# nkkrnkl/category-agnostic-pose-estimation

Measured on AMD Instinct MI355X. Metric: episodes/sec (1-shot, 256x256, 17kpt) training step, higher is better.
Workload: dtype f32 storage/accumulate, GEMMs as bf16x3 split (3 bf16 MFMAs per product); 1 GPU; configs[1]: 1-shot training step (fwd+loss+bwd+clip+AdamW at learning rate 0, dropout on), 256x256, 17 kpt, ResNet-50 + deformable transformer, 16 episodes x 2 queries per GPU; episodes_per_gpu=16, queries_per_episode=2, image_size=256, global_batch_episodes=16, parallelism=dp1, weights=random init (no checkpoint offline)

## Files before the change

### category-agnostic-pose-estimation_amd/csrc/msda.hip

```cpp
#include <stdlib.h>
#include "common.h"

namespace {

struct Levels {
  int H[4], W[4], start[4];
};

constexpr int HEADS = 8, HD = 32, CH = HEADS * HD;

__device__ __forceinline__ int sel4(const int (&a)[4], int l) { return l == 0 ? a[0] : (l == 1 ? a[1] : (l == 2 ? a[2] : a[3])); }

__global__ void __launch_bounds__(256) msda_fwd_kernel(const float* __restrict__ value, const float* __restrict__ offw,
                                                        const float* __restrict__ ref, float* __restrict__ out,
                                                        Levels lv, int N, int S, int Lq, int L, int P, int blocks_per_image) {
  const int lane = threadIdx.x & 63, wv = threadIdx.x >> 6;
  int n, chunk;
  {
    const int b = blockIdx.x;
    const int xcd = b & 7, loc = b >> 3;
    const int imgs_per_x = (N + 7) >> 3;
    const int ii = loc / blocks_per_image;
    chunk = loc - ii * blocks_per_image;
    n = ii * 8 + xcd;
    if (ii >= imgs_per_x || n >= N) return;
  }
  const int q = chunk * 4 + wv;
  if (q >= Lq) return;
  const int LP = L * P;
  const int h = lane >> 3, c4 = lane & 7;
  const long long qrow = (long long)n * Lq + q;
  const float* ow = offw + qrow * (HEADS * LP * 3);
  const float* offs = ow + h * LP * 2;
  const float* logit = ow + HEADS * LP * 2 + h * LP;
  float px[2], py[2], lg[2];
  int lev[2];
#pragma unroll
  for (int s = 0; s < 2; ++s) {
    const int j = c4 + 8 * s;
    if (j < LP) {
      const int l = j / P;
      lev[s] = l;
      const float rx = ref[(qrow * L + l) * 2 + 0], ry = ref[(qrow * L + l) * 2 + 1];
      const float ox = offs[j * 2 + 0], oy = offs[j * 2 + 1];
      const float Wf = (float)sel4(lv.W, l), Hf = (float)sel4(lv.H, l);
      px[s] = (rx + ox / Wf) * Wf - 0.5f;
      py[s] = (ry + oy / Hf) * Hf - 0.5f;
      lg[s] = logit[j];
    } else {
      lev[s] = 0; px[s] = 0.f; py[s] = 0.f; lg[s] = -INFINITY;
    }
  }
  float mx = fmaxf(lg[0], lg[1]);
  mx = fmaxf(mx, __shfl_xor(mx, 1, 64)); mx = fmaxf(mx, __shfl_xor(mx, 2, 64)); mx = fmaxf(mx, __shfl_xor(mx, 4, 64));
  float e0 = __expf(lg[0] - mx), e1 = __expf(lg[1] - mx);
  float sm = e0 + e1;
  sm += __shfl_xor(sm, 1, 64); sm += __shfl_xor(sm, 2, 64); sm += __shfl_xor(sm, 4, 64);
  const float inv = 1.f / sm;
  const float aw[2] = {e0 * inv, e1 * inv};

  float4 acc = make_float4(0.f, 0.f, 0.f, 0.f);
  const float* vbase = value + (long long)n * S * CH + h * HD + c4 * 4;
#pragma unroll
  for (int s = 0; s < 2; ++s) {
#pragma unroll
    for (int jj = 0; jj < 8; ++jj) {
      const int j = jj + 8 * s;
      if (j >= LP) break;
      const int src = (lane & ~7) | jj;
      const float x = __shfl(px[s], src, 64), y = __shfl(py[s], src, 64), a = __shfl(aw[s], src, 64);
      const int l = __shfl(lev[s], src, 64);
      const int W = sel4(lv.W, l), H = sel4(lv.H, l);
      const float xf = floorf(x), yf = floorf(y);
      const float fx = x - xf, fy = y - yf;
      const int x0 = (int)xf, y0 = (int)yf;
      const float* vl = vbase + (long long)sel4(lv.start, l) * CH;
      const bool xa = x0 >= 0 && x0 < W, xb = x0 + 1 >= 0 && x0 + 1 < W;
      const bool ya = y0 >= 0 && y0 < H, yb = y0 + 1 >= 0 && y0 + 1 < H;
      float4 v;
      if (ya && xa) { v = *reinterpret_cast<const float4*>(vl + (long long)(y0 * W + x0) * CH); const float w = a * (1.f - fx) * (1.f - fy);
        acc.x += w * v.x; acc.y += w * v.y; acc.z += w * v.z; acc.w += w * v.w; }
      if (ya && xb) { v = *reinterpret_cast<const float4*>(vl + (long long)(y0 * W + x0 + 1) * CH); const float w = a * fx * (1.f - fy);
        acc.x += w * v.x; acc.y += w * v.y; acc.z += w * v.z; acc.w += w * v.w; }
      if (yb && xa) { v = *reinterpret_cast<const float4*>(vl + (long long)((y0 + 1) * W + x0) * CH); const float w = a * (1.f - fx) * fy;
        acc.x += w * v.x; acc.y += w * v.y; acc.z += w * v.z; acc.w += w * v.w; }
      if (yb && xb) { v = *reinterpret_cast<const float4*>(vl + (long long)((y0 + 1) * W + x0 + 1) * CH); const float w = a * fx * fy;
        acc.x += w * v.x; acc.y += w * v.y; acc.z += w * v.z; acc.w += w * v.w; }
    }
  }
  *reinterpret_cast<float4*>(out + qrow * CH + h * HD + c4 * 4) = acc;
}

__device__ __forceinline__ float half_sum32(float v) {
  v += __shfl_xor(v, 1, 64); v += __shfl_xor(v, 2, 64); v += __shfl_xor(v, 4, 64);
  v += __shfl_xor(v, 8, 64); v += __shfl_xor(v, 16, 64);
  return v;
}

__global__ void __launch_bounds__(256) msda_bwd_kernel(const float* __restrict__ d_out, const float* __restrict__ value,
                                                        const float* __restrict__ offw, const float* __restrict__ ref,
                                                        float* __restrict__ d_value, float* __restrict__ d_offw,
                                                        float* __restrict__ d_ref, Levels lv, int N, int S, int Lq, int L,
                                                        int P, long long total_waves) {
  const int lane = threadIdx.x & 63, wv = threadIdx.x >> 6;
  const long long wid = (long long)blockIdx.x * 4 + wv;
  if (wid >= total_waves) return;
  const int pair = (int)(wid & 3);
  const long long qrow = wid >> 2;
  const int n = (int)(qrow / Lq);
  const int hh = lane >> 5, c = lane & 31;
  const int h = pair * 2 + hh;
  const int LP = L * P;
  const int j = c & 15;
  const int rowlen = HEADS * LP * 3;
  const float* ow = offw + qrow * rowlen;
  float px = 0.f, py = 0.f, lg = -INFINITY;
  int l_own = 0;
  if (j < LP) {
    l_own = j / P;
    const float rx = ref[(qrow * L + l_own) * 2 + 0], ry = ref[(qrow * L + l_own) * 2 + 1];
    const float ox = ow[(h * LP + j) * 2 + 0], oy = ow[(h * LP + j) * 2 + 1];
    const float Wf = (float)sel4(lv.W, l_own), Hf = (float)sel4(lv.H, l_own);
    px = (rx + ox / Wf) * Wf - 0.5f;
    py = (ry + oy / Hf) * Hf - 0.5f;
    lg = ow[HEADS * LP * 2 + h * LP + j];
  }
  float mx = lg;
  mx = fmaxf(mx, __shfl_xor(mx, 1, 64)); mx = fmaxf(mx, __shfl_xor(mx, 2, 64));
  mx = fmaxf(mx, __shfl_xor(mx, 4, 64)); mx = fmaxf(mx, __shfl_xor(mx, 8, 64));
  const float e = __expf(lg - mx);
  float sm = e;
  sm += __shfl_xor(sm, 1, 64); sm += __shfl_xor(sm, 2, 64); sm += __shfl_xor(sm, 4, 64); sm += __shfl_xor(sm, 8, 64);
  const float aw = e / sm;

  const float go = d_out[qrow * CH + h * HD + c];
  const float* vbase = value + (long long)n * S * CH + h * HD + c;
  float* dvbase = d_value + (long long)n * S * CH + h * HD + c;
  float my_daw = 0.f, my_dpx = 0.f, my_dpy = 0.f;
  for (int jj = 0; jj < LP; ++jj) {
    const int src = (lane & 32) | jj;
    const float x = __shfl(px, src, 64), y = __shfl(py, src, 64), a = __shfl(aw, src, 64);
    const int l = __shfl(l_own, src, 64);
    const int W = sel4(lv.W, l), H = sel4(lv.H, l);
    const float xf = floorf(x), yf = floorf(y);
    const float fx = x - xf, fy = y - yf;
    const int x0 = (int)xf, y0 = (int)yf;
    const long long lofs = (long long)sel4(lv.start, l) * CH;
    const bool xa = x0 >= 0 && x0 < W, xb = x0 + 1 >= 0 && x0 + 1 < W;
    const bool ya = y0 >= 0 && y0 < H, yb = y0 + 1 >= 0 && y0 + 1 < H;
    float v00 = 0.f, v01 = 0.f, v10 = 0.f, v11 = 0.f;
    const float ga = go * a;
    if (ya && xa) { const long long o = lofs + (long long)(y0 * W + x0) * CH; v00 = vbase[o]; atomicAdd(dvbase + o, ga * (1.f - fx) * (1.f - fy)); }
    if (ya && xb) { const long long o = lofs + (long long)(y0 * W + x0 + 1) * CH; v01 = vbase[o]; atomicAdd(dvbase + o, ga * fx * (1.f - fy)); }
    if (yb && xa) { const long long o = lofs + (long long)((y0 + 1) * W + x0) * CH; v10 = vbase[o]; atomicAdd(dvbase + o, ga * (1.f - fx) * fy); }
    if (yb && xb) { const long long o = lofs + (long long)((y0 + 1) * W + x0 + 1) * CH; v11 = vbase[o]; atomicAdd(dvbase + o, ga * fx * fy); }
    const float samp = (1.f - fy) * ((1.f - fx) * v00 + fx * v01) + fy * ((1.f - fx) * v10 + fx * v11);
    const float dsx = (1.f - fy) * (v01 - v00) + fy * (v11 - v10);
    const float dsy = (1.f - fx) * (v10 - v00) + fx * (v11 - v01);
    const float r_aw = half_sum32(go * samp);
    const float r_px = half_sum32(ga * dsx);
    const float r_py = half_sum32(ga * dsy);
    if (j == jj) { my_daw = r_aw; my_dpx = r_px; my_dpy = r_py; }
  }
  float dot = aw * my_daw;
  dot += __shfl_xor(dot, 1, 64); dot += __shfl_xor(dot, 2, 64); dot += __shfl_xor(dot, 4, 64); dot += __shfl_xor(dot, 8, 64);
  const float dlogit = aw * (my_daw - dot);
  float* dow = d_offw + qrow * rowlen;
  if (c < 16 && j < LP) {
    dow[(h * LP + j) * 2 + 0] = my_dpx;
    dow[(h * LP + j) * 2 + 1] = my_dpy;
    dow[HEADS * LP * 2 + h * LP + j] = dlogit;
  }
  if (d_ref) {
    float rx = (c < 16 && j < LP) ? my_dpx * (float)sel4(lv.W, l_own) : 0.f;
    float ry = (c < 16 && j < LP) ? my_dpy * (float)sel4(lv.H, l_own) : 0.f;
    if (P == 4) {
      rx += __shfl_xor(rx, 1, 64); rx += __shfl_xor(rx, 2, 64);
      ry += __shfl_xor(ry, 1, 64); ry += __shfl_xor(ry, 2, 64);
      if (c < 16 && j < LP && (j & 3) == 0) {
        atomicAdd(&d_ref[(qrow * L + l_own) * 2 + 0], rx);
        atomicAdd(&d_ref[(qrow * L + l_own) * 2 + 1], ry);
      }
    } else if (c < 16 && j < LP) {
      atomicAdd(&d_ref[(qrow * L + l_own) * 2 + 0], rx);
      atomicAdd(&d_ref[(qrow * L + l_own) * 2 + 1], ry);
    }
  }
}



template <int CTRL>
__device__ __forceinline__ float dpp_f(float v) {
  return __builtin_bit_cast(float, __builtin_amdgcn_update_dpp(0, __builtin_bit_cast(int, v), CTRL, 0xf, 0xf, true));
}
__device__ __forceinline__ float sum8(float v) { v += dpp_f<0xB1>(v); v += dpp_f<0x4E>(v); v += dpp_f<0x141>(v); return v; }
__device__ __forceinline__ float max8(float v) {
  v = fmaxf(v, dpp_f<0xB1>(v)); v = fmaxf(v, dpp_f<0x4E>(v)); v = fmaxf(v, dpp_f<0x141>(v));
  return v;
}
__device__ __forceinline__ float sum16(float v) { v = sum8(v); v += dpp_f<0x140>(v); return v; }
__device__ __forceinline__ float max16(float v) { v = max8(v); v = fmaxf(v, dpp_f<0x140>(v)); return v; }

struct Tap { unsigned i00, i01, i10, i11; float fx, fy; };
__device__ __forceinline__ Tap make_tap(float px, float py, int W, int H, int start, bool live, int S) {
  const float xf = floorf(px), yf = floorf(py);
  Tap t;
  t.fx = px - xf; t.fy = py - yf;
  const int x0 = (int)xf, y0 = (int)yf;
  const bool xa = x0 >= 0 && x0 < W, xb = x0 + 1 >= 0 && x0 + 1 < W;
  const bool ya = y0 >= 0 && y0 < H, yb = y0 + 1 >= 0 && y0 + 1 < H;
  const int base = start + y0 * W + x0;
  t.i00 = (live && ya && xa) ? (unsigned)base : (unsigned)S;
  t.i01 = (live && ya && xb) ? (unsigned)(base + 1) : (unsigned)S;
  t.i10 = (live && yb && xa) ? (unsigned)(base + W) : (unsigned)S;
  t.i11 = (live && yb && xb) ? (unsigned)(base + W + 1) : (unsigned)S;
  return t;
}

__global__ void __launch_bounds__(256) msda_fwd_rec_kernel(const float* __restrict__ value, const float* __restrict__ offw,
                                                            const float* __restrict__ ref, float* __restrict__ out, Levels lv,
                                                            int N, int S, int Lq, int L, int P, int blocks_per_image) {
  __shared__ uint2 rec_ids[4][HEADS * 16];
  __shared__ float4 rec_w[4][HEADS * 16];
  const int lane = threadIdx.x & 63, wv = threadIdx.x >> 6;
  int n, chunk;
  {
    const int b = blockIdx.x;
    const int xcd = b & 7, loc = b >> 3;
    const int ii = loc / blocks_per_image;
    chunk = loc - ii * blocks_per_image;
    n = ii * 8 + xcd;
    if (n >= N) return;
  }
  const int q = chunk * 4 + wv;
  if (q >= Lq) return;
  const int LP = L * P;
  const int h = lane >> 3, i = lane & 7;
  const long long qrow = (long long)n * Lq + q;
  const float* ow = offw + qrow * (HEADS * LP * 3);
  float px[2], py[2], lg[2];
  int W[2], H[2], st[2];
#pragma unroll
  for (int s = 0; s < 2; ++s) {
    const int j = i + 8 * s;
    px[s] = 0.f; py[s] = 0.f; lg[s] = -INFINITY; W[s] = 1; H[s] = 1; st[s] = 0;
    if (j < LP) {
      const int l = j / P;
      W[s] = sel4(lv.W, l); H[s] = sel4(lv.H, l); st[s] = sel4(lv.start, l);
      const float2 rr = *reinterpret_cast<const float2*>(ref + (qrow * L + l) * 2);
      const float2 oo = *reinterpret_cast<const float2*>(ow + (h * LP + j) * 2);
      const float Wf = (float)W[s], Hf = (float)H[s];
      px[s] = (rr.x + oo.x / Wf) * Wf - 0.5f;
      py[s] = (rr.y + oo.y / Hf) * Hf - 0.5f;
      lg[s] = ow[HEADS * LP * 2 + h * LP + j];
    }
  }
  const float mx = max8(fmaxf(lg[0], lg[1]));
  const float e0 = __expf(lg[0] - mx), e1 = __expf(lg[1] - mx);
  const float inv = 1.f / sum8(e0 + e1);
  const float aw[2] = {e0 * inv, e1 * inv};
#pragma unroll
  for (int s = 0; s < 2; ++s) {
    const int j = i + 8 * s;
    const Tap t = make_tap(px[s], py[s], W[s], H[s], st[s], j < LP, S);
    const unsigned cl = (unsigned)(S - 1);
    float4 w = make_float4(aw[s] * (1.f - t.fx) * (1.f - t.fy), aw[s] * t.fx * (1.f - t.fy), aw[s] * (1.f - t.fx) * t.fy,
                           aw[s] * t.fx * t.fy);
    if (t.i00 >= (unsigned)S) w.x = 0.f;
    if (t.i01 >= (unsigned)S) w.y = 0.f;
    if (t.i10 >= (unsigned)S) w.z = 0.f;
    if (t.i11 >= (unsigned)S) w.w = 0.f;
    rec_ids[wv][h * 16 + j] = make_uint2(min(t.i00, cl) | (min(t.i01, cl) << 16), min(t.i10, cl) | (min(t.i11, cl) << 16));
    rec_w[wv][h * 16 + j] = w;
  }
  const float* vb = value + (long long)n * S * CH + h * HD + i * 4;
  const uint2* rid = &rec_ids[wv][h * 16];
  const float4* rw = &rec_w[wv][h * 16];
  constexpr int PF = 4;
  float4 v[PF + 1][4];
  auto fetch = [&](int j, int slot) {
    const uint2 ids = rid[j];
    v[slot][0] = *reinterpret_cast<const float4*>(vb + (ids.x & 0xFFFFu) * (unsigned)CH);
    v[slot][1] = *reinterpret_cast<const float4*>(vb + (ids.x >> 16) * (unsigned)CH);
    v[slot][2] = *reinterpret_cast<const float4*>(vb + (ids.y & 0xFFFFu) * (unsigned)CH);
    v[slot][3] = *reinterpret_cast<const float4*>(vb + (ids.y >> 16) * (unsigned)CH);
  };
#pragma unroll
  for (int j = 0; j < PF; ++j)
    if (j < LP) fetch(j, j);
  float4 acc = make_float4(0.f, 0.f, 0.f, 0.f);
#pragma unroll
  for (int j = 0; j < 16; ++j) {
    if (j >= LP) continue;
    if (j + PF < LP) fetch(j + PF, (j + PF) % (PF + 1));
    const int slot = j % (PF + 1);
    const float4 w = rw[j];
    acc.x += w.x * v[slot][0].x + w.y * v[slot][1].x + w.z * v[slot][2].x + w.w * v[slot][3].x;
    acc.y += w.x * v[slot][0].y + w.y * v[slot][1].y + w.z * v[slot][2].y + w.w * v[slot][3].y;
    acc.z += w.x * v[slot][0].z + w.y * v[slot][1].z + w.z * v[slot][2].z + w.w * v[slot][3].z;
    acc.w += w.x * v[slot][0].w + w.y * v[slot][1].w + w.z * v[slot][2].w + w.w * v[slot][3].w;
  }
  *reinterpret_cast<float4*>(out + qrow * CH + h * HD + i * 4) = acc;
}

__global__ void __launch_bounds__(256) msda_bwd_offw_kernel(const float* __restrict__ d_out, const float* __restrict__ value,
                                                             const float* __restrict__ offw, const float* __restrict__ ref,
                                                             float* __restrict__ d_offw, float* __restrict__ d_ref, Levels lv,
                                                             int N, int S, int Lq, int L, int P, int blocks_per_image) {
  __shared__ uint4 recs[4][HEADS * 16];
  const int lane = threadIdx.x & 63, wv = threadIdx.x >> 6;
  int n, chunk;
  {
    const int b = blockIdx.x;
    const int xcd = b & 7, loc = b >> 3;
    const int ii = loc / blocks_per_image;
    chunk = loc - ii * blocks_per_image;
    n = ii * 8 + xcd;
    if (n >= N) return;
  }
  const int q = chunk * 4 + wv;
  if (q >= Lq) return;
  const int LP = L * P;
  const int h = lane >> 3, i = lane & 7;
  const long long qrow = (long long)n * Lq + q;
  const int rowlen = HEADS * LP * 3;
  const float* ow = offw + qrow * rowlen;
  float lg[2], aw[2];
  int lev[2];
#pragma unroll
  for (int s = 0; s < 2; ++s) {
    const int j = i + 8 * s;
    const bool live = j < LP;
    float px = 0.f, py = 0.f;
    int W = 1, H = 1, st = 0;
    lg[s] = -INFINITY; lev[s] = 0;
    if (live) {
      const int l = j / P;
      lev[s] = l;
      W = sel4(lv.W, l); H = sel4(lv.H, l); st = sel4(lv.start, l);
      const float2 rr = *reinterpret_cast<const float2*>(ref + (qrow * L + l) * 2);
      const float2 oo = *reinterpret_cast<const float2*>(ow + (h * LP + j) * 2);
      const float Wf = (float)W, Hf = (float)H;
      px = (rr.x + oo.x / Wf) * Wf - 0.5f;
      py = (rr.y + oo.y / Hf) * Hf - 0.5f;
      lg[s] = ow[HEADS * LP * 2 + h * LP + j];
    }
    const Tap t = make_tap(px, py, W, H, st, live, S);
    recs[wv][h * 16 + j] = make_uint4(t.i00 | (t.i01 << 16), t.i10 | (t.i11 << 16), __float_as_uint(t.fx), __float_as_uint(t.fy));
  }
  {
    const float mx = max8(fmaxf(lg[0], lg[1]));
    const float e0 = __expf(lg[0] - mx), e1 = __expf(lg[1] - mx);
    const float inv = 1.f / sum8(e0 + e1);
    aw[0] = e0 * inv; aw[1] = e1 * inv;
  }
  const float4 go = *reinterpret_cast<const float4*>(d_out + qrow * CH + h * HD + i * 4);
  const float* vb = value + (long long)n * S * CH + h * HD + i * 4;
  float daw[2] = {0.f, 0.f}, dpx[2] = {0.f, 0.f}, dpy[2] = {0.f, 0.f};
  const uint4* myrec = &recs[wv][h * 16];
  constexpr int PF = 2;
  uint4 ra[PF + 1];
  float4 v[PF + 1][4];
  auto fetch = [&](int j, int slot) {
    ra[slot] = myrec[j];
    const unsigned ids[4] = {ra[slot].x & 0xFFFFu, ra[slot].x >> 16, ra[slot].y & 0xFFFFu, ra[slot].y >> 16};
#pragma unroll
    for (int k = 0; k < 4; ++k) {
      const unsigned idc = min(ids[k], (unsigned)(S - 1));
      const float4 x = *reinterpret_cast<const float4*>(vb + idc * (unsigned)CH);
      v[slot][k] = ids[k] < (unsigned)S ? x : make_float4(0.f, 0.f, 0.f, 0.f);
    }
  };
#pragma unroll
  for (int j = 0; j < PF; ++j)
    if (j < LP) fetch(j, j);
#pragma unroll
  for (int j = 0; j < 16; ++j) {
    if (j >= LP) continue;
    if (j + PF < LP) fetch(j + PF, (j + PF) % (PF + 1));
    const int slot = j % (PF + 1);
    const float fx = __uint_as_float(ra[slot].z), fy = __uint_as_float(ra[slot].w);
    const float4 v00 = v[slot][0], v01 = v[slot][1], v10 = v[slot][2], v11 = v[slot][3];
    float p_aw = 0.f, p_x = 0.f, p_y = 0.f;
#define CAPE_TAP_CH(C)                                                             \
    {                                                                              \
      const float dt = v01.C - v00.C, db = v11.C - v10.C;                          \
      const float top = v00.C + fx * dt, bot = v10.C + fx * db;                    \
      p_aw += go.C * (top + fy * (bot - top));                                     \
      p_x += go.C * (dt + fy * (db - dt));                                         \
      p_y += go.C * (bot - top);                                                   \
    }
    CAPE_TAP_CH(x) CAPE_TAP_CH(y) CAPE_TAP_CH(z) CAPE_TAP_CH(w)
#undef CAPE_TAP_CH
    const float r_aw = sum8(p_aw), r_x = sum8(p_x), r_y = sum8(p_y);
    if (i == (j & 7)) { daw[j >> 3] = r_aw; dpx[j >> 3] = r_x; dpy[j >> 3] = r_y; }
  }
  const float dot = sum8(aw[0] * daw[0] + aw[1] * daw[1]);
  float* dow = d_offw + qrow * rowlen;
#pragma unroll
  for (int s = 0; s < 2; ++s) {
    const int j = i + 8 * s;
    const bool live = j < LP;
    const float gx = aw[s] * dpx[s], gy = aw[s] * dpy[s];
    if (live) {
      *reinterpret_cast<float2*>(dow + (h * LP + j) * 2) = make_float2(gx, gy);
      dow[HEADS * LP * 2 + h * LP + j] = aw[s] * (daw[s] - dot);
    }
    if (d_ref) {
      float rx = live ? gx * (float)sel4(lv.W, lev[s]) : 0.f;
      float ry = live ? gy * (float)sel4(lv.H, lev[s]) : 0.f;
      if (P == 4) {
        rx += dpp_f<0xB1>(rx); rx += dpp_f<0x4E>(rx);
        ry += dpp_f<0xB1>(ry); ry += dpp_f<0x4E>(ry);
        rx += __shfl_xor(rx, 8); rx += __shfl_xor(rx, 16); rx += __shfl_xor(rx, 32);
        ry += __shfl_xor(ry, 8); ry += __shfl_xor(ry, 16); ry += __shfl_xor(ry, 32);
        if (live && h == 0 && (i & 3) == 0) *reinterpret_cast<float2*>(&d_ref[(qrow * L + lev[s]) * 2]) = make_float2(rx, ry);
      } else if (live) {
        atomicAdd(&d_ref[(qrow * L + lev[s]) * 2 + 0], rx);
        atomicAdd(&d_ref[(qrow * L + lev[s]) * 2 + 1], ry);
      }
    }
  }
}

struct ValRec { uint2 ids; float4 w; };

template <int VC>
__global__ void __launch_bounds__(1024) msda_bwd_value_kernel(const float* __restrict__ d_out, const float* __restrict__ offw,
                                                              const float* __restrict__ ref, float* __restrict__ d_value,
                                                              Levels lv, int N, int S, int Lq, int L, int P) {
  constexpr int VS = VC, GROUPS = HD / VC, BPI = HEADS * GROUPS;
  constexpr int SLOTS = 64 / VC;
  extern __shared__ __attribute__((aligned(16))) double slab[];
  __shared__ uint2 rec_ids[16][64];
  __shared__ float4 rec_w[16][64];
  int n, sub;
  {
    const int b = blockIdx.x, xcd = b & 7, loc = b >> 3;
    n = (loc / BPI) * 8 + xcd;
    sub = loc % BPI;
    if (n >= N) return;
  }
  const int h = sub / GROUPS, grp = sub % GROUPS;
  for (int k = threadIdx.x; k < (S + 1) * VS; k += 1024) slab[k] = 0.0;
  __syncthreads();

  const int lane = threadIdx.x & 63, wv = threadIdx.x >> 6;
  const int g = lane >> 4, j = lane & 15;
  const int c = lane & (VC - 1), slot = lane / VC;
  static_assert(SLOTS * VC == 64 && 16 % VC == 0, "a slot's records must stay inside one query");
  const int LP = L * P;
  const int rowlen = HEADS * LP * 3;
  const int choff = h * HD + grp * VC + c;

  const int l_own = j < LP ? j / P : 0;
  const int W = sel4(lv.W, l_own), H = sel4(lv.H, l_own), st = sel4(lv.start, l_own);
  const float Wf = (float)W, Hf = (float)H;
  const int g2 = (slot * VC) >> 4;
  struct In { float2 rr, oo; float lg, go; };
  auto fetch = [&](int qb) {
    In in;
    const int q = qb + g, q2 = qb + g2;
    const long long qrow = (long long)n * Lq + min(q, Lq - 1);
    const float* ow = offw + qrow * rowlen;
    const int jj = min(j, LP - 1);
    in.rr = *reinterpret_cast<const float2*>(ref + (qrow * L + l_own) * 2);
    in.oo = *reinterpret_cast<const float2*>(ow + (h * LP + jj) * 2);
    in.lg = ow[HEADS * LP * 2 + h * LP + jj];
    in.go = d_out[((long long)n * Lq + min(q2, Lq - 1)) * CH + choff];
    return in;
  };
  In cur = fetch(wv * 4);
  for (int qb = wv * 4; qb < Lq; qb += 64) {
    const In nxt = fetch(min(qb + 64, Lq - 1));
    const int q = qb + g;
    const bool qlive = q < Lq;
    {
      const bool slive = qlive && j < LP;
      const float px = (cur.rr.x + cur.oo.x / Wf) * Wf - 0.5f;
      const float py = (cur.rr.y + cur.oo.y / Hf) * Hf - 0.5f;
      const float lg = slive ? cur.lg : -INFINITY;
      const float mx = max16(lg);
      const float e = slive ? __expf(lg - mx) : 0.f;
      const float sm = sum16(e);
      const float aw = slive ? e / sm : 0.f;
      const Tap t = make_tap(px, py, W, H, st, slive, S);
      rec_ids[wv][lane] = make_uint2(t.i00 | (t.i01 << 16), t.i10 | (t.i11 << 16));
      rec_w[wv][lane] = make_float4(aw * (1.f - t.fx) * (1.f - t.fy), aw * t.fx * (1.f - t.fy), aw * (1.f - t.fx) * t.fy,
                                    aw * t.fx * t.fy);
    }
    const float go = (qb + g2 < Lq) ? cur.go : 0.f;
    const int rbase = slot * VC;
#pragma unroll
    for (int s = 0; s < VC; ++s) {
      const uint2 ids = rec_ids[wv][rbase + s];
      const float4 w = rec_w[wv][rbase + s];
      atomicAdd(&slab[(ids.x & 0xFFFFu) * VS + c], (double)(go * w.x));
      atomicAdd(&slab[(ids.x >> 16) * VS + c], (double)(go * w.y));
      atomicAdd(&slab[(ids.y & 0xFFFFu) * VS + c], (double)(go * w.z));
      atomicAdd(&slab[(ids.y >> 16) * VS + c], (double)(go * w.w));
    }
    cur = nxt;
  }
  __syncthreads();
  float* dvb = d_value + (long long)n * S * CH + h * HD + grp * VC;
  if constexpr (VC >= 4) {
    constexpr int Q = VC / 4;
    for (int k = threadIdx.x; k < S * Q; k += 1024) {
      const int p_ = k / Q, c4 = (k % Q) * 4;
      const double* sp = &slab[p_ * VS + c4];
      *reinterpret_cast<float4*>(dvb + (long long)p_ * CH + c4) = make_float4((float)sp[0], (float)sp[1], (float)sp[2], (float)sp[3]);
    }
  } else {
    for (int k = threadIdx.x; k < S; k += 1024)
      *reinterpret_cast<float2*>(dvb + (long long)k * CH) = make_float2((float)slab[k * VS], (float)slab[k * VS + 1]);
  }
}

typedef float v2f __attribute__((ext_vector_type(2)));

template <int VP>
__global__ void __launch_bounds__(1024) msda_bwd_value_fx_kernel(const float* __restrict__ d_out, const float* __restrict__ offw,
                                                                 const float* __restrict__ ref, float* __restrict__ d_value,
                                                                 Levels lv, int N, int S, int Lq, int L, int P) {
  constexpr int VC = 2 * VP, GROUPS = HD / VC, BPI = HEADS * GROUPS;
  constexpr int SLOTS = 64 / VP;
  extern __shared__ __attribute__((aligned(16))) unsigned long long fslab[];
  __shared__ uint4 rec_off[16][64];
  __shared__ float4 rec_w[16][64];
  __shared__ unsigned gmax_w[16];
  int n, sub;
  {
    const int b = blockIdx.x, xcd = b & 7, loc = b >> 3;
    n = (loc / BPI) * 8 + xcd;
    sub = loc % BPI;
    if (n >= N) return;
  }
  const int h = sub / GROUPS, grp = sub % GROUPS;
  const int lane = threadIdx.x & 63, wv = threadIdx.x >> 6;
  const int ch0 = h * HD + grp * VC;
  for (int k = threadIdx.x; k < (S + 1) * VP; k += 1024) fslab[k] = 0ull;
  unsigned gb = 0u;
  for (int k = threadIdx.x; k < Lq * VP; k += 1024) {
    const int q = k / VP, c2 = (k - q * VP) * 2;
    const float2 v = *reinterpret_cast<const float2*>(d_out + ((long long)n * Lq + q) * CH + ch0 + c2);
    gb = max(gb, max(__float_as_uint(fabsf(v.x)), __float_as_uint(fabsf(v.y))));
  }
#pragma unroll
  for (int o = 32; o >= 1; o >>= 1) gb = max(gb, (unsigned)__shfl_xor((int)gb, o));
  if (lane == 0) gmax_w[wv] = gb;
  __syncthreads();
  gb = gmax_w[0];
#pragma unroll
  for (int k = 1; k < 16; ++k) gb = max(gb, gmax_w[k]);
  const bool finite = gb < 0x7f800000u;
  float scale = 0.f, inv_scale = 0.f;
  if (finite && gb != 0u) {
    int e;
    (void)frexpf(__uint_as_float(gb), &e);
    const int lq_bits = Lq > 1 ? 32 - __clz(Lq - 1) : 0;
    const int sx = max(-126, min(126, min(30 - lq_bits, 21) - e));
    scale = ldexpf(1.f, sx);
    inv_scale = ldexpf(1.f, -sx);
  }

  const int g = lane >> 4, j = lane & 15;
  const int c = lane & (VP - 1), slot = lane / VP;
  static_assert(SLOTS * VP == 64 && 16 % VP == 0, "a slot's records must stay inside one query");
  const int LP = L * P;
  const int rowlen = HEADS * LP * 3;
  const int choff = ch0 + 2 * c;
  const int l_own = j < LP ? j / P : 0;
  const int W = sel4(lv.W, l_own), H = sel4(lv.H, l_own), st = sel4(lv.start, l_own);
  const float Wf = (float)W, Hf = (float)H;
  const int g2 = (slot * VP) >> 4;
  struct In { float2 rr, oo, go; float lg; };
  auto fetch = [&](int qb) {
    In in;
    const int q = qb + g, q2 = qb + g2;
    const long long qrow = (long long)n * Lq + min(q, Lq - 1);
    const float* ow = offw + qrow * rowlen;
    const int jj = min(j, LP - 1);
    in.rr = *reinterpret_cast<const float2*>(ref + (qrow * L + l_own) * 2);
    in.oo = *reinterpret_cast<const float2*>(ow + (h * LP + jj) * 2);
    in.lg = ow[HEADS * LP * 2 + h * LP + jj];
    in.go = *reinterpret_cast<const float2*>(d_out + ((long long)n * Lq + min(q2, Lq - 1)) * CH + choff);
    return in;
  };
  char* const slab_c = reinterpret_cast<char*>(fslab) + c * 8;
  auto add2 = [&](unsigned off, float wgt, v2f gg) {
    const v2f t = __builtin_elementwise_fma(gg, (v2f)(wgt), (v2f)(12582912.f));
    const int v0 = (int)__float_as_uint(t.x) - 0x4B400000, v1 = (int)__float_as_uint(t.y) - 0x4B400000;
    const unsigned long long pk = ((unsigned long long)(unsigned)(v1 + (v0 >> 31)) << 32) | (unsigned)v0;
    atomicAdd(reinterpret_cast<unsigned long long*>(slab_c + off), pk);
  };
  In cur = fetch(wv * 4);
  for (int qb = wv * 4; qb < Lq; qb += 64) {
    const In nxt = fetch(min(qb + 64, Lq - 1));
    const int q = qb + g;
    const bool qlive = q < Lq;
    {
      const bool slive = qlive && j < LP;
      const float px = (cur.rr.x + cur.oo.x / Wf) * Wf - 0.5f;
      const float py = (cur.rr.y + cur.oo.y / Hf) * Hf - 0.5f;
      const float lg = slive ? cur.lg : -INFINITY;
      const float mx = max16(lg);
      const float e = slive ? __expf(lg - mx) : 0.f;
      const float sm = sum16(e);
      const float aw = slive ? e / sm : 0.f;
      const Tap t = make_tap(px, py, W, H, st, slive, S);
      rec_off[wv][lane] = make_uint4(t.i00 * (VP * 8), t.i01 * (VP * 8), t.i10 * (VP * 8), t.i11 * (VP * 8));
      rec_w[wv][lane] = make_float4(aw * (1.f - t.fx) * (1.f - t.fy), aw * t.fx * (1.f - t.fy), aw * (1.f - t.fx) * t.fy,
                                    aw * t.fx * t.fy);
    }
    const bool live2 = qb + g2 < Lq;
    v2f gg;
    gg.x = live2 ? cur.go.x * scale : 0.f;
    gg.y = live2 ? cur.go.y * scale : 0.f;
    const int rbase = slot * VP;
#pragma unroll
    for (int s = 0; s < VP; ++s) {
      const uint4 off = rec_off[wv][rbase + s];
      const float4 w = rec_w[wv][rbase + s];
      add2(off.x, w.x, gg);
      add2(off.y, w.y, gg);
      add2(off.z, w.z, gg);
      add2(off.w, w.w, gg);
    }
    cur = nxt;
  }
  __syncthreads();
  float* dvb = d_value + (long long)n * S * CH + ch0;
  const float nanv = __uint_as_float(0x7fc00000u);
  auto dec = [&](unsigned long long wd, float& lo, float& hi) {
    const int l = (int)(unsigned)wd;
    const int hh = (int)(unsigned)(wd >> 32) - (l >> 31);
    lo = finite ? (float)l * inv_scale : nanv;
    hi = finite ? (float)hh * inv_scale : nanv;
  };
  constexpr int Q = VP / 2;
  for (int k = threadIdx.x; k < S * Q; k += 1024) {
    const int p_ = k / Q, c2 = (k % Q) * 2;
    float4 o;
    dec(fslab[p_ * VP + c2], o.x, o.y);
    dec(fslab[p_ * VP + c2 + 1], o.z, o.w);
    *reinterpret_cast<float4*>(dvb + (long long)p_ * CH + c2 * 2) = o;
  }
}

int fill_levels(Levels& lv, const int* shapes, const int* level_start, int L, int S) {
  CAPE_REQUIRE(L >= 1 && L <= 4, "cape_msda: L=%d must be in 1..4", L);
  long long tot = 0;
  for (int l = 0; l < 4; ++l) {
    lv.H[l] = l < L ? shapes[2 * l] : 1;
    lv.W[l] = l < L ? shapes[2 * l + 1] : 1;
    lv.start[l] = l < L ? level_start[l] : 0;
    if (l < L) {
      CAPE_REQUIRE(lv.H[l] > 0 && lv.W[l] > 0 && lv.start[l] == tot, "cape_msda: level %d shape/start inconsistent", l);
      tot += (long long)lv.H[l] * lv.W[l];
    }
  }
  CAPE_REQUIRE(tot == S, "cape_msda: sum(H*W)=%lld != S=%d", tot, S);
  return 0;
}

}

extern "C" int cape_msda_fwd(const float* value, const float* offw, const float* ref, const int* shapes,
                             const int* level_start, float* out, int N, int S, int Lq, int L, int P,
                             cape_stream_t stream) {
  CAPE_REQUIRE(value && offw && ref && shapes && level_start && out, "cape_msda_fwd: null pointer");
  CAPE_REQUIRE(P >= 1 && L * P <= 16, "cape_msda_fwd: L*P=%d must be <= 16", L * P);
  if (N <= 0 || Lq <= 0) return 0;
  Levels lv;
  if (fill_levels(lv, shapes, level_start, L, S)) return 1;
  const int bpi = (Lq + 3) / 4;
  const int imgs_per_x = (N + 7) / 8;
  const long long blocks = (long long)imgs_per_x * bpi * 8;
  CAPE_REQUIRE(blocks < (1ll << 31), "cape_msda_fwd: grid too large");
  static const bool shuffle_form = getenv("CAPE_MSDA_FWD_SHUFFLE") != nullptr;
  if (S < 65535 && !shuffle_form)
    hipLaunchKernelGGL(msda_fwd_rec_kernel, dim3((unsigned)blocks), dim3(256), 0, as_stream(stream), value, offw, ref, out, lv,
                       N, S, Lq, L, P, bpi);
  else
    hipLaunchKernelGGL(msda_fwd_kernel, dim3((unsigned)blocks), dim3(256), 0, as_stream(stream), value, offw, ref, out, lv,
                       N, S, Lq, L, P, bpi);
  CAPE_LAUNCH_CHECK("cape_msda_fwd");
  return 0;
}

static int msda_bwd_check(const float* d_out, const float* value, const float* offw, const float* ref, const int* shapes,
                          const int* level_start, float* d_value, float* d_offw, int L, int P) {
  CAPE_REQUIRE(d_out && value && offw && ref && shapes && level_start && d_value && d_offw, "cape_msda_bwd: null pointer");
  CAPE_REQUIRE(P >= 1 && L * P <= 16, "cape_msda_bwd: L*P=%d must be <= 16", L * P);
  return 0;
}

extern "C" int cape_msda_bwd_atomic(const float* d_out, const float* value, const float* offw, const float* ref,
                                    const int* shapes, const int* level_start, float* d_value, float* d_offw, float* d_ref,
                                    int N, int S, int Lq, int L, int P, cape_stream_t stream) {
  if (msda_bwd_check(d_out, value, offw, ref, shapes, level_start, d_value, d_offw, L, P)) return 1;
  if (N <= 0 || Lq <= 0) return 0;
  Levels lv;
  if (fill_levels(lv, shapes, level_start, L, S)) return 1;
  hipError_t e = hipMemsetAsync(d_value, 0, sizeof(float) * (size_t)N * S * CH, as_stream(stream));
  if (e == hipSuccess && d_ref) e = hipMemsetAsync(d_ref, 0, sizeof(float) * (size_t)N * Lq * L * 2, as_stream(stream));
  if (e != hipSuccess) return cape_set_error("cape_msda_bwd_atomic: memset: %s", hipGetErrorString(e));
  const long long waves = (long long)N * Lq * 4;
  const long long blocks = (waves + 3) / 4;
  CAPE_REQUIRE(blocks < (1ll << 31), "cape_msda_bwd_atomic: grid too large");
  hipLaunchKernelGGL(msda_bwd_kernel, dim3((unsigned)blocks), dim3(256), 0, as_stream(stream), d_out, value, offw, ref,
                     d_value, d_offw, d_ref, lv, N, S, Lq, L, P, waves);
  CAPE_LAUNCH_CHECK("cape_msda_bwd_atomic");
  return 0;
}

extern "C" int cape_msda_bwd(const float* d_out, const float* value, const float* offw, const float* ref,
                             const int* shapes, const int* level_start, float* d_value, float* d_offw, float* d_ref,
                             int N, int S, int Lq, int L, int P, cape_stream_t stream) {
  return cape_msda_bwd_ex(d_out, value, offw, ref, shapes, level_start, d_value, d_offw, d_ref, N, S, Lq, L, P, 0, stream);
}

extern "C" int cape_msda_bwd_ex(const float* d_out, const float* value, const float* offw, const float* ref,
                                const int* shapes, const int* level_start, float* d_value, float* d_offw, float* d_ref,
                                int N, int S, int Lq, int L, int P, int value_accum, cape_stream_t stream) {
  CAPE_REQUIRE(value_accum == 0 || value_accum == 1, "cape_msda_bwd_ex: value_accum must be 0 (fp64 slab) or 1 (fixed-point pairs)");
  if (msda_bwd_check(d_out, value, offw, ref, shapes, level_start, d_value, d_offw, L, P)) return 1;
  if (N <= 0 || Lq <= 0) return 0;
  const size_t kMaxSlab = 160 * 1024 - 16 * 64 * (sizeof(uint4) + sizeof(float4)) - 512;
  int vc = 8;
  while (vc >= 2 && (size_t)(S + 1) * vc * sizeof(double) > kMaxSlab) vc >>= 1;
  const size_t slab_bytes = (size_t)(S + 1) * vc * sizeof(double);
  static const bool force_atomic = getenv("CAPE_MSDA_BWD_ATOMIC") != nullptr;
  const long long imgs8 = ((long long)N + 7) / 8;
  const int bpi = (Lq + 3) / 4;
  const long long vblocks = imgs8 * 8 * HEADS * (HD / (vc < 2 ? 2 : vc));
  if (force_atomic || vc < 2 || S >= 65535 || vblocks >= (1ll << 31) || imgs8 * 8 * bpi >= (1ll << 31))
    return cape_msda_bwd_atomic(d_out, value, offw, ref, shapes, level_start, d_value, d_offw, d_ref, N, S, Lq, L, P, stream);
  Levels lv;
  if (fill_levels(lv, shapes, level_start, L, S)) return 1;
  static bool attr_done = false;
  if (!attr_done) {
    hipError_t e = hipFuncSetAttribute(reinterpret_cast<const void*>(msda_bwd_value_kernel<8>),
                                       hipFuncAttributeMaxDynamicSharedMemorySize, (int)kMaxSlab);
    if (e == hipSuccess) e = hipFuncSetAttribute(reinterpret_cast<const void*>(msda_bwd_value_kernel<4>),
                                                 hipFuncAttributeMaxDynamicSharedMemorySize, (int)kMaxSlab);
    if (e == hipSuccess) e = hipFuncSetAttribute(reinterpret_cast<const void*>(msda_bwd_value_kernel<2>),
                                                 hipFuncAttributeMaxDynamicSharedMemorySize, (int)kMaxSlab);
    if (e == hipSuccess) e = hipFuncSetAttribute(reinterpret_cast<const void*>(msda_bwd_value_fx_kernel<8>),
                                                 hipFuncAttributeMaxDynamicSharedMemorySize, (int)kMaxSlab);
    if (e == hipSuccess) e = hipFuncSetAttribute(reinterpret_cast<const void*>(msda_bwd_value_fx_kernel<4>),
                                                 hipFuncAttributeMaxDynamicSharedMemorySize, (int)kMaxSlab);
    if (e == hipSuccess) e = hipFuncSetAttribute(reinterpret_cast<const void*>(msda_bwd_value_fx_kernel<2>),
                                                 hipFuncAttributeMaxDynamicSharedMemorySize, (int)kMaxSlab);
    if (e != hipSuccess) return cape_set_error("cape_msda_bwd: hipFuncSetAttribute: %s", hipGetErrorString(e));
    attr_done = true;
  }
  if (d_ref && P != 4) {
    hipError_t e = hipMemsetAsync(d_ref, 0, sizeof(float) * (size_t)N * Lq * L * 2, as_stream(stream));
    if (e != hipSuccess) return cape_set_error("cape_msda_bwd: memset: %s", hipGetErrorString(e));
  }
#define VALUE_LAUNCH(W)                                                                                                     \
  hipLaunchKernelGGL((msda_bwd_value_kernel<W>), dim3((unsigned)vblocks), dim3(1024), slab_bytes, as_stream(stream), d_out, offw, \
                     ref, d_value, lv, N, S, Lq, L, P)
#define VALUE_LAUNCH_FX(W)                                                                                                  \
  hipLaunchKernelGGL((msda_bwd_value_fx_kernel<W>), dim3((unsigned)fxblocks), dim3(1024), fx_bytes, as_stream(stream),           \
                     d_out, offw, ref, d_value, lv, N, S, Lq, L, P)
  if (value_accum == 1) {
    int vp = vc;
    while (vp > 2 && imgs8 * 8 * HEADS * (HD / (2 * vp)) < 256) vp >>= 1;
    const long long fxblocks = imgs8 * 8 * HEADS * (HD / (2 * vp));
    const size_t fx_bytes = (size_t)(S + 1) * vp * sizeof(unsigned long long);
    if (vp == 8) VALUE_LAUNCH_FX(8); else if (vp == 4) VALUE_LAUNCH_FX(4); else VALUE_LAUNCH_FX(2);
  } else {
    if (vc == 8) VALUE_LAUNCH(8); else if (vc == 4) VALUE_LAUNCH(4); else VALUE_LAUNCH(2);
  }
#undef VALUE_LAUNCH_FX
#undef VALUE_LAUNCH
  hipLaunchKernelGGL(msda_bwd_offw_kernel, dim3((unsigned)(imgs8 * 8 * bpi)), dim3(256), 0, as_stream(stream), d_out, value, offw,
                     ref, d_offw, d_ref, lv, N, S, Lq, L, P, bpi);
  CAPE_LAUNCH_CHECK("cape_msda_bwd");
  return 0;
}
```

### category-agnostic-pose-estimation_amd/hip/functional.py

```python
import contextlib
import ctypes
import os

import torch

from . import lib, ops


class Runtime:
    rng = None
    direct_grad = False
    use_side_stream = os.environ.get("CAPE_SIDE_STREAM", "1") == "1"
    side = None
    on_param_grad = []
    capture_keep = None

    pending = []
    side_dirty = False

    defer_wgrad = os.environ.get("CAPE_DEFER_WGRAD", "1") == "1"
    wgrad_group = int(os.environ.get("CAPE_WGRAD_GROUP", "12"))
    wq = {}
    wq_total = 0
    wq_notify = []
# ... 536 lines not shown
    return BottleneckFn.apply(x, w1, w2, w3, wd, bn1[0], bn1[1], bn2[0], bn2[1], bn3[0], bn3[1], sd, bd, int(stride), torch.is_grad_enabled(),
                              int(dilation))


def conv_bn_act(x, weight, scale, shift, stride=1, pad=0, relu=False, residual=None, dilation=1):
    return ConvFn.apply(x, weight, scale, shift, residual, int(stride), int(pad), bool(relu), torch.is_grad_enabled(), int(dilation))


class AddLayerNormFn(torch.autograd.Function):
    @staticmethod
    def forward(ctx, x, y, gamma, beta, pos, dropout_p, rng_stream):
        x, y, pos = _c(x), _c(y), _c(pos)
        rng = Runtime.get_rng(x.device) if dropout_p > 0 else None
        out, mean, rstd, out_pos = ops.add_layernorm_fwd(x, y, gamma, beta, pos=pos, dropout_p=dropout_p, rng=rng,
                                                         rng_stream=rng_stream)
        ctx.save_for_backward(x, y, gamma, mean, rstd)
        ctx.refs = (gamma, beta)
        ctx.slot = _slot_of(x)
        ctx.meta = (dropout_p, rng_stream, pos is not None)
        ctx.set_materialize_grads(False)
        if pos is None:
            return out
        return out, out_pos

    @staticmethod
    def backward(ctx, d_out, d_out_pos=None):
        x, y, gamma, mean, rstd = ctx.saved_tensors
        p, stream, has_pos = ctx.meta
        g_pos = d_out_pos
        if d_out is None and d_out_pos is None:
            return None, None, None, None, None, None, None
        if d_out is None:
            d_out, d_out_pos = d_out_pos, None
        d_out, d_out_pos = _c(d_out), _c(d_out_pos)
        pg = _ParamGrads(ctx.refs)
        rng = Runtime.get_rng(x.device) if p > 0 else None
        dx, dy = ops.add_layernorm_bwd(d_out, d_out_pos, x, y, gamma, mean, rstd, *pg.bufs, dropout_p=p, rng=rng,
                                       rng_stream=stream)
        if y is None or dy is not dx:
            _slot_offer(ctx.slot, dx)
        dpos = g_pos if (has_pos and ctx.needs_input_grad[4]) else None
        return (dx, (dy if y is not None else None)) + pg.result() + (dpos, None, None)


def add_layernorm(x, y, gamma, beta, pos=None, dropout_p=0.0, rng_stream=0):
    return AddLayerNormFn.apply(x, y, gamma, beta, pos, float(dropout_p), int(rng_stream))


class AddFn(torch.autograd.Function):
    @staticmethod
    def forward(ctx, a, b):
        return ops.add(_c(a), _c(b))

    @staticmethod
    def backward(ctx, g):
        return g, g


def add(a, b):
    return AddFn.apply(a, b)


class FanOutFn(torch.autograd.Function):

    @staticmethod
    def forward(ctx, x, k, slot):
        ctx.k, ctx.slot = k, slot
        ctx.set_materialize_grads(False)
        return tuple(x.view_as(x) for _ in range(k))

    @staticmethod
    def backward(ctx, *grads):
        ctx.slot.buf = None
        gs, seen = [], set()
        for g in grads:
            if g is not None and (g.data_ptr(), g.numel()) not in seen:
                seen.add((g.data_ptr(), g.numel()))
                gs.append(g)
        if not gs:
            return None, None, None
        if len(gs) > 1 and len(gs) <= 8 and not all(g.is_contiguous() for g in gs) and all(_row_strided(g) for g in gs):
            return ops.add_n_rows(gs), None, None
        gs = [_c(g) for g in gs]
        out = gs[0]
        for i in range(0, len(gs) - 1, 7):
            out = ops.add_n([out] + gs[1 + i:8 + i]) if len(gs) > 1 else out
        return out, None, None


def _row_strided(g):
    if g.dim() < 2 or g.stride(-1) != 1 or g.shape[-1] % 4 or g.data_ptr() % 16 or g.stride(-2) % 4:
        return False
    st, sh = g.stride(), g.shape
    return all(st[i] == st[i + 1] * sh[i + 1] for i in range(len(sh) - 2))


def fanout(x, k):
    if k == 1 or not (torch.is_grad_enabled() and x.requires_grad):
        return (x,) * k
    slot = _Slot()
    outs = FanOutFn.apply(x, k, slot)
    for o in outs:
        o._cape_slot = slot
    return outs


class GeluFn(torch.autograd.Function):
    @staticmethod
    def forward(ctx, x):
        x = _c(x)
        ctx.save_for_backward(x)
        return ops.gelu(x)

    @staticmethod
    def backward(ctx, g):
        (x,) = ctx.saved_tensors
        return ops.gelu_bwd(x, _c(g))


def gelu(x):
    return GeluFn.apply(x)


class ScaleResidualFn(torch.autograd.Function):

    @staticmethod
    def forward(ctx, x, y, gamma):
        y = _c(y)
        ctx.has_x = x is not None
        ctx.save_for_backward(y, gamma)
        ctx.gref = gamma
        return ops.scale_residual(_c(x) if x is not None else torch.zeros_like(y), y, gamma)

    @staticmethod
    def backward(ctx, g):
        y, gamma = ctx.saved_tensors
        g = _c(g)
        dx = g if ctx.has_x else None
        if gamma is None:
            return dx, g, None
        pg = _ParamGrads((ctx.gref,))
        dy = ops.scale_residual_bwd(g, y, gamma, pg.bufs[0])
        return (dx, dy) + pg.result()


def scale_residual(x, y, gamma=None):
    return ScaleResidualFn.apply(x, y, gamma)


class BiAttnCoreFn(torch.autograd.Function):

    @staticmethod
    def forward(ctx, rv_l, rv_p, nheads, scale):
        rv_l, rv_p = _c(rv_l), _c(rv_p)
        B, Nl, D2 = rv_l.shape
        Np, D = rv_p.shape[1], D2 // 2
        ctx.route = "scalar"
        lat, s1 = ops.attn_core_fwd(ctx.route, rv_l[..., :D], rv_p[..., :D], rv_p[..., D:], B, nheads, Nl, Np, scale)
        pat, s2 = ops.attn_core_fwd(ctx.route, rv_p[..., :D], rv_l[..., :D], rv_l[..., D:], B, nheads, Np, Nl, scale)
        ctx.save_for_backward(rv_l, rv_p, lat, pat, *s1, *s2)
        ctx.meta = (nheads, scale)
        return lat, pat

    @staticmethod
    def backward(ctx, d_lat, d_pat):
        rv_l, rv_p, lat, pat, *saved = ctx.saved_tensors
        s1, s2 = saved[:len(saved) // 2], saved[len(saved) // 2:]
        nheads, scale = ctx.meta
        B, Nl, D2 = rv_l.shape
        Np, D = rv_p.shape[1], D2 // 2
        d_l, d_p = torch.empty_like(rv_l), torch.empty_like(rv_p)
        t_l, t_p = torch.empty_like(rv_l), torch.empty_like(rv_p)
        ops.attn_core_bwd(ctx.route, s1, _c(d_lat), rv_l[..., :D], rv_p[..., :D], rv_p[..., D:], lat, d_l[..., :D], d_p[..., :D],
                          d_p[..., D:], B, nheads, Nl, Np, scale)
        ops.attn_core_bwd(ctx.route, s2, _c(d_pat), rv_p[..., :D], rv_l[..., :D], rv_l[..., D:], pat, t_p[..., :D], t_l[..., :D],
                          d_l[..., D:], B, nheads, Np, Nl, scale)
        ops.add_n_rows([d_l[..., :D], t_l[..., :D]], out=d_l[..., :D])
        ops.add_n_rows([d_p[..., :D], t_p[..., :D]], out=d_p[..., :D])
        return d_l, d_p, None, None


def bi_attn_core(rv_l, rv_p, nheads, scale):
    return BiAttnCoreFn.apply(rv_l, rv_p, nheads, float(scale))


class AttnKVFn(torch.autograd.Function):

    @staticmethod
    def forward(ctx, r_q, rv_kv, nheads, scale):
        r_q, rv_kv = _c(r_q), _c(rv_kv)
        B, Nq, D = r_q.shape
        Nk = rv_kv.shape[1]
        ctx.route = "scalar"
        out, saved = ops.attn_core_fwd(ctx.route, r_q, rv_kv[..., :D], rv_kv[..., D:], B, nheads, Nq, Nk, scale)
        ctx.save_for_backward(r_q, rv_kv, out, *saved)
        ctx.meta = (nheads, scale)
        return out

    @staticmethod
    def backward(ctx, d_out):
        r_q, rv_kv, out, *saved = ctx.saved_tensors
        nheads, scale = ctx.meta
        B, Nq, D = r_q.shape
        Nk = rv_kv.shape[1]
        dq, dkv = torch.empty_like(r_q), torch.empty_like(rv_kv)
        ops.attn_core_bwd(ctx.route, saved, _c(d_out), r_q, rv_kv[..., :D], rv_kv[..., D:], out, dq, dkv[..., :D], dkv[..., D:], B, nheads,
                          Nq, Nk, scale)
        return dq, dkv, None, None


def attn_kv(r_q, rv_kv, nheads, scale):
    return AttnKVFn.apply(r_q, rv_kv, nheads, float(scale))


class LevelGroupNormFn(torch.autograd.Function):

    @staticmethod
    def forward(ctx, geo, *args):
        L = geo.L
        xs, gammas, betas = args[:L], args[L:2 * L], args[2 * L:3 * L]
        N, C = xs[0].shape[0], xs[0].shape[-1]
        out = torch.empty(N, geo.S, C, dtype=torch.float32, device=xs[0].device)
        stats = []
        xs = [_c(x) for x in xs]
        for l, x in enumerate(xs):
            h, w = geo.shapes[l]
            assert x.shape[1] == h and x.shape[2] == w
            stats.append(ops.groupnorm_fwd(x, gammas[l], betas[l], out[:, geo.starts[l]:], geo.S * C, N, h * w, C))
        ctx.geo = geo
        ctx.refs = (tuple(gammas), tuple(betas))
        ctx.save_for_backward(*xs, *gammas, *[s for st in stats for s in st])
        return out

    @staticmethod
    def backward(ctx, d_out):
        geo = ctx.geo
        L = geo.L
        sv = ctx.saved_tensors
        xs, gammas, st = sv[:L], sv[L:2 * L], sv[2 * L:]
        d_out = _c(d_out)
        N, S, C = d_out.shape
        dxs, dgs, dbs = [], [], []
        for l in range(L):
            h, w = geo.shapes[l]
            pg = _ParamGrads((ctx.refs[0][l], ctx.refs[1][l]))
            dx = ops.groupnorm_bwd(d_out[:, geo.starts[l]:], S * C, xs[l], gammas[l], st[2 * l], st[2 * l + 1], *pg.bufs, N,
                                   h * w, C)
            dg, db = pg.result()
            dxs.append(dx); dgs.append(dg); dbs.append(db)
        return (None, *dxs, *dgs, *dbs)


def level_groupnorm(geo, xs, gammas, betas):
    return LevelGroupNormFn.apply(geo, *xs, *gammas, *betas)


_SINE_CACHE = {}


class LevelPosFn(torch.autograd.Function):

    @staticmethod
    def forward(ctx, geo, level_embed, *masks_u8):
        N = masks_u8[0].shape[0]
        C = level_embed.shape[1]
        out = torch.empty(N, geo.S, C, dtype=torch.float32, device=level_embed.device)
        key = (tuple(m.data_ptr() for m in masks_u8), tuple(geo.shapes), N, C, str(level_embed.device))
        sine = _SINE_CACHE.get(key) if all(getattr(m, "_cape_all_false", False) for m in masks_u8) else None
        if sine is None:
            target = out
            if all(getattr(m, "_cape_all_false", False) for m in masks_u8) and not capturing():
                target = torch.empty_like(out)
            zero_row = torch.zeros(C, dtype=torch.float32, device=level_embed.device) if target is not out else None
            for l, m in enumerate(masks_u8):
                h, w = geo.shapes[l]
                ops.pos_sine_level(_c(m), zero_row if zero_row is not None else level_embed[l], target[:, geo.starts[l]:], geo.S * C, N, h, w, C)
            if target is not out:
                if len(_SINE_CACHE) >= 8:
                    _SINE_CACHE.pop(next(iter(_SINE_CACHE)))
                _SINE_CACHE[key] = sine = target
        if sine is not None:
            ops.level_embed_add(sine, _c(level_embed), geo, out)
        ctx.geo = geo
        ctx.N = N
        ctx.le_ref = level_embed
        return out

    @staticmethod
    def backward(ctx, d_pos):
        geo, N = ctx.geo, ctx.N
        d_pos = _c(d_pos)
        C = d_pos.shape[-1]
        pg = _ParamGrads((ctx.le_ref,))
        for l in range(geo.L):
            h, w = geo.shapes[l]
            ops.colsum(d_pos[0, geo.starts[l]:], h * w, C, pg.bufs[0][l], nbatch=N, batch_stride=geo.S * C)
        return (None,) + pg.result() + (None,) * geo.L


def level_pos(geo, level_embed, masks_u8):
    return LevelPosFn.apply(geo, level_embed, *masks_u8)


class MSDAFn(torch.autograd.Function):
    @staticmethod
    def forward(ctx, value, offw, ref, geo, P):
        value, offw, ref = _c(value), _c(offw), _c(ref)
        N, Lq = offw.shape[0], offw.shape[1]
        out = ops.msda_fwd(value, offw, ref, geo, N, Lq, P)
        ctx.save_for_backward(value, offw, ref)
        ctx.meta = (geo, N, Lq, P)
        return out

    @staticmethod
    def backward(ctx, d_out):
        value, offw, ref = ctx.saved_tensors
        geo, N, Lq, P = ctx.meta
        dv, do, dr = ops.msda_bwd(_c(d_out), value, offw, ref, geo, N, Lq, P, need_ref_grad=ctx.needs_input_grad[2])
        return dv, do, dr, None, None


def msda(value, offw, ref, geo, P=4):
    return MSDAFn.apply(value, offw, ref, geo, P)


def _from_row(t, r):
    return t if (t is None or r == 0) else t[r:]


def _col_blocks(groups, bufs, C):
    return [buf[..., j * C:(j + 1) * C] for (_, w, *_), buf in zip(groups, bufs) for j in range(w)]


class MHAFn(torch.autograd.Function):

    @staticmethod
    def forward(ctx, q_in, k_in, v_in, in_w, in_b, out_w, out_b, nheads, mask_mode, kpm_u8, dropout_p, rng_stream):
        ins = q_in, k_in, v_in = _c(q_in), _c(k_in), _c(v_in)
        N, Lq, C = q_in.shape
        Lk = k_in.shape[1]
        dev = q_in.device
        scale = (C // nheads) ** -0.5
        rng = Runtime.get_rng(dev) if dropout_p > 0 else None
        ctx.route = ops.attn_route(N, nheads, Lq, Lk, flash=False)
        if ctx.route != "mm" and k_in is v_in:
            layout = ((0, 3),) if q_in is k_in else ((0, 1), (1, 2))
        else:
            layout = ((0, 1), (1, 1), (2, 1))
        ctx.groups = tuple((r, w, r != 1 and ins[r] is k_in) for r, w in layout)
        bufs = [torch.empty(N, ins[r].shape[1], w * C, dtype=torch.float32, device=dev) for r, w in layout]
        for (r, w), buf in zip(layout, bufs):
            ops.gemm(ins[r].view(-1, C), _from_row(in_w, r * C), buf, N * ins[r].shape[1], w * C, C, bias=_from_row(in_b, r * C))
        q, k, v = _col_blocks(layout, bufs, C)
        O, saved = ops.attn_core_fwd(ctx.route, q, k, v, N, nheads, Lq, Lk, scale, mask_mode=mask_mode, kpm=kpm_u8, dropout_p=dropout_p,
                                     rng=rng, rng_stream=rng_stream)
        out = torch.empty(N, Lq, C, dtype=torch.float32, device=dev)
        ops.gemm(O.view(-1, C), out_w, out, N * Lq, C, C, bias=out_b)
        ctx.save_for_backward(q_in, k_in, v_in, in_w, out_w, q, k, v, O, kpm_u8, *saved)
        ctx.refs = (in_w, in_b, out_w, out_b)
        ctx.slot_q = _slot_of(q_in)
        ctx.meta = (nheads, mask_mode, dropout_p, rng_stream, scale)
        return out

    @staticmethod
    def backward(ctx, d_out):
        q_in, k_in, v_in, in_w, out_w, q, k, v, O, kpm, *saved = ctx.saved_tensors
        nheads, mask_mode, p, stream, scale = ctx.meta
        ins = q_in, k_in, v_in
        N, Lq, C = q_in.shape
        Lk = k_in.shape[1]
        dev = d_out.device
        d_out2 = _c(d_out).view(-1, C)
        Mq = N * Lq
        dO = torch.empty(Mq, C, dtype=torch.float32, device=dev)
        ops.gemm(d_out2, out_w, dO, Mq, C, C, a_mode=0, b_mode=1)
        pg = _ParamGrads(ctx.refs)
        d_in_w, d_in_b, d_out_w, d_out_b = pg.bufs
        with pg.side(d_out2, O):
            pg.gemm(d_out2, O.view(-1, C), d_out_w, C, C, Mq, a_mode=1, b_mode=1, accumulate=True,
                    split_k=ops.pick_split_k(C, C, Mq), colsum_out=d_out_b)
        dbufs = [torch.empty(N, ins[r].shape[1], w * C, dtype=torch.float32, device=dev) for r, w, _ in ctx.groups]
        dq, dk, dv = _col_blocks(ctx.groups, dbufs, C)
        rng = Runtime.get_rng(dev) if p > 0 else None
        ops.attn_core_bwd(ctx.route, saved, dO.view(N, Lq, C), q, k, v, O, dq, dk, dv, N, nheads, Lq, Lk, scale, mask_mode=mask_mode,
                          kpm=kpm, dropout_p=p, rng=rng, rng_stream=stream)
        pairs = list(zip(ctx.groups, dbufs))
        with pg.side(*dbufs, q_in, k_in, v_in):
            for (r, w, _), g in pairs:
                M = N * ins[r].shape[1]
                pg.gemm(g.view(-1, w * C), ins[r].view(-1, C), _from_row(d_in_w, r * C), w * C, C, M, a_mode=1, b_mode=1, lda=w * C,
                        accumulate=True, split_k=ops.pick_split_k(w * C, C, M), colsum_out=_from_row(d_in_b, r * C))
        d_in_w, d_in_b, d_out_w, d_out_b = pg.result()
        d_ins, dk_in = [None, None, None], None
        for (r, w, dup), g in pairs[1:] + pairs[:1]:
            live = [j for j in range(r, r + w) if ctx.needs_input_grad[j]]
            if not live:
                continue
            if dup and dk_in is not None:
                dst, acc = dk_in, True
            else:
                if r == 0 and len(pairs) == 2:
                    dst, acc = _grad_target(ctx.slot_q, ins[r].shape, dev)
                else:
                    dst, acc = torch.empty(ins[r].shape, dtype=torch.float32, device=dev), False
                d_ins[live[0]] = dst
            ops.gemm(g.view(-1, w * C), _from_row(in_w, r * C), dst, N * ins[r].shape[1], C, w * C, a_mode=0, b_mode=1, accumulate=acc)
            if live[0] == 1:
                dk_in = dst
        return (*d_ins, d_in_w, d_in_b, d_out_w, d_out_b, None, None, None, None, None)


class DecSelfAttnFn(torch.autograd.Function):

    @staticmethod
    def forward(ctx, tgt, pos, wq, wk, wv, in_w, in_b, out_w, out_b, nheads, dropout_p, rng_stream):
        N, L, C = tgt.shape
        M = N * L
        dev = tgt.device
        x, pos2 = _c(tgt).view(M, C), _c(pos).view(M, C)
        stacked = _adjacent(wq, wk) and _adjacent(wk, wv)
        qkv1 = torch.empty(M, 3 * C, dtype=torch.float32, device=dev)
        if stacked:
            ops.gemm(x, torch.as_strided(wq, (3 * C, C), (C, 1)), qkv1, M, 3 * C, C, residual=pos2, ldr=C, res_cols=C)
        else:
            ops.gemm(x, wq, qkv1, M, C, C, ldc=3 * C, residual=pos2, ldr=C)
            ops.gemm(x, wk, qkv1[:, C:], M, C, C, ldc=3 * C)
            ops.gemm(x, wv, qkv1[:, 2 * C:], M, C, C, ldc=3 * C)
        qkv2 = torch.empty(N, L, 3 * C, dtype=torch.float32, device=dev)
        ops.gemm(qkv1, in_w, qkv2, M, C, C, lda=3 * C, ldb=C, ldc=3 * C, bias=in_b,
                 batch=(3, 3, 0, C, 0, C * C, 0, C), bias_strides=(0, C))
        q, k, v = qkv2[..., :C], qkv2[..., C:2 * C], qkv2[..., 2 * C:]
        scale = (C // nheads) ** -0.5
        rng = Runtime.get_rng(dev) if dropout_p > 0 else None
        ctx.route = ops.attn_route(N, nheads, L, L, flash=True)
        O, saved = ops.attn_core_fwd(ctx.route, q, k, v, N, nheads, L, L, scale, mask_mode=1, dropout_p=dropout_p, rng=rng,
                                     rng_stream=rng_stream)
        out = torch.empty(N, L, C, dtype=torch.float32, device=dev)
        ops.gemm(O.view(M, C), out_w, out, M, C, C, bias=out_b)
        ctx.save_for_backward(x, wq, wk, wv, in_w, out_w, qkv1, qkv2, O, *saved)
        ctx.refs = (wq, wk, wv, in_w, in_b, out_w, out_b)
        ctx.meta = (nheads, dropout_p, rng_stream, scale, stacked, N, L, C)
        ctx.slot = _slot_of(tgt)
        return out

    @staticmethod
    def backward(ctx, d_out):
        x, wq, wk, wv, in_w, out_w, qkv1, qkv2, O, *saved = ctx.saved_tensors
        nheads, p, stream, scale, stacked, N, L, C = ctx.meta
        M = N * L
        dev = d_out.device
        d_out2 = _c(d_out).view(M, C)
        dO = torch.empty(M, C, dtype=torch.float32, device=dev)
        ops.gemm(d_out2, out_w, dO, M, C, C, a_mode=0, b_mode=1)
        dqkv2 = torch.empty(N, L, 3 * C, dtype=torch.float32, device=dev)
        dq, dk, dv = dqkv2[..., :C], dqkv2[..., C:2 * C], dqkv2[..., 2 * C:]
        q, k, v = qkv2[..., :C], qkv2[..., C:2 * C], qkv2[..., 2 * C:]
        rng = Runtime.get_rng(dev) if p > 0 else None
        ops.attn_core_bwd(ctx.route, saved, dO.view(N, L, C), q, k, v, O, dq, dk, dv, N, nheads, L, L, scale, mask_mode=1, dropout_p=p,
                          rng=rng, rng_stream=stream)
        dqkv1 = torch.empty(M, 3 * C, dtype=torch.float32, device=dev)
        ops.gemm(dqkv2.view(M, 3 * C), in_w, dqkv1, M, C, C, a_mode=0, b_mode=1, lda=3 * C, ldb=C, ldc=3 * C,
                 batch=(3, 3, 0, C, 0, C * C, 0, C))
        need_x, need_pos = ctx.needs_input_grad[0], ctx.needs_input_grad[1]
        dx = None
        if need_x:
            dx, acc = _grad_target(ctx.slot, (N, L, C), dev)
            if stacked:
                ops.gemm(dqkv1, torch.as_strided(wq, (3 * C, C), (C, 1)), dx, M, C, 3 * C, a_mode=0, b_mode=1, accumulate=acc)
            else:
                for i, w in enumerate((wq, wk, wv)):
                    ops.gemm(dqkv1[:, i * C:], w, dx, M, C, C, a_mode=0, b_mode=1, lda=3 * C, accumulate=acc or i > 0)

        pg = _ParamGrads(ctx.refs)
        d_wq, d_wk, d_wv, d_in_w, d_in_b, d_out_w, d_out_b = pg.bufs
        with pg.side(d_out2, O, dqkv2, qkv1, dqkv1, x):
            Mv = dqkv2.view(M, 3 * C)
            pg.gemm(d_out2, O.view(M, C), d_out_w, C, C, M, a_mode=1, b_mode=1, accumulate=True, split_k=ops.pick_split_k(C, C, M),
                    colsum_out=d_out_b)
            for i, dw in enumerate((d_wq, d_wk, d_wv)):
                pg.gemm(Mv[:, i * C:], qkv1[:, i * C:], d_in_w[i * C:], C, C, M, a_mode=1, b_mode=1, lda=3 * C, ldb=3 * C, accumulate=True,
                        split_k=ops.pick_split_k(C, C, M), colsum_out=d_in_b[i * C:])
                pg.gemm(dqkv1[:, i * C:], x, dw, C, C, M, a_mode=1, b_mode=1, lda=3 * C, ldb=C, accumulate=True,
                        split_k=ops.pick_split_k(C, C, M))
        dpos = dqkv1[:, :C].view(N, L, C) if need_pos else None
        return (dx, dpos) + pg.result() + (None, None, None)


def dec_self_attn(tgt, pos, wq, wk, wv, in_w, in_b, out_w, out_b, nheads=8, dropout_p=0.0, rng_stream=0):
    return DecSelfAttnFn.apply(tgt, pos, wq, wk, wv, in_w, in_b, out_w, out_b, nheads, float(dropout_p), int(rng_stream))


def mha(q_in, k_in, v_in, in_w, in_b, out_w, out_b, nheads=8, mask_mode=0, kpm_u8=None, dropout_p=0.0, rng_stream=0):
    return MHAFn.apply(q_in, k_in, v_in, in_w, in_b, out_w, out_b, nheads, mask_mode, kpm_u8, float(dropout_p), int(rng_stream))


class TokenEmbedFn(torch.autograd.Function):
    @staticmethod
    def forward(ctx, table, pad_idx, s11, s21, s12, s22, dx1, dx2, dy1, dy2):
        shape = s11.shape
        seqs = [_c(s).view(-1) for s in (s11, s21, s12, s22)]
        deltas = [_c(d).view(-1) for d in (dx1, dx2, dy1, dy2)]
        out = ops.token_embed_fwd(table, seqs, deltas)
        ctx.save_for_backward(*seqs, *deltas)
        ctx.t_ref = table
        ctx.meta = (table.shape, pad_idx)
        return out.view(*shape, table.shape[1])

    @staticmethod
    def backward(ctx, d_out):
        sv = ctx.saved_tensors
        tshape, pad_idx = ctx.meta
        pg = _ParamGrads((ctx.t_ref,))
        ops.token_embed_bwd(_c(d_out).view(-1, tshape[1]), sv[:4], sv[4:], pg.bufs[0], pad_idx if pad_idx is not None else -1)
        return pg.result() + (None,) * 9


def token_embed(table, pad_idx, s11, s21, s12, s22, dx1, dx2, dy1, dy2):
    return TokenEmbedFn.apply(table, pad_idx, s11, s21, s12, s22, dx1, dx2, dy1, dy2)


class QuerySineFn(torch.autograd.Function):
    @staticmethod
    def forward(ctx, ref):
        ref = _c(ref)
        ctx.save_for_backward(ref)
        return ops.query_sine_fwd(ref).view(*ref.shape[:-1], 256)

    @staticmethod
    def backward(ctx, d_out):
        (ref,) = ctx.saved_tensors
        return ops.query_sine_bwd(_c(d_out).view(-1, 256), ref).view_as(ref)


def query_sine(ref):
    return QuerySineFn.apply(ref)


class RefineFn(torch.autograd.Function):
    @staticmethod
    def forward(ctx, delta, ref):
        delta, ref = _c(delta), _c(ref)
        out = ops.refine_fwd(delta, ref)
        ctx.save_for_backward(out, ref)
        return out

    @staticmethod
    def backward(ctx, d_new):
        out, ref = ctx.saved_tensors
        d_delta, d_ref = ops.refine_bwd(_c(d_new), out, ref)
        return d_delta, d_ref


def refine(delta, ref):
    return RefineFn.apply(delta, ref)


class SigmoidFn(torch.autograd.Function):
    @staticmethod
    def forward(ctx, x):
        y = ops.sigmoid_fwd(_c(x))
        ctx.save_for_backward(y)
        return y

    @staticmethod
    def backward(ctx, dy):
        (y,) = ctx.saved_tensors
        return ops.sigmoid_bwd(_c(dy), y)


def sigmoid(x):
    return SigmoidFn.apply(x)


class RefScaleFn(torch.autograd.Function):

    @staticmethod
    def forward(ctx, ref, valid_ratios):
        ref, vr = _c(ref), _c(valid_ratios)
        N, Lq, _ = ref.shape
        L = vr.shape[1]
        ctx.save_for_backward(vr)
        ctx.meta = (N, Lq, L)
        return ops.ref_scale_fwd(ref, vr, Lq, L).view(N, Lq, L, 2)

    @staticmethod
    def backward(ctx, d):
        (vr,) = ctx.saved_tensors
        N, Lq, L = ctx.meta
        return ops.ref_scale_bwd(_c(d), vr, Lq, L).view(N, Lq, 2), None


def ref_scale(ref, valid_ratios):
    return RefScaleFn.apply(ref, valid_ratios)


class SupportEmbedFn(torch.autograd.Function):

    @staticmethod
    def forward(ctx, coords, W0, b0, pe1d):
        coords = _c(coords)
        N, P, _ = coords.shape
        C = W0.shape[0]
        h, pe = ops.support_embed_fwd(coords, W0, b0, pe1d, N, P, C)
        ctx.save_for_backward(h, coords)
        ctx.refs = (W0, b0)
        ctx.meta = (N, P, C)
        ctx.mark_non_differentiable(pe)
        ctx.set_materialize_grads(False)
        return h.view(N, P, C), pe.view(N, P, C)

    @staticmethod
    def backward(ctx, d_h, _d_pe):
        if d_h is None:
            return None, None, None, None
        h, coords = ctx.saved_tensors
        N, P, C = ctx.meta
        pg = _ParamGrads(ctx.refs)
        ops.support_embed_bwd(_c(d_h).view(-1, C), h, coords, *pg.bufs, N, P, C)
        return (None,) + pg.result() + (None,)


def support_embed(coords, W0, b0, pe1d):
    return SupportEmbedFn.apply(coords, W0, b0, pe1d)


class GCNAggFn(torch.autograd.Function):
# ... 156 lines not shown
```

### category-agnostic-pose-estimation_amd/hip/lib.py

```python
import ctypes
import os

import torch

from ctypes import POINTER, c_char_p, c_float, c_int, c_int32, c_int64, c_longlong, c_size_t, c_uint32, c_uint64, c_uint8, c_void_p

_HERE = os.path.dirname(os.path.abspath(__file__))
LIB_PATH = os.environ.get("CAPE_HIP_LIB", os.path.join(_HERE, "..", "csrc", "libcape_hip.so"))
LIB_PATH = os.path.abspath(LIB_PATH)

if not os.path.exists(LIB_PATH):
    raise ImportError(
        f"libcape_hip.so not found at {LIB_PATH}; build it with `python -c 'import __graft_entry__ as g; g.build()'` "
        "(or `make -C category-agnostic-pose-estimation_amd/csrc`).  There is no CPU fallback.")
try:
    _lib = ctypes.CDLL(LIB_PATH)
except OSError as e:
    raise ImportError(f"cannot load {LIB_PATH}: {e}") from e

_lib.cape_last_error.restype = c_char_p
_lib.cape_abi_version.restype = c_int


class GemmDesc(ctypes.Structure):
    _fields_ = [
        ("M", c_int), ("N", c_int), ("K", c_int), ("a_mode", c_int), ("b_mode", c_int),
        ("A", c_void_p), ("lda", c_longlong), ("B", c_void_p), ("ldb", c_longlong), ("C", c_void_p), ("ldc", c_longlong),
        ("cN", c_int), ("cH", c_int), ("cW", c_int), ("cC", c_int), ("cKH", c_int), ("cKW", c_int),
        ("cStride", c_int), ("cPad", c_int), ("cOH", c_int), ("cOW", c_int), ("cO", c_int),
        ("scale", c_void_p), ("bias", c_void_p), ("residual", c_void_p), ("ldr", c_longlong),
        ("relu", c_int), ("accumulate", c_int), ("split_k", c_int), ("dropout_p", c_float),
        ("rng_state", c_void_p), ("rng_stream", c_uint32), ("colsum_out", c_void_p), ("precision", c_int),
        ("B_packed", c_void_p),
        ("mask_src", c_void_p), ("ldm", c_longlong), ("mask_scale", c_float),
        ("batch", c_int), ("batch_div", c_int), ("sA0", c_longlong), ("sA1", c_longlong), ("sB0", c_longlong), ("sB1", c_longlong),
        ("sC0", c_longlong), ("sC1", c_longlong),
        ("res_cols", c_int), ("sBias0", c_longlong), ("sBias1", c_longlong),
        ("cPadX", c_int), ("cKHp", c_int), ("cKWp", c_int), ("cTapH0", c_int), ("cTapHS", c_int), ("cTapW0", c_int), ("cTapWS", c_int),
        ("cDil", c_int),
    ]


class PackItem(ctypes.Structure):
    _fields_ = [("B", c_void_p), ("out", c_void_p), ("ldb", c_longlong), ("N", c_int), ("K", c_int), ("b_mode", c_int), ("pad", c_int)]


class DecodeLinearDesc(ctypes.Structure):
    _fields_ = [
        ("N", c_int), ("K", c_int), ("Nout", c_int),
        ("X", c_void_p), ("ldx", c_longlong), ("in_gamma", c_void_p), ("in_beta", c_void_p), ("in_add", c_void_p), ("ld_add", c_longlong),
        ("W", c_void_p), ("ldw", c_longlong), ("bias", c_void_p),
        ("X2", c_void_p), ("ldx2", c_longlong), ("K2", c_int), ("W2", c_void_p), ("ldw2", c_longlong), ("n2", c_int),
        ("R", c_void_p), ("ldr", c_longlong), ("res_gamma", c_void_p), ("res_beta", c_void_p),
        ("relu", c_int), ("nseg", c_int), ("seg", c_int), ("out", c_void_p * 3), ("ldo", c_longlong * 3),
    ]


class DecodeTailDesc(ctypes.Structure):
    _fields_ = [
        ("N", c_int), ("L", c_int),
        ("P4", c_void_p), ("ldp", c_longlong), ("g3", c_void_p), ("b3", c_void_p),
        ("W1", c_void_p), ("B1", c_void_p), ("W2", c_void_p), ("B2", c_void_p), ("W3", c_void_p), ("B3", c_void_p),
        ("ref", c_void_p),
        ("Wc", c_void_p), ("Bc", c_void_p), ("ncls", c_int),
        ("Wp", c_void_p), ("Bp", c_void_p), ("gp", c_void_p), ("bp", c_void_p),
        ("dim_t", c_void_p), ("vr", c_void_p),
        ("ref_out", c_void_p), ("ld_ref", c_longlong),
        ("qpos_out", c_void_p), ("refin_out", c_void_p),
        ("cls_out", c_void_p), ("ld_cls", c_longlong),
        ("hs_out", c_void_p), ("ld_hs", c_longlong),
    ]


class AugItem(ctypes.Structure):
    _fields_ = [("src", c_void_p), ("aug", c_void_p), ("out", c_void_p), ("stat", c_void_p), ("h", c_int), ("w", c_int),
                ("M", c_float * 6), ("color_on", c_int), ("order", c_int * 4),
                ("bright", c_float), ("contrast", c_float), ("sat", c_float), ("hue", c_float),
                ("mode", c_int), ("noise_std", c_float), ("seed", c_uint32), ("blur_k", c_int), ("blur_w", c_float * 49)]


DECODE_MAX_LAYERS = 8
GEMM_GROUP_MAX = 32
SUMSQ_PARTS = 256
GUARD_ROW_SERIAL, GUARD_ROW_OK, GUARD_ROW_TOTAL, GUARD_ROW_NORM, GUARD_ROW_COEF, GUARD_ROW_LR, GUARD_ROW_LOSSES = range(7)
GUARD_NO_STEP = -1.0


class DecodeLayerDesc(ctypes.Structure):
    _fields_ = [(n, c_void_p) for n in (
        "w_qkv", "b_qkv", "w_qin", "k_cache", "v_cache", "w_o", "b_o", "ln2_g", "ln2_b",
        "w_sq", "b_sq", "sup_k", "sup_v", "sup_mask", "w_so", "b_so", "lns_g", "lns_b",
        "w_off", "b_off", "value", "w_mo", "b_mo", "ln1_g", "ln1_b",
        "w1", "b1", "w2", "b2", "ln3_g", "ln3_b", "m1w", "m1b", "m2w", "m2b", "m3w", "m3b")]


class DecodeStepDesc(ctypes.Structure):
    _fields_ = [
        ("N", c_int), ("n_layers", c_int), ("step", c_int), ("T", c_int), ("P", c_int), ("S", c_int), ("L", c_int),
        ("n_points", c_int), ("ncls", c_int), ("ffn_dim", c_int),
        ("shapes", c_int * 8), ("level_start", c_int * 4),
        ("emb", c_void_p), ("qpos0", c_void_p), ("refin0", c_void_p), ("ref0", c_void_p), ("vr", c_void_p), ("dim_t", c_void_p),
        ("class_w", c_void_p), ("class_b", c_void_p),
        ("pos_w", c_void_p), ("pos_b", c_void_p), ("pos_gamma", c_void_p), ("pos_beta", c_void_p),
        ("out_logits", c_void_p), ("ld_logits", c_longlong),
        ("out_coords", c_void_p), ("ld_coords", c_longlong),
        ("out_hs", c_void_p), ("ld_hs", c_longlong),
        ("layers", DecodeLayerDesc * DECODE_MAX_LAYERS),
    ]


P, I, LL, F, U32 = c_void_p, c_int, c_longlong, c_float, c_uint32
_SIGS = {
    "cape_rng_advance": [P, P],
    "cape_stream_fork": [P, P],
    "cape_stream_join": [P, P],
    "cape_gemm_f32": [POINTER(GemmDesc), P],
    "cape_gemm_group_f32": [POINTER(GemmDesc), I, I, P],
    "cape_pack_weights": [P, I, I, P],
    "cape_colsum_f32": [P, LL, I, LL, I, I, P, I, P],
    "cape_add_layernorm_fwd": [P, P, P, P, P, P, P, P, P, I, I, F, P, U32, P],
    "cape_add_layernorm_bwd": [P, P, P, P, P, P, P, P, P, P, P, I, I, F, P, U32, P],
    "cape_groupnorm_fwd": [P, P, P, P, LL, P, P, I, I, I, I, P, c_size_t, P],
    "cape_groupnorm_bwd": [P, LL, P, P, P, P, P, P, P, I, I, I, I, P, c_size_t, P],
    "cape_msda_fwd": [P, P, P, P, P, P, I, I, I, I, I, P],
    "cape_msda_bwd": [P, P, P, P, P, P, P, P, P, I, I, I, I, I, P],
    "cape_msda_bwd_ex": [P, P, P, P, P, P, P, P, P, I, I, I, I, I, I, P],
    "cape_msda_bwd_atomic": [P, P, P, P, P, P, P, P, P, I, I, I, I, I, P],
    "cape_attn_fwd": [P, P, P, P, P, LL, LL, LL, LL, LL, LL, LL, LL, I, I, I, I, F, I, I, P, F, P, U32, P],
    "cape_attn_bwd": [P, P, P, P, P, P, P, P, P, LL, LL, LL, LL, LL, LL, LL, LL, I, I, I, I, F, I, I, P, F, P, U32, P],
    "cape_flash_attn_fwd": [P, P, P, P, P, LL, LL, LL, LL, LL, LL, LL, LL, I, I, I, I, F, I, I, P, F, P, U32, P],
    "cape_flash_attn_bwd": [P, P, P, P, P, P, P, P, P, P, LL, LL, LL, LL, LL, LL, LL, LL, I, I, I, I, F, I, I, P, F, P, U32, P],
    "cape_attn_softmax_fwd": [P, P, P, I, I, I, I, F, I, I, P, F, P, U32, P],
    "cape_attn_softmax_bwd": [P, P, I, I, I, I, F, F, P, U32, P],
    "cape_add_f32": [P, P, P, LL, P],
    "cape_level_embed_add": [P, P, P, P, I, I, I, I, P],
    "cape_add_n_f32": [POINTER(c_void_p), I, P, LL, P],
    "cape_add_n_rows_f32": [POINTER(c_void_p), POINTER(c_longlong), I, P, LL, LL, I, P],
    "cape_augment_batch": [P, I, I, I, P, P, P],
    "cape_gelu_f32": [P, P, LL, P],
    "cape_support_masks": [P, P, P, I, I, I, P],
    "cape_interleave2x2_f32": [POINTER(c_void_p), P, P, I, I, I, I, P],
    "cape_gelu_bwd_f32": [P, P, P, LL, P],
    "cape_scale_residual_bwd_f32": [P, P, P, P, P, LL, I, P],
    "cape_scale_residual_f32": [P, P, P, P, LL, I, P],
    "cape_nchw_to_nhwc": [P, P, I, I, I, I, I, P],
    "cape_bn_fold": [P, P, P, P, F, P, P, I, P],
    "cape_maxpool3x3s2_nhwc": [P, P, I, I, I, I, P],
    "cape_bn_relu_bwd": [P, P, P, P, P, LL, I, I, P],
    "cape_affine_act_f32": [P, P, P, P, LL, I, I, P],
    "cape_relu_drop_bwd": [P, P, P, LL, F, P],
    "cape_pos_sine_level": [P, P, P, P, LL, I, I, I, I, P],
    "cape_token_embed_fwd": [P, P, P, P, P, P, P, P, P, P, LL, I, I, P],
    "cape_token_embed_bwd": [P, P, P, P, P, P, P, P, P, P, LL, I, I, I, P],
    "cape_query_sine_fwd": [P, P, P, LL, P],
    "cape_query_sine_bwd": [P, P, P, P, I, LL, P],
    "cape_refine_fwd": [P, P, P, LL, P],
    "cape_refine_bwd": [P, P, P, P, P, I, LL, P],
    "cape_sigmoid_fwd": [P, P, LL, P],
    "cape_sigmoid_bwd": [P, P, P, I, LL, P],
    "cape_ref_scale_fwd": [P, P, P, LL, I, I, P],
    "cape_ref_scale_bwd": [P, P, P, I, LL, I, I, P],
    "cape_support_embed_fwd": [P, P, P, P, P, P, P, I, I, I, P],
    "cape_support_embed_bwd": [P, P, P, P, P, I, I, I, P],
    "cape_adjacency": [P, P, P, P, I, I, P],
    "cape_gcn_aggregate_fwd": [P, P, P, I, I, I, P],
    "cape_gcn_aggregate_bwd": [P, P, P, P, I, I, I, P],
    "cape_zero_rows": [P, P, LL, I, P],
    "cape_legacy_coord_embed_fwd": [P, P, P, P, I, I, P],
    "cape_legacy_coord_embed_bwd": [P, P, P, P, P, P, P, I, I, P],
    "cape_support_edge_info_fwd": [P, P, P, P, LL, P, P, P, I, I, I, P],
    "cape_support_edge_info_bwd": [P, LL, P, P, P, I, I, P],
    "cape_pe_dropout_fwd": [P, P, P, I, I, I, F, P, U32, P],
    "cape_pe_dropout_bwd": [P, P, LL, F, P, U32, P],
    "cape_loss_fwd_bwd": [P, P, P, P, P, P, F, F, F, P, P, P, P, I, LL, P],
    "cape_sumsq": [P, LL, P, P],
    "cape_adamw_step": [P, P, P, P, LL, F, F, F, F, F, F, P, I, P, P, P],
    "cape_step_increment": [P, P],
    "cape_step_guard": [P, P, I, P, I, F, P, P, P, P, P, I, I, P],
    "cape_adamw_step_guarded": [P, P, P, P, LL, F, F, F, F, F, F, P, I, P, P, P, P],
    "cape_decode_next_tokens": [P, P, P, P, P, P, I, I, I, I, I, I, P],
    "cape_decode_advance": [P, LL, P, LL, P, P, P, I, I, I, I, I, I, I, P, I, I, P, P, P],
    "cape_decode_linear": [POINTER(DecodeLinearDesc), P],
    "cape_decode_tail": [POINTER(DecodeTailDesc), P],
    "cape_decode_step": [POINTER(DecodeStepDesc), P],
}
EXPORTS = ["cape_last_error", "cape_abi_version", "cape_groupnorm_workspace_bytes", "cape_packed_weight_bytes"] + list(_SIGS)
_lib.cape_packed_weight_bytes.argtypes = [I, I]
_lib.cape_packed_weight_bytes.restype = c_size_t
_lib.cape_groupnorm_workspace_bytes.argtypes = [I, I, I]
_lib.cape_groupnorm_workspace_bytes.restype = c_size_t

for _name, _args in _SIGS.items():
    _fn = getattr(_lib, _name)
    _fn.argtypes = _args
    _fn.restype = c_int


def last_error() -> str:
    return _lib.cape_last_error().decode()


def abi_version() -> int:
    return _lib.cape_abi_version()


def call(name, *args):
    rc = getattr(_lib, name)(*args)
    if rc != 0:
        raise RuntimeError(f"{name} failed: {last_error()}")


def raw():
    return _lib
```

### category-agnostic-pose-estimation_amd/hip/ops.py

```python
import ctypes
import math
import os
import weakref

import torch

from . import lib

_F32 = torch.float32


_raw_stream = getattr(torch._C, "_cuda_getCurrentRawStream", None)
_raw_device = getattr(torch._C, "_cuda_getDevice", None)


_side = [None]


def raw_current_stream():
    if _raw_stream is not None and _raw_device is not None:
        return _raw_stream(_raw_device())
    return torch.cuda.current_stream().cuda_stream


# ... 130 lines not shown
                return None
            cls._pack([e])
            e["epoch"], e["version"] = cls.epoch, base._version
        return e["buf"]

    @classmethod
    def _items(cls, es):
        arr = (lib.PackItem * len(es))()
        for i, e in enumerate(es):
            ptr, N, K, ldb, mode = e["item"]
            arr[i].B, arr[i].out, arr[i].ldb, arr[i].N, arr[i].K, arr[i].b_mode = ptr, e["buf"].data_ptr(), ldb, N, K, mode
        host = torch.frombuffer(bytearray(bytes(arr)), dtype=torch.uint8)
        return host

    @classmethod
    def _pack(cls, es):
        dev = es[0]["buf"].device
        tab = cls._items(es).to(dev)
        lib.call("cape_pack_weights", _p(tab), len(es), 16, _stream())
        es[0].setdefault("_keep", None)
        es[0]["_keep"] = tab

    @classmethod
    def invalidate_and_repack(cls):
        cls.epoch += 1
        if not cls.enabled or not cls.entries:
            return
        dead = [k for k, e in cls.entries.items() if e["base"]() is None]
        if dead and not torch.cuda.is_current_stream_capturing():
            for k in dead:
                del cls.entries[k]
            cls._table = None
        es = list(cls.entries.values())
        if not es:
            return
        if cls._table is None or cls._table[1] != len(es):
            if torch.cuda.is_current_stream_capturing():
                raise RuntimeError("PackedWeights: new weights were registered inside a graph capture")
            cls._table = (cls._items(es).to(es[0]["buf"].device), len(es))
        lib.call("cape_pack_weights", _p(cls._table[0]), len(es), 16, _stream())
        for e in es:
            b = e["base"]()
            e["epoch"], e["version"] = cls.epoch, (b._version if b is not None else -1)

    @classmethod
    def signature(cls):
        return tuple(cls.entries.keys())

    @classmethod
    def mark_repacked(cls):
        cls.epoch += 1
        for e in cls.entries.values():
            b = e["base"]()
            e["epoch"], e["version"] = cls.epoch, (b._version if b is not None else -1)

    @classmethod
    def clear(cls):
        cls.entries, cls._table = {}, None


def gemm(*args, **kw):
    launch_gemm(gemm_desc(*args, **kw)[0])


def gemm_desc(A, B, C, M, N, K, a_mode=0, b_mode=0, lda=None, ldb=None, ldc=None, bias=None, scale=None, residual=None,
              ldr=None, relu=False, accumulate=False, split_k=1, dropout_p=0.0, rng=None, rng_stream=0, conv=None,
              colsum_out=None, packed=None, mask_src=None, mask_scale=1.0, batch=None, res_cols=0, bias_strides=None, conv_sub=None,
              conv_dil=1):
    for t, n in ((A, "A"), (B, "B"), (C, "C"), (bias, "bias"), (scale, "scale"), (residual, "residual")):
        _chk(t, "gemm." + n, contiguous=False)
    if (_AUTO_SPLIT_NN and a_mode == 0 and b_mode == 1 and split_k == 1 and K >= 512 and M > 64 and batch is None and conv is None
            and bias is None and scale is None and residual is None and not relu and mask_src is None and dropout_p == 0.0
            and colsum_out is None and (ldc is None or ldc == N) and C.is_contiguous() and ((M + 63) // 64) * ((N + 63) // 64) <= 64):
        sk = pick_split_k(M, N, K)
        if sk >= 4 and _avail(C) >= M * N:
            if not accumulate:
                C.view(-1)[:M * N].zero_()
            split_k, accumulate = sk, True
    d = lib.GemmDesc()
    d.M, d.N, d.K, d.a_mode, d.b_mode = M, N, K, a_mode, b_mode
    d.A, d.B, d.C = A.data_ptr(), B.data_ptr(), C.data_ptr()
    d.lda = lda if lda is not None else (K if a_mode == 0 else M)
    d.ldb = ldb if ldb is not None else (K if b_mode == 0 else N)
    d.ldc = ldc if ldc is not None else N
    if conv is not None:
        (d.cN, d.cH, d.cW, d.cC, d.cKH, d.cKW, d.cStride, d.cPad, d.cOH, d.cOW, d.cO) = conv
        if conv_sub is not None:
            (d.cPadX, d.cKHp, d.cKWp, d.cTapH0, d.cTapHS, d.cTapW0, d.cTapWS) = conv_sub
            assert a_mode == 3 and b_mode == 2 and _avail(B) >= d.cO * d.cKHp * d.cKWp * d.cC
            assert _avail(A) >= d.cN * d.cOH * d.cOW * d.cO and _avail(C) >= d.cN * d.cH * d.cW * d.cC
            assert conv_dil == 1, "gemm: a tap sub-lattice takes no dilation"
        else:
            assert conv_dil >= 1, "gemm: conv dilation must be >= 1"
            assert d.cOH == (d.cH + 2 * d.cPad - conv_dil * (d.cKH - 1) - 1) // d.cStride + 1, "gemm: conv OH does not match the geometry"
            assert d.cOW == (d.cW + 2 * d.cPad - conv_dil * (d.cKW - 1) - 1) // d.cStride + 1, "gemm: conv OW does not match the geometry"
            n_in, n_out, n_w = d.cN * d.cH * d.cW * d.cC, d.cN * d.cOH * d.cOW * d.cO, d.cO * d.cKH * d.cKW * d.cC
            if a_mode == 2:
                assert _avail(A) >= n_in, "gemm: conv input too small"
            if a_mode == 3:
                assert _avail(A) >= n_out, "gemm: conv output gradient too small"
            if b_mode == 2:
                assert _avail(B) >= n_w, "gemm: conv weight too small"
            if b_mode == 3:
                assert _avail(B) >= n_in, "gemm: conv input too small"
        d.cDil = int(conv_dil)
    else:
        assert conv_dil == 1 and conv_sub is None, "gemm: conv_dil / conv_sub need the conv geometry"
    d.scale = scale.data_ptr() if scale is not None else None
    d.bias = bias.data_ptr() if bias is not None else None
    d.residual = residual.data_ptr() if residual is not None else None
    d.ldr = ldr if ldr is not None else N
    d.res_cols = int(res_cols)
    d.relu, d.accumulate, d.split_k = int(relu), int(accumulate), int(split_k)
    d.dropout_p = float(dropout_p)
    d.rng_state = rng.t.data_ptr() if (rng is not None and dropout_p > 0) else None
    d.rng_stream = rng_stream
    d.precision = GEMM_PRECISION
    if (packed is None and PackedWeights.enabled and GEMM_PRECISION >= 1 and a_mode == 0 and b_mode in (0, 1) and batch is None
            and split_k == 1 and K in (64, 128, 256) and M > 64 and 32 <= N <= _PACK_MAX_N):
        packed = PackedWeights.lookup(B, N, K, d.ldb, b_mode)
    if packed is not None and GEMM_PRECISION >= 1:
        assert packed.dtype == torch.int16 and packed.is_cuda and packed.numel() * 2 >= lib.raw().cape_packed_weight_bytes(N, K)
        d.B_packed = packed.data_ptr()
    if mask_src is not None:
        _chk(mask_src, "gemm.mask_src")
        assert mask_src.numel() == M * N and split_k == 1
        d.mask_src, d.ldm, d.mask_scale = mask_src.data_ptr(), N, float(mask_scale)
    if colsum_out is not None:
        _chk(colsum_out, "gemm.colsum_out", contiguous=False)
        assert a_mode == 1 and _avail(colsum_out) >= M
        d.colsum_out = colsum_out.data_ptr()
    if batch is not None:
        cnt, div, sA0, sA1, sB0, sB1, sC0, sC1 = batch
        assert cnt >= 1 and div >= 1 and cnt % div == 0
        d.batch, d.batch_div = cnt, div
        d.sA0, d.sA1, d.sB0, d.sB1, d.sC0, d.sC1 = sA0, sA1, sB0, sB1, sC0, sC1
        if bias_strides is not None:
            d.sBias0, d.sBias1 = bias_strides
            assert bias is not None and _avail(bias) >= (cnt // div - 1) * d.sBias0 + (div - 1) * d.sBias1 + N
        last0, last1 = cnt // div - 1, div - 1
        offA, offB, offC = last0 * sA0 + last1 * sA1, last0 * sB0 + last1 * sB1, last0 * sC0 + last1 * sC1
    else:
        offA = offB = offC = 0
    if a_mode == 0 and M > 0:
        assert _avail(A) >= offA + (M - 1) * d.lda + K, "gemm: A too small"
    if a_mode == 1 and K > 0:
        assert _avail(A) >= offA + (K - 1) * d.lda + M, "gemm: A^T too small"
    if b_mode == 0 and N > 0:
        assert _avail(B) >= offB + (N - 1) * d.ldb + K, "gemm: B too small"
    if b_mode == 1 and K > 0:
        assert _avail(B) >= offB + (K - 1) * d.ldb + N, "gemm: B too small"
    if M > 0:
        assert _avail(C) >= offC + (M - 1) * d.ldc + N, "gemm: C too small"
    if residual is not None:
        assert res_cols % 32 == 0 and 0 <= res_cols <= N
        assert _avail(residual) >= (M - 1) * d.ldr + (res_cols or N), "gemm: residual too small"
    if bias is not None:
        assert _avail(bias) >= N
    if scale is not None:
        assert scale.numel() >= N
    return d, (A, B, C, colsum_out)


def launch_gemm(d):
    if GemmProfiler.enabled:
        e0, e1 = torch.cuda.Event(enable_timing=True), torch.cuda.Event(enable_timing=True)
        st = _stream()
        ext = torch.cuda.ExternalStream(st.value) if _side[0] is not None else None
        e0.record(ext)
        lib.call("cape_gemm_f32", ctypes.byref(d), st)
        e1.record(ext)
        M, N, K, nb = d.M, d.N, d.K, max(d.batch, 1)
        GemmProfiler.records.append((e0, e1, 2.0 * M * N * K * nb, (M, N, K, d.a_mode, d.b_mode, d.split_k, nb),
                                     GemmProfiler.alg_bytes(M, N, K, nb), 1))
        return
    lib.call("cape_gemm_f32", ctypes.byref(d), _stream())


_AUTO_SPLIT_NN = os.environ.get("CAPE_AUTO_SPLIT_NN", "1") == "1" and os.environ.get("CAPE_DETERMINISTIC", "0") != "1"
_PACK_MAX_N = int(os.environ.get("CAPE_PACK_MAX_N", "1000000"))
_GROUP_BIG_MN = int(os.environ.get("CAPE_GROUP_BIG_MN", str(64 * 1024)))


def group_tile(M, N, K):
    return 128 if (M >= 128 and N >= 128 and M * N >= _GROUP_BIG_MN and K >= 4096) else 64


def plan_group_splits(shapes, tile):
    target = 1024 if tile == 64 else 512
    tiles = [((M + tile - 1) // tile) * ((N + tile - 1) // tile) for M, N, K in shapes]
    kt = [(K + 31) // 32 for M, N, K in shapes]
    work = sum(t * k for t, k in zip(tiles, kt))
    per_block = max(8.0, work / float(target))
    out = []
    for k in kt:
        s = int(max(1, min(round(k / per_block), k // 8 if k >= 16 else 1, 64)))
        if s >= 8:
            s = s // 8 * 8
        out.append(s)
    return out


def gemm_group(descs, shapes, tile):
    n = len(descs)
    assert 1 <= n <= lib.GEMM_GROUP_MAX
    arr = (lib.GemmDesc * n)(*descs)
    if GemmProfiler.enabled:
        e0, e1 = torch.cuda.Event(enable_timing=True), torch.cuda.Event(enable_timing=True)
        st = _stream()
        ext = torch.cuda.ExternalStream(st.value) if _side[0] is not None else None
        e0.record(ext)
        lib.call("cape_gemm_group_f32", arr, n, tile, st)
        e1.record(ext)
        fl = sum(2.0 * M * N * K for M, N, K, _, _ in shapes)
        by = sum(GemmProfiler.alg_bytes(M, N, K) for M, N, K, _, _ in shapes)
        GemmProfiler.records.append((e0, e1, fl, ("group", tile, shapes[0][4], n), by, n))
        return
    lib.call("cape_gemm_group_f32", arr, n, tile, _stream())


def colsum(X, M, N, out, ldx=None, accumulate=True, nbatch=1, batch_stride=0):
    _chk(X, "colsum.X", contiguous=False)
    _chk(out, "colsum.out", contiguous=False)
    ldx = N if ldx is None else ldx
    assert M == 0 or _avail(X) >= (nbatch - 1) * batch_stride + (M - 1) * ldx + N
    assert _avail(out) >= N
    lib.call("cape_colsum_f32", _p(X), ldx, nbatch, batch_stride, M, N, _p(out), int(accumulate), _stream())


def add_layernorm_fwd(x, y, gamma, beta, pos=None, dropout_p=0.0, rng=None, rng_stream=0):
    C = x.shape[-1]
    rows = x.numel() // C
    for t, n in ((x, "x"), (y, "y"), (gamma, "gamma"), (beta, "beta"), (pos, "pos")):
        _chk(t, "ln." + n)
    if y is not None:
        assert y.shape == x.shape
    if pos is not None:
        assert pos.numel() == x.numel()
    out = torch.empty_like(x)
    mean = torch.empty(rows, dtype=_F32, device=x.device)
    rstd = torch.empty(rows, dtype=_F32, device=x.device)
    out_pos = torch.empty_like(x) if pos is not None else None
    lib.call("cape_add_layernorm_fwd", _p(x), _p(y), _p(gamma), _p(beta), _p(out), _p(mean), _p(rstd), _p(pos),
             _p(out_pos), rows, C, float(dropout_p), rng.ptr if (rng is not None and dropout_p > 0) else None,
             rng_stream, _stream())
    return out, mean, rstd, out_pos


def add_layernorm_bwd(d_out, d_out_pos, x, y, gamma, mean, rstd, dgamma, dbeta, dropout_p=0.0, rng=None, rng_stream=0):
    C = x.shape[-1]
    rows = x.numel() // C
    for t, n in ((d_out, "d_out"), (d_out_pos, "d_out_pos"), (x, "x"), (y, "y"), (dgamma, "dgamma"), (dbeta, "dbeta")):
        _chk(t, "ln_bwd." + n)
    d_x = torch.empty_like(x)
    d_y = torch.empty_like(x) if (y is not None and dropout_p > 0) else None
    lib.call("cape_add_layernorm_bwd", _p(d_out), _p(d_out_pos), _p(x), _p(y), _p(gamma), _p(mean), _p(rstd), _p(d_x),
             _p(d_y), _p(dgamma), _p(dbeta), rows, C, float(dropout_p),
             rng.ptr if (rng is not None and dropout_p > 0) else None, rng_stream, _stream())
    return d_x, (d_y if d_y is not None else d_x)


def _gn_workspace(N, C, G, device):
    nbytes = lib.raw().cape_groupnorm_workspace_bytes(N, C, G)
    return torch.empty((nbytes + 7) // 8, dtype=torch.float64, device=device), nbytes


def groupnorm_fwd(x, gamma, beta, out, out_image_stride, N, HW, C, G=32):
    for t, n in ((x, "x"), (gamma, "gamma"), (beta, "beta")):
        _chk(t, "gn." + n)
    _chk(out, "gn.out", contiguous=False)
    assert x.numel() == N * HW * C
    mean = torch.empty(N * G, dtype=_F32, device=x.device)
    rstd = torch.empty(N * G, dtype=_F32, device=x.device)
    ws, nbytes = _gn_workspace(N, C, G, x.device)
    lib.call("cape_groupnorm_fwd", _p(x), _p(gamma), _p(beta), _p(out), out_image_stride, _p(mean), _p(rstd), N, HW, C, G,
             _p(ws), nbytes, _stream())
    return mean, rstd


def groupnorm_bwd(d_out, d_out_image_stride, x, gamma, mean, rstd, dgamma, dbeta, N, HW, C, G=32):
    _chk(d_out, "gn_bwd.d_out", contiguous=False)
    d_x = torch.empty_like(x)
    ws, nbytes = _gn_workspace(N, C, G, x.device)
    lib.call("cape_groupnorm_bwd", _p(d_out), d_out_image_stride, _p(x), _p(gamma), _p(mean), _p(rstd), _p(d_x),
             _p(dgamma), _p(dbeta), N, HW, C, G, _p(ws), nbytes, _stream())
    return d_x


class LevelGeometry:

    def __init__(self, shapes):
        self.shapes = [(int(h), int(w)) for h, w in shapes]
        self.L = len(self.shapes)
        starts, s = [], 0
        for h, w in self.shapes:
            starts.append(s)
            s += h * w
        self.S = s
        self.starts = starts
        self._shapes_c = (ctypes.c_int * (2 * self.L))(*[v for hw in self.shapes for v in hw])
        self._starts_c = (ctypes.c_int * self.L)(*starts)


def msda_fwd(value, offw, ref, geo, N, Lq, P=4):
    for t, n in ((value, "value"), (offw, "offw"), (ref, "ref")):
        _chk(t, "msda." + n)
    assert value.numel() == N * geo.S * 256 and offw.numel() == N * Lq * 8 * geo.L * P * 3
    assert ref.numel() == N * Lq * geo.L * 2
    out = torch.empty(N, Lq, 256, dtype=_F32, device=value.device)
    lib.call("cape_msda_fwd", _p(value), _p(offw), _p(ref), geo._shapes_c, geo._starts_c, _p(out), N, geo.S, Lq, geo.L, P,
             _stream())
    return out


MSDA_VALUE_ACCUM = os.environ.get("CAPE_MSDA_VALUE_ACCUM", "auto")


def msda_bwd(d_out, value, offw, ref, geo, N, Lq, P=4, need_ref_grad=True, form="split"):
    _chk(d_out, "msda_bwd.d_out")
    d_value = torch.empty_like(value)
    d_offw = torch.empty_like(offw)
    d_ref = torch.empty_like(ref) if need_ref_grad else None
    if form == "split":
        form = MSDA_VALUE_ACCUM if MSDA_VALUE_ACCUM != "auto" else ("f64" if GEMM_PRECISION == 0 else "fx")
    if form == "atomic":
        lib.call("cape_msda_bwd_atomic", _p(d_out), _p(value), _p(offw), _p(ref), geo._shapes_c, geo._starts_c, _p(d_value),
                 _p(d_offw), _p(d_ref), N, geo.S, Lq, geo.L, P, _stream())
    else:
        lib.call("cape_msda_bwd_ex", _p(d_out), _p(value), _p(offw), _p(ref), geo._shapes_c, geo._starts_c, _p(d_value),
                 _p(d_offw), _p(d_ref), N, geo.S, Lq, geo.L, P, {"f64": 0, "fx": 1}[form], _stream())
    return d_value, d_offw, d_ref


def _ld(t):
    assert t.stride(-1) == 1
    return t.stride(-2)


def _attn_views(tag, Q, K, V, N, H, Lq, Lk, flash):
    for t, n, L_ in ((Q, "Q", Lq), (K, "K", Lk), (V, "V", Lk)):
        _chk(t, tag + "." + n, contiguous=False)
        assert t.dim() == 3 and t.shape[0] == N and t.shape[1] >= L_ and t.shape[2] == H * 32
        if flash:
            assert t.stride(2) == 1 and t.stride(1) % 4 == 0 and t.stride(0) % 4 == 0 and t.data_ptr() % 16 == 0
        assert _avail(t) >= (N - 1) * t.stride(0) + (L_ - 1) * t.stride(1) + H * 32


def _rng_ptr(rng, dropout_p):
    return rng.ptr if (rng is not None and dropout_p > 0) else None


def _attn_tail(Q, K, V, N, H, Lq, Lk, scale, mask_mode, causal_offset, kpm, dropout_p, rng, rng_stream):
    return (_ld(Q), _ld(K), _ld(V), H * 32, Q.stride(0), K.stride(0), V.stride(0), Lq * H * 32, N, H, Lq, Lk, float(scale), mask_mode,
            causal_offset, _p(kpm), float(dropout_p), _rng_ptr(rng, dropout_p), rng_stream, _stream())


def _attn_fwd(flash, Q, K, V, N, H, Lq, Lk, scale, mask_mode, causal_offset, kpm, dropout_p, rng, rng_stream):
    tag = "flash_attn" if flash else "attn"
    _attn_views(tag, Q, K, V, N, H, Lq, Lk, flash)
    if kpm is not None:
        _chk(kpm, tag + ".kpm", dtype=torch.uint8)
        assert kpm.numel() == N * Lk
    O = torch.empty(N, Lq, H * 32, dtype=_F32, device=Q.device)
    lse = torch.empty(N, H, Lq, dtype=_F32, device=Q.device)
    lib.call("cape_" + tag + "_fwd", _p(Q), _p(K), _p(V), _p(O), _p(lse),
             *_attn_tail(Q, K, V, N, H, Lq, Lk, scale, mask_mode, causal_offset, kpm, dropout_p, rng, rng_stream))
    return O, lse


def _attn_bwd(flash, dO, Q, K, V, O, lse, dQ, dK, dV, N, H, Lq, Lk, scale, mask_mode, causal_offset, kpm, dropout_p, rng, rng_stream):
    tag = "flash_attn_bwd" if flash else "attn_bwd"
    _chk(dO, tag + ".dO")
    for t in (dQ, dK, dV):
        _chk(t, tag + ".grad", contiguous=False)
    assert _ld(dQ) == _ld(Q) and _ld(dK) == _ld(K) and _ld(dV) == _ld(V)
    assert dQ.stride(0) == Q.stride(0) and dK.stride(0) == K.stride(0) and dV.stride(0) == V.stride(0)
    assert O.is_contiguous() and dO.shape == O.shape
    ws = None
    if flash:
        _attn_views("flash_attn", Q, K, V, N, H, Lq, Lk, True)
        _attn_views("flash_attn", dQ, dK, dV, N, H, Lq, Lk, True)
        _chk(O, tag + ".O"); _chk(lse, tag + ".lse")
        assert O.shape == (N, Lq, H * 32) and lse.numel() == N * H * Lq
        ws = torch.empty(N * H * Lq, dtype=_F32, device=dO.device)
    lib.call("cape_" + tag, _p(dO), _p(Q), _p(K), _p(V), _p(O), _p(lse), _p(dQ), _p(dK), _p(dV), *((_p(ws),) if flash else ()),
             *_attn_tail(Q, K, V, N, H, Lq, Lk, scale, mask_mode, causal_offset, kpm, dropout_p, rng, rng_stream))


def attn_fwd(Q, K, V, N, H, Lq, Lk, scale, mask_mode=0, causal_offset=0, kpm=None, dropout_p=0.0, rng=None, rng_stream=0):
    return _attn_fwd(False, Q, K, V, N, H, Lq, Lk, scale, mask_mode, causal_offset, kpm, dropout_p, rng, rng_stream)


def attn_bwd(dO, Q, K, V, O, lse, dQ, dK, dV, N, H, Lq, Lk, scale, mask_mode=0, causal_offset=0, kpm=None, dropout_p=0.0,
             rng=None, rng_stream=0):
    _attn_bwd(False, dO, Q, K, V, O, lse, dQ, dK, dV, N, H, Lq, Lk, scale, mask_mode, causal_offset, kpm, dropout_p, rng, rng_stream)


FLASH_MAX_L = 224


def flash_attn_ok(N, H, Lq, Lk):
    return (os.environ.get("CAPE_FLASH_ATTN", "1") == "1" and GEMM_PRECISION == 1 and 32 <= Lq <= FLASH_MAX_L and 32 <= Lk <= FLASH_MAX_L
            and N <= 65535 and H <= 65535)


def flash_attn_fwd(Q, K, V, N, H, Lq, Lk, scale, mask_mode=0, causal_offset=0, kpm=None, dropout_p=0.0, rng=None, rng_stream=0):
    return _attn_fwd(True, Q, K, V, N, H, Lq, Lk, scale, mask_mode, causal_offset, kpm, dropout_p, rng, rng_stream)


def flash_attn_bwd(dO, Q, K, V, O, lse, dQ, dK, dV, N, H, Lq, Lk, scale, mask_mode=0, causal_offset=0, kpm=None, dropout_p=0.0,
                   rng=None, rng_stream=0):
    _attn_bwd(True, dO, Q, K, V, O, lse, dQ, dK, dV, N, H, Lq, Lk, scale, mask_mode, causal_offset, kpm, dropout_p, rng, rng_stream)


def attn_mm_ok(N, H, Lq, Lk):
    return (os.environ.get("CAPE_ATTN_MM", "1") == "1" and Lq >= 64 and Lk >= 64 and Lq % 4 == 0 and Lk % 4 == 0 and N * H <= 65535)


def attn_mm_fwd(Q, K, V, N, H, Lq, Lk, scale, mask_mode=0, causal_offset=0, kpm=None, dropout_p=0.0, rng=None, rng_stream=0):
    dev = Q.device
    S = torch.empty(N, H, Lq, Lk, dtype=_F32, device=dev)
    gemm(Q, K, S, Lq, Lk, 32, lda=_ld(Q), ldb=_ld(K), ldc=Lk,
         batch=(N * H, H, Q.stride(0), 32, K.stride(0), 32, H * Lq * Lk, Lq * Lk))
    P = torch.empty_like(S)
    Pd = torch.empty_like(S) if dropout_p > 0 else None
    lib.call("cape_attn_softmax_fwd", _p(S), _p(P), _p(Pd), N, H, Lq, Lk, float(scale), mask_mode, causal_offset, _p(kpm),
             float(dropout_p), _rng_ptr(rng, dropout_p), rng_stream, _stream())
    Pu = Pd if Pd is not None else P
    O = torch.empty(N, Lq, H * 32, dtype=_F32, device=dev)
    gemm(Pu, V, O, Lq, 32, Lk, a_mode=0, b_mode=1, lda=Lk, ldb=_ld(V), ldc=H * 32,
         batch=(N * H, H, H * Lq * Lk, Lq * Lk, V.stride(0), 32, Lq * H * 32, 32))
    return O, P, Pu


def attn_mm_bwd(dO, Q, K, V, P, Pu, dQ, dK, dV, N, H, Lq, Lk, scale, dropout_p=0.0, rng=None, rng_stream=0):
    blk, img = Lq * Lk, H * Lq * Lk
    gemm(Pu, dO, dV, Lk, 32, Lq, a_mode=1, b_mode=1, lda=Lk, ldb=H * 32, ldc=_ld(dV),
         batch=(N * H, H, img, blk, Lq * H * 32, 32, dV.stride(0), 32))
    dS = torch.empty(N, H, Lq, Lk, dtype=_F32, device=dO.device)
    gemm(dO, V, dS, Lq, Lk, 32, lda=H * 32, ldb=_ld(V), ldc=Lk,
         batch=(N * H, H, Lq * H * 32, 32, V.stride(0), 32, img, blk))
    lib.call("cape_attn_softmax_bwd", _p(P), _p(dS), N, H, Lq, Lk, float(scale), float(dropout_p),
             _rng_ptr(rng, dropout_p), rng_stream, _stream())
    gemm(dS, K, dQ, Lq, 32, Lk, a_mode=0, b_mode=1, lda=Lk, ldb=_ld(K), ldc=_ld(dQ),
         batch=(N * H, H, img, blk, K.stride(0), 32, dQ.stride(0), 32))
    gemm(dS, Q, dK, Lk, 32, Lq, a_mode=1, b_mode=1, lda=Lk, ldb=_ld(Q), ldc=_ld(dK),
         batch=(N * H, H, img, blk, Q.stride(0), 32, dK.stride(0), 32))


def attn_route(N, H, Lq, Lk, flash=False):
    if flash and flash_attn_ok(N, H, Lq, Lk):
        return "flash"
    return "mm" if attn_mm_ok(N, H, Lq, Lk) else "scalar"


_ATTN_LAUNCHERS = {"scalar": (attn_fwd, attn_bwd), "flash": (flash_attn_fwd, flash_attn_bwd)}


def attn_core_fwd(route, Q, K, V, N, H, Lq, Lk, scale, mask_mode=0, causal_offset=0, kpm=None, dropout_p=0.0, rng=None, rng_stream=0):
    if route == "mm":
        O, P, Pu = attn_mm_fwd(Q, K, V, N, H, Lq, Lk, scale, mask_mode, causal_offset, kpm, dropout_p, rng, rng_stream)
        return O, (P, Pu)
    O, lse = _ATTN_LAUNCHERS[route][0](Q, K, V, N, H, Lq, Lk, scale, mask_mode, causal_offset, kpm, dropout_p, rng, rng_stream)
    return O, (lse,)


def attn_core_bwd(route, saved, dO, Q, K, V, O, dQ, dK, dV, N, H, Lq, Lk, scale, mask_mode=0, causal_offset=0, kpm=None, dropout_p=0.0,
                  rng=None, rng_stream=0):
    if route == "mm":
        attn_mm_bwd(dO, Q, K, V, *saved, dQ, dK, dV, N, H, Lq, Lk, scale, dropout_p, rng, rng_stream)
    else:
        _ATTN_LAUNCHERS[route][1](dO, Q, K, V, O, *saved, dQ, dK, dV, N, H, Lq, Lk, scale, mask_mode, causal_offset, kpm, dropout_p,
                                  rng, rng_stream)


def add(a, b):
    _chk(a, "add.a"); _chk(b, "add.b")
    assert a.shape == b.shape
    out = torch.empty_like(a)
    lib.call("cape_add_f32", _p(a), _p(b), _p(out), a.numel(), _stream())
    return out


def add_n(tensors):
    k = len(tensors)
    assert 1 <= k <= 8
    for t in tensors:
        _chk(t, "add_n.src")
        assert t.shape == tensors[0].shape
    if k == 1:
        return tensors[0]
    out = torch.empty_like(tensors[0])
    arr = (ctypes.c_void_p * k)(*[t.data_ptr() for t in tensors])
    lib.call("cape_add_n_f32", arr, k, _p(out), out.numel(), _stream())
    return out


def augment_batch(items_dev_u8, n, max_pixels, out_size, mean=None, std=None):
    _chk(items_dev_u8, "augment.items", dtype=torch.uint8)
    assert items_dev_u8.numel() >= n * ctypes.sizeof(lib.AugItem)
    if mean is not None:
        _chk(mean, "augment.mean"); _chk(std, "augment.std")
        assert mean.numel() == 3 and std.numel() == 3
    lib.call("cape_augment_batch", _p(items_dev_u8), n, int(max_pixels), int(out_size), _p(mean), _p(std), _stream())


def _row_ld(t, rows, cols):
    if t.is_contiguous():
        return cols
    st, sh = t.stride(), t.shape
    assert t.stride(-1) == 1 and all(st[i] == st[i + 1] * sh[i + 1] for i in range(len(sh) - 2)), "add_n_rows: leading dims do not collapse"
    return st[-2]


def add_n_rows(tensors, out=None):
    k = len(tensors)
    assert 1 <= k <= 8
    shape = tensors[0].shape
    cols = shape[-1]
    rows = tensors[0].numel() // cols
    lds = []
    for t in tensors:
        _chk(t, "add_n_rows.src", contiguous=False)
        assert t.shape == shape and t.stride(-1) == 1 and cols % 4 == 0
        v = t.reshape(rows, cols) if t.is_contiguous() else t
        if not t.is_contiguous():
            st, sh = t.stride(), t.shape
            assert all(st[i] == st[i + 1] * sh[i + 1] for i in range(len(sh) - 2)), "add_n_rows: leading dims do not collapse"
            lds.append(st[-2])
        else:
            lds.append(cols)
        assert _avail(t) >= (rows - 1) * lds[-1] + cols
    if out is None:
        out = torch.empty(shape, dtype=_F32, device=tensors[0].device)
    _chk(out, "add_n_rows.out", contiguous=False)
    assert out.shape == shape
    ldo = _row_ld(out, rows, cols)
    assert _avail(out) >= (rows - 1) * ldo + cols
    arr = (ctypes.c_void_p * k)(*[t.data_ptr() for t in tensors])
    ld = (ctypes.c_longlong * k)(*lds)
    lib.call("cape_add_n_rows_f32", arr, ld, k, _p(out), ldo, rows, cols, _stream())
    return out


def gelu(x):
    _chk(x, "gelu.x")
    out = torch.empty_like(x)
    lib.call("cape_gelu_f32", _p(x), _p(out), x.numel(), _stream())
    return out


def interleave2x2(classes, acc, out):
    _chk(out, "interleave2x2.out"); _chk(acc, "interleave2x2.acc")
    N, H, W, C = out.shape
    assert len(classes) == 4 and H % 2 == 0 and W % 2 == 0 and C % 4 == 0 and (acc is None or acc.shape == out.shape)
    for c in classes:
        _chk(c, "interleave2x2.class")
        assert c is None or c.numel() == N * (H // 2) * (W // 2) * C
    arr = (ctypes.c_void_p * 4)(*[c.data_ptr() if c is not None else None for c in classes])
    lib.call("cape_interleave2x2_f32", arr, _p(acc), _p(out), N, H, W, C, _stream())
    return out


def gelu_bwd(x, g):
    _chk(x, "gelu_bwd.x"); _chk(g, "gelu_bwd.g")
    assert x.shape == g.shape
    dx = torch.empty_like(x)
    lib.call("cape_gelu_bwd_f32", _p(x), _p(g), _p(dx), x.numel(), _stream())
    return dx


def scale_residual_bwd(g, y, gamma, dgamma):
    _chk(g, "scale_residual_bwd.g"); _chk(y, "scale_residual_bwd.y"); _chk(gamma, "scale_residual_bwd.gamma")
    _chk(dgamma, "scale_residual_bwd.dgamma", contiguous=False)
    C = y.shape[-1]
    assert g.shape == y.shape and gamma.numel() == C and _avail(dgamma) >= C
    dy = torch.empty_like(y)
    lib.call("cape_scale_residual_bwd_f32", _p(g), _p(y), _p(gamma), _p(dy), _p(dgamma), y.numel() // C, C, _stream())
    return dy


def scale_residual(x, y, gamma=None):
    _chk(x, "scale_residual.x"); _chk(y, "scale_residual.y"); _chk(gamma, "scale_residual.gamma")
    assert x.shape == y.shape and (gamma is None or gamma.numel() == x.shape[-1])
    out = torch.empty_like(x)
    C = x.shape[-1]
    lib.call("cape_scale_residual_f32", _p(x), _p(y), _p(gamma), _p(out), x.numel() // C, C, _stream())
    return out


def nchw_to_nhwc(x, Cp):
    _chk(x, "nchw_to_nhwc.x")
    N, C, H, W = x.shape
    out = torch.empty(N, H, W, Cp, dtype=_F32, device=x.device)
    lib.call("cape_nchw_to_nhwc", _p(x), _p(out), N, C, H, W, Cp, _stream())
    return out


def bn_fold(w, b, rm, rv, eps=1e-5):
    for t in (w, b, rm, rv):
        _chk(t, "bn_fold")
    scale, shift = torch.empty_like(w), torch.empty_like(w)
    lib.call("cape_bn_fold", _p(w), _p(b), _p(rm), _p(rv), float(eps), _p(scale), _p(shift), w.numel(), _stream())
    return scale, shift


def maxpool3x3s2(x):
    _chk(x, "maxpool.x")
    N, H, W, C = x.shape
    OH, OW = (H - 1) // 2 + 1, (W - 1) // 2 + 1
    out = torch.empty(N, OH, OW, C, dtype=_F32, device=x.device)
    lib.call("cape_maxpool3x3s2_nhwc", _p(x), _p(out), N, H, W, C, _stream())
    return out


def bn_relu_bwd(dy, y, scale, relu, want_res):
    _chk(dy, "bn_relu_bwd.dy"); _chk(y, "bn_relu_bwd.y"); _chk(scale, "bn_relu_bwd.scale")
    C = dy.shape[-1]
    rows = dy.numel() // C
    d_pre = torch.empty_like(dy)
    d_res = torch.empty_like(dy) if want_res else None
    lib.call("cape_bn_relu_bwd", _p(dy), _p(y), _p(scale), _p(d_pre), _p(d_res), rows, C, int(relu), _stream())
    return d_pre, d_res


def affine_act_(x, scale, bias, residual, relu):
    _chk(x, "affine_act.x"); _chk(scale, "affine_act.scale"); _chk(bias, "affine_act.bias"); _chk(residual, "affine_act.residual")
    C = x.shape[-1]
    assert (scale is None or scale.numel() == C) and (bias is None or bias.numel() == C) and (residual is None or residual.shape == x.shape)
    lib.call("cape_affine_act_f32", _p(x), _p(scale), _p(bias), _p(residual), x.numel() // C, C, int(relu), _stream())
    return x


# ... 495 lines not shown
```

### category-agnostic-pose-estimation_amd/models/deformable_transformer_v2.py

```python
import copy
import math
import os

import numpy as np
import torch
from torch import nn
from torch.nn.init import normal_

from ..hip import functional as HF
from ..hip import ops
from .deformable_transformer import (DeformableTransformerEncoder, DeformableTransformerEncoderLayer, MSDeformAttn)
from ..util.misc import cached_zero_mask
from .kv_cache import KVCache, VCache

_ONES_VR = {}
_FUSED_SELF_ATTN = os.environ.get("CAPE_DEC_SELF_ATTN_NODE", "1") == "1"


def Embedding(num_embeddings, embedding_dim, padding_idx=None, zero_init=False):
    m = nn.Embedding(num_embeddings, embedding_dim, padding_idx=padding_idx)
    nn.init.normal_(m.weight, mean=0, std=embedding_dim ** -0.5)
    if padding_idx is not None:
        nn.init.constant_(m.weight[padding_idx], 0)
    if zero_init:
        nn.init.constant_(m.weight, 0)
    return m


def get_1d_sincos_pos_embed_from_grid(embed_dim, seq_len):
    pos = np.arange(seq_len, dtype=np.float32)
    omega = 1.0 / 10000 ** (np.arange(embed_dim // 2, dtype=np.float64) / (embed_dim / 2.0))
    out = np.einsum("m,d->md", pos.reshape(-1), omega)
    return np.concatenate([np.sin(out), np.cos(out)], axis=1)


class TransformerDecoderLayer(nn.Module):

    def __init__(self, d_model=256, d_ffn=1024, dropout=0.1, activation="relu", n_levels=4, n_heads=8, n_points=4,
                 use_qkv_proj=True):
        super().__init__()
        if activation != "relu" or not use_qkv_proj:
            raise ValueError("CAPE path: relu FFN and dec_qkv_proj=True (reference defaults)")
        self.d_model, self.n_heads = d_model, n_heads
        self.attn_q = nn.Linear(d_model, d_model, bias=False)
        self.attn_k = nn.Linear(d_model, d_model, bias=False)
        self.attn_v = nn.Linear(d_model, d_model, bias=False)
        self.self_attn = nn.MultiheadAttention(d_model, n_heads, dropout=dropout)
        self.dropout2 = nn.Dropout(dropout)
        self.norm2 = nn.LayerNorm(d_model)
        self.support_attn = nn.MultiheadAttention(d_model, n_heads, dropout=dropout, batch_first=True)
        self.dropout_support = nn.Dropout(dropout)
        self.norm_support = nn.LayerNorm(d_model)
        self.cross_attn = MSDeformAttn(d_model, n_levels, n_heads, n_points)
        self.dropout1 = nn.Dropout(dropout)
        self.norm1 = nn.LayerNorm(d_model)
        self.linear1 = nn.Linear(d_model, d_ffn)
        self.dropout3 = nn.Dropout(dropout)
        self.linear2 = nn.Linear(d_ffn, d_model)
        self.dropout4 = nn.Dropout(dropout)
        self.norm3 = nn.LayerNorm(d_model)
        self.kv_cache = None
        self._streams = [ops.new_stream_id() for _ in range(8)]

    def forward(self, tgt, query_pos, reference_points, src, geo, padding_rows_u8=None, support_features=None,
                support_kpm_u8=None):
        p = self.dropout2.p if self.training else 0.0
        st = self._streams
        sa = self.self_attn
        qp_q, qp_s = HF.fanout(query_pos, 2)
        if _FUSED_SELF_ATTN:
            t_a, t_r = HF.fanout(tgt, 2)
            t2 = HF.dec_self_attn(t_a, qp_q, self.attn_q.weight, self.attn_k.weight, self.attn_v.weight, sa.in_proj_weight,
                                  sa.in_proj_bias, sa.out_proj.weight, sa.out_proj.bias, self.n_heads, dropout_p=p, rng_stream=st[0])
        else:
            t_q, t_k, t_v, t_r = HF.fanout(tgt, 4)
            q = HF.linear(t_q, self.attn_q.weight, residual=qp_q)
            k = HF.linear(t_k, self.attn_k.weight)
            v = HF.linear(t_v, self.attn_v.weight)
            t2 = HF.mha(q, k, v, sa.in_proj_weight, sa.in_proj_bias, sa.out_proj.weight, sa.out_proj.bias, self.n_heads,
                        mask_mode=1, dropout_p=p, rng_stream=st[0])
        tgt = HF.add_layernorm(t_r, t2, self.norm2.weight, self.norm2.bias, dropout_p=p, rng_stream=st[1])
        if support_features is not None:
            ca = self.support_attn
            t_q, t_r = HF.fanout(tgt, 2)
            t2 = HF.mha(t_q, support_features, support_features, ca.in_proj_weight, ca.in_proj_bias, ca.out_proj.weight,
                        ca.out_proj.bias, self.n_heads, mask_mode=2 if support_kpm_u8 is not None else 0,
                        kpm_u8=support_kpm_u8, dropout_p=p, rng_stream=st[2])
            tgt, tgt_pos = HF.add_layernorm(t_r, t2, self.norm_support.weight, self.norm_support.bias, pos=qp_s,
                                            dropout_p=p, rng_stream=st[3])
        else:
            tgt, t_r = HF.fanout(tgt, 2)
            tgt_pos = HF.add(t_r, qp_s)
        t2 = self.cross_attn(tgt_pos, reference_points, src, geo, padding_rows_u8)
        tgt = HF.add_layernorm(tgt, t2, self.norm1.weight, self.norm1.bias, dropout_p=p, rng_stream=st[4])
        t_f, t_r = HF.fanout(tgt, 2)
        h = HF.ffn(t_f, self.linear1.weight, self.linear1.bias, self.linear2.weight, self.linear2.bias, dropout_p=p, rng_stream=st[5])
        return HF.add_layernorm(t_r, h, self.norm3.weight, self.norm3.bias, dropout_p=p, rng_stream=st[6])

    @torch.no_grad()
    def decode_step(self, tgt, query_pos, reference_points, geo, step, cache):
        C, H = self.d_model, self.n_heads
        N = tgt.shape[0]
        sa = self.self_attn
        W, B = sa.in_proj_weight, sa.in_proj_bias
        dev = tgt.device
        t2d = tgt.view(N, C)
        tmp = torch.empty(3, N, C, dtype=torch.float32, device=dev)
        ops.gemm(t2d, self.attn_q.weight, tmp[0], N, C, C, residual=query_pos.view(N, C))
        ops.gemm(t2d, self.attn_k.weight, tmp[1], N, C, C)
        ops.gemm(t2d, self.attn_v.weight, tmp[2], N, C, C)
        q = torch.empty(N, 1, C, dtype=torch.float32, device=dev)
        ops.gemm(tmp[0], W, q, N, C, C, bias=B)
        max_len = cache["k"].shape[1]
        ops.gemm(tmp[1], W[C:], cache["k"][:, step], N, C, C, bias=B[C:], ldc=max_len * C)
        ops.gemm(tmp[2], W[2 * C:], cache["v"][:, step], N, C, C, bias=B[2 * C:], ldc=max_len * C)
        Lk = step + 1
        O, _ = ops.attn_fwd(q, cache["k"], cache["v"], N, H, 1, Lk, (C // H) ** -0.5, mask_mode=0)
        t2 = torch.empty(N, 1, C, dtype=torch.float32, device=dev)
        ops.gemm(O.view(N, C), sa.out_proj.weight, t2, N, C, C, bias=sa.out_proj.bias)
        tgt, _, _, _ = ops.add_layernorm_fwd(tgt, t2, self.norm2.weight, self.norm2.bias)
        tgt_pos = None
        if cache.get("sup_k") is not None:
            ca = self.support_attn
            ops.gemm(tgt.view(N, C), ca.in_proj_weight, q, N, C, C, bias=ca.in_proj_bias)
            P = cache["sup_k"].shape[1]
            O, _ = ops.attn_fwd(q, cache["sup_k"], cache["sup_v"], N, H, 1, P, (C // H) ** -0.5,
                                mask_mode=2 if cache["sup_kpm"] is not None else 0, kpm=cache["sup_kpm"])
            ops.gemm(O.view(N, C), ca.out_proj.weight, t2, N, C, C, bias=ca.out_proj.bias)
            tgt, _, _, tgt_pos = ops.add_layernorm_fwd(tgt, t2, self.norm_support.weight, self.norm_support.bias, pos=query_pos)
        else:
            tgt_pos = ops.add(tgt, query_pos)
        m = self.cross_attn
        LP3 = m.n_heads * m.n_levels * m.n_points
        offw = torch.empty(N, 1, 3 * LP3, dtype=torch.float32, device=dev)
        ops.gemm(tgt_pos.view(N, C), m.sampling_offsets.weight, offw, N, 2 * LP3, C, bias=m.sampling_offsets.bias, ldc=3 * LP3)
        ops.gemm(tgt_pos.view(N, C), m.attention_weights.weight, offw.view(N, -1)[:, 2 * LP3:], N, LP3, C,
                 bias=m.attention_weights.bias, ldc=3 * LP3)
        a = ops.msda_fwd(cache["value"], offw, reference_points, geo, N, 1, m.n_points)
        ops.gemm(a.view(N, C), m.output_proj.weight, t2, N, C, C, bias=m.output_proj.bias)
        tgt, _, _, _ = ops.add_layernorm_fwd(tgt, t2, self.norm1.weight, self.norm1.bias)
        F_ = self.linear1.weight.shape[0]
        h = torch.empty(N, F_, dtype=torch.float32, device=dev)
        ops.gemm(tgt.view(N, C), self.linear1.weight, h, N, F_, C, bias=self.linear1.bias, relu=True)
        ops.gemm(h, self.linear2.weight, t2, N, C, F_, bias=self.linear2.bias)
        tgt, _, _, _ = ops.add_layernorm_fwd(tgt, t2, self.norm3.weight, self.norm3.bias)
        return tgt


class TransformerDecoder(nn.Module):
    def __init__(self, decoder_layer, num_layers, poly_refine=True, return_intermediate=False, aux_loss=False,
                 query_pos_type="none", vocab_size=None, pad_idx=None, use_anchor=None):
        super().__init__()
        if not poly_refine or query_pos_type != "sine" or use_anchor:
            raise ValueError("CAPE path: with_poly_refine=True, query_pos_type='sine', use_anchor=False (reference defaults)")
        self.layers = nn.ModuleList([copy.deepcopy(decoder_layer) for _ in range(num_layers)])
        for layer in self.layers:
            layer._streams = [ops.new_stream_id() for _ in range(8)]
        self.num_layers = num_layers
        self.poly_refine = poly_refine
        self.return_intermediate = return_intermediate
        self.aux_loss = aux_loss
        self.query_pos_type = query_pos_type
        self.coords_embed = None
        self.class_embed = None
        self.pos_trans = None
        self.pos_trans_norm = None
        self.use_anchor = use_anchor
        self.room_class_embed = None
        self.room_class_trans = None
        self.pad_idx = pad_idx
        self.token_embed = Embedding(vocab_size, self.layers[0].d_model, padding_idx=pad_idx, zero_init=False)

    def _seq_embed(self, seq11, seq12, seq21, seq22, delta_x1, delta_x2, delta_y1, delta_y2):
        return HF.token_embed(self.token_embed.weight, self.pad_idx, seq11, seq21, seq12, seq22,
                              delta_x1, delta_x2, delta_y1, delta_y2)

    def _query_pos(self, reference_points):
        qs = HF.query_sine(reference_points)
        qp = HF.linear(qs, self.pos_trans.weight, self.pos_trans.bias)
        return HF.add_layernorm(qp, None, self.pos_trans_norm.weight, self.pos_trans_norm.bias)

    def _mlp(self, mlp, x):
        n = len(mlp.layers)
        for i, layer in enumerate(mlp.layers):
            x = HF.linear(x, layer.weight, layer.bias, relu=(i < n - 1))
        return x

    def forward(self, reference_points, src, geo, src_valid_ratios, padding_rows_u8=None, seq_kwargs=None,
                support_features=None, support_mask=None):
        if support_features is None:
            support_features = getattr(self, "support_features", None)
        if support_mask is None:
            support_mask = getattr(self, "support_mask", None)
        kpm = ops.as_u8(support_mask) if (support_features is not None and support_mask is not None) else None
        output = self._seq_embed(seq11=seq_kwargs["seq11"], seq12=seq_kwargs["seq12"], seq21=seq_kwargs["seq21"],
                                 seq22=seq_kwargs["seq22"], delta_x1=seq_kwargs["delta_x1"], delta_x2=seq_kwargs["delta_x2"],
                                 delta_y1=seq_kwargs["delta_y1"], delta_y2=seq_kwargs["delta_y2"])
        hs, refs, clss = [], [], []
        nl = len(self.layers)
        mems = HF.fanout(src, nl)
        sups = HF.fanout(support_features, nl) if support_features is not None else (None,) * nl
        for lid, layer in enumerate(self.layers):
            r_scale, r_sine, r_ref = HF.fanout(reference_points, 3)
            ref_in = HF.ref_scale(r_scale, src_valid_ratios)
            query_pos = self._query_pos(r_sine)
            output = layer(output, query_pos, ref_in, mems[lid], geo, padding_rows_u8, sups[lid], kpm)
            o_mlp, o_cls, o_hs, output = HF.fanout(output, 4)
            delta = self._mlp(self.coords_embed[lid], o_mlp)
            reference_points, r_keep = HF.fanout(HF.refine(delta, r_ref), 2)
            cls = HF.linear(o_cls, self.class_embed[lid].weight, self.class_embed[lid].bias)
            hs.append(o_hs); refs.append(r_keep); clss.append(cls)
        return hs, torch.stack(refs), torch.stack(clss)

    @torch.no_grad()
    def decode_step(self, tok, delta, ref_step, geo, valid_ratios, step, caches):
        N = tok.shape[1]
        output = ops.token_embed_fwd(self.token_embed.weight, [tok[0], tok[2], tok[1], tok[3]],
                                     [delta[0], delta[1], delta[2], delta[3]]).view(N, 1, -1)
        ref = ref_step
        for lid, layer in enumerate(self.layers):
            ref_in = ops.ref_scale_fwd(ref, valid_ratios, 1, geo.L).view(N, 1, geo.L, 2)
            qs = ops.query_sine_fwd(ref)
            qp = torch.empty(N, 256, dtype=torch.float32, device=ref.device)
            ops.gemm(qs, self.pos_trans.weight, qp, N, 256, 256, bias=self.pos_trans.bias)
            qp, _, _, _ = ops.add_layernorm_fwd(qp, None, self.pos_trans_norm.weight, self.pos_trans_norm.bias)
            output = layer.decode_step(output, qp.view(N, 1, 256), ref_in, geo, step, caches[lid])
            x = output.view(N, 256)
            mlp = self.coords_embed[lid].layers
            for i, l in enumerate(mlp):
                y = torch.empty(N, l.weight.shape[0], dtype=torch.float32, device=x.device)
                ops.gemm(x, l.weight, y, N, l.weight.shape[0], l.weight.shape[1], bias=l.bias, relu=(i < len(mlp) - 1))
                x = y
            ref = ops.refine_fwd(x.view(N, 1, 2), ref)
        ce = self.class_embed[-1]
        cls = torch.empty(N, ce.weight.shape[0], dtype=torch.float32, device=ref.device)
        ops.gemm(output.view(N, 256), ce.weight, cls, N, ce.weight.shape[0], 256, bias=ce.bias)
        return output, ref, cls


class DeformableTransformer(nn.Module):
    def __init__(self, d_model=256, nhead=8, num_encoder_layers=6, num_decoder_layers=6, dim_feedforward=1024, dropout=0.1,
                 activation="relu", poly_refine=True, return_intermediate_dec=False, aux_loss=False, num_feature_levels=4,
                 dec_n_points=4, enc_n_points=4, query_pos_type="none", vocab_size=None, seq_len=1024,
                 pre_decoder_pos_embed=False, learnable_dec_pe=False, dec_attn_concat_src=False, dec_qkv_proj=True,
                 dec_layer_type="v1", pad_idx=None, use_anchor=False, inject_cls_embed=False):
        super().__init__()
        if dec_layer_type != "v1":
            raise TypeError(f"dec_layer_type={dec_layer_type!r}: only the v1 decoder layer accepts support features "
                            "(the other variants raise TypeError in the reference as well)")
        if pre_decoder_pos_embed or dec_attn_concat_src or inject_cls_embed:
            raise ValueError("pre_decoder_pos_embed / dec_attn_concat_src / inject_cls_embed are off on the CAPE path")
        self.d_model, self.nhead = d_model, nhead
        self.poly_refine, self.use_anchor = poly_refine, use_anchor
        self.num_feature_levels = num_feature_levels
        enc_layer = DeformableTransformerEncoderLayer(d_model, dim_feedforward, dropout, activation, num_feature_levels,
                                                      nhead, enc_n_points)
        self.encoder = DeformableTransformerEncoder(enc_layer, num_encoder_layers)
        dec_layer = TransformerDecoderLayer(d_model, dim_feedforward, dropout, activation, num_feature_levels, nhead,
                                            dec_n_points, use_qkv_proj=dec_qkv_proj)
        self.decoder = TransformerDecoder(dec_layer, num_decoder_layers, poly_refine, return_intermediate_dec, aux_loss,
                                          query_pos_type, vocab_size, pad_idx, use_anchor=use_anchor)
        self.level_embed = nn.Parameter(torch.Tensor(num_feature_levels, d_model))
        self.decoder.pos_trans = nn.Linear(d_model, d_model)
        self.decoder.pos_trans_norm = nn.LayerNorm(d_model)
        self.pos_embed = nn.Parameter(torch.zeros(1, seq_len, d_model), requires_grad=learnable_dec_pe)
        self.pos_embed.data.copy_(torch.from_numpy(get_1d_sincos_pos_embed_from_grid(d_model, seq_len)).float().unsqueeze(0))
        self._reset_parameters()

    def _reset_parameters(self):
        for p in self.parameters():
            if p.dim() > 1:
                nn.init.xavier_uniform_(p)
        for m in self.modules():
            if isinstance(m, MSDeformAttn):
                m._reset_parameters()
        normal_(self.level_embed)

    @staticmethod
    def valid_ratio(mask):
        _, H, W = mask.shape
        vh = torch.sum(~mask[:, :, 0], 1).float() / H
        vw = torch.sum(~mask[:, 0, :], 1).float() / W
        return torch.stack([vw, vh], -1)

    def encode(self, srcs_nhwc, gn_params, masks, has_padding):
        geo = ops.LevelGeometry([(s.shape[1], s.shape[2]) for s in srcs_nhwc])
        src_flatten = HF.level_groupnorm(geo, srcs_nhwc, gn_params[0], gn_params[1])
        if has_padding:
            masks_u8 = [m.to(torch.uint8).contiguous() for m in masks]
            with torch.no_grad():
                valid_ratios = torch.stack([self.valid_ratio(m) for m in masks], 1).contiguous()
                pad_rows = torch.cat([m.flatten(1) for m in masks_u8], 1).contiguous()
        else:
            N = srcs_nhwc[0].shape[0]
            masks_u8 = [cached_zero_mask(N, s.shape[1], s.shape[2], s.device, torch.uint8) for s in srcs_nhwc]
            key = (N, len(masks), str(srcs_nhwc[0].device))
            valid_ratios = _ONES_VR.get(key)
            if valid_ratios is None:
                valid_ratios = _ONES_VR[key] = torch.ones(N, len(masks), 2, dtype=torch.float32, device=srcs_nhwc[0].device)
            pad_rows = None
        pos = HF.level_pos(geo, self.level_embed, masks_u8)
        memory = self.encoder(src_flatten, geo, valid_ratios, pos, pad_rows)
        return {"memory": memory, "geo": geo, "valid_ratios": valid_ratios, "pad_rows": pad_rows, "src_flatten": src_flatten}

    def forward(self, enc, query_embed, seq_kwargs, support_features=None, support_mask=None):
        bs = enc["memory"].shape[0]
        L = seq_kwargs["seq11"].shape[1]
        ref_all = HF.sigmoid(query_embed)
        reference_points = ref_all[:L].unsqueeze(0).expand(bs, -1, -1).contiguous()
        hs, refs, clss = self.decoder(reference_points, enc["memory"], enc["geo"], enc["valid_ratios"], enc["pad_rows"],
                                      seq_kwargs, support_features, support_mask)
        return hs, reference_points, refs, clss

    def _setup_caches(self, max_batch_size, max_seq_length, max_vision_length, model_dim, nhead, dtype, device):
        for layer in self.decoder.layers:
            layer.kv_cache = KVCache(max_batch_size, max_seq_length, model_dim, dtype).to(device)
            layer.cross_attn.cache = VCache(max_batch_size, max_vision_length, nhead, int(model_dim // nhead), dtype).to(device)


def build_deforamble_transformer(args, pad_idx=None):
    return DeformableTransformer(
        d_model=args.hidden_dim, nhead=args.nheads, num_encoder_layers=args.enc_layers,
        num_decoder_layers=args.dec_layers, dim_feedforward=args.dim_feedforward, dropout=args.dropout,
        activation="relu", poly_refine=args.with_poly_refine, return_intermediate_dec=True, aux_loss=args.aux_loss,
        num_feature_levels=args.num_feature_levels, dec_n_points=args.dec_n_points, enc_n_points=args.enc_n_points,
        query_pos_type=args.query_pos_type, vocab_size=args.vocab_size, seq_len=args.seq_len,
        pre_decoder_pos_embed=args.pre_decoder_pos_embed, learnable_dec_pe=args.learnable_dec_pe,
        dec_attn_concat_src=args.dec_attn_concat_src, dec_qkv_proj=args.dec_qkv_proj, dec_layer_type=args.dec_layer_type,
        pad_idx=pad_idx, use_anchor=args.use_anchor, inject_cls_embed=getattr(args, "inject_cls_embed", False))
```

### category-agnostic-pose-estimation_amd/runtime/arena.py

```python
import torch

DEAD_PREFIXES = ("support_cross_attention_layers.", "support_attn_layer_norms.", "base_model.room_class_embed.")


def _align(n, a=64):
    return (n + a - 1) // a * a


class ParamGroupArena:
    def __init__(self, named_params, device):
        self.names = [n for n, _ in named_params]
        self.params = [p for _, p in named_params]
        self.offsets = []
        off = 0
        for p in self.params:
            self.offsets.append(off)
            off += _align(p.numel())
        self.numel = off
        self.data = torch.zeros(off, dtype=torch.float32, device=device)
        self.grad = torch.zeros(off, dtype=torch.float32, device=device)
        self.exp_avg = torch.zeros(off, dtype=torch.float32, device=device)
        self.exp_avg_sq = torch.zeros(off, dtype=torch.float32, device=device)
        for p, o in zip(self.params, self.offsets):
            assert p.dtype == torch.float32 and p.device == self.data.device
            self._rebind(p, o)

    def _view(self, slab, p, o):
        return torch.as_strided(slab, p.shape, p.stride(), storage_offset=o)

    def _rebind(self, p, o):
        dense = p.numel() == 0 or _is_dense(p)
        assert dense, "parameters must be dense (contiguous up to a permutation)"
        v = self._view(self.data, p, o)
        with torch.no_grad():
            v.copy_(p.data)
        p.data = v
        p.grad = self._view(self.grad, p, o)

    def zero_grad(self):
        self.grad.zero_()

    def grad_view(self, i):
        return self._view(self.grad, self.params[i], self.offsets[i])


def _is_dense(t):
    sizes_strides = sorted(((st, sz) for sz, st in zip(t.shape, t.stride()) if sz > 1), key=lambda x: x[0])
    expect = 1
    for st, sz in sizes_strides:
        if st != expect:
            return False
        expect *= sz
    return True


def split_groups(model):
    main, backbone, dead = [], [], []
    seen = set()
    for n, p in model.named_parameters():
        if not p.requires_grad or id(p) in seen:
            continue
        seen.add(id(p))
        if n.startswith(DEAD_PREFIXES):
            dead.append((n, p))
        elif "backbone" in n:
            backbone.append((n, p))
        else:
            main.append((n, p))
    return _colocate(main), backbone, dead


def _colocate(named):
    out = list(named)
    for i in range(len(out) - 2):
        a, b, c = out[i][0], out[i + 1][0], out[i + 2][0]
        if a.endswith("sampling_offsets.weight") and b.endswith("sampling_offsets.bias") and c.endswith("attention_weights.weight") \
                and a[:-len("sampling_offsets.weight")] == c[:-len("attention_weights.weight")]:
            out[i + 1], out[i + 2] = out[i + 2], out[i + 1]
    return out
```

### include/cape_hip.h

```cpp
#ifndef CAPE_HIP_H
#define CAPE_HIP_H

#include <stddef.h>
#include <stdint.h>

#ifdef __cplusplus
extern "C" {
#endif

typedef void* cape_stream_t;

const char* cape_last_error(void);
int cape_abi_version(void);

int cape_rng_advance(uint64_t* rng_state, cape_stream_t stream);

int cape_stream_fork(cape_stream_t main_stream, cape_stream_t side_stream);
int cape_stream_join(cape_stream_t main_stream, cape_stream_t side_stream);

typedef struct {
  int M, N, K;
  int a_mode, b_mode;
  const float* A; long long lda;
  const float* B; long long ldb;
  float* C; long long ldc;
  int cN, cH, cW, cC, cKH, cKW, cStride, cPad, cOH, cOW, cO;
  const float* scale;
  const float* bias;
  const float* residual;
  long long ldr;
  int relu;
  int accumulate;
  int split_k;
  float dropout_p;
  const uint64_t* rng_state;
  uint32_t rng_stream;
  float* colsum_out;
  int precision;
  const uint16_t* B_packed;
  const float* mask_src; long long ldm; float mask_scale;
  int batch, batch_div; long long sA0, sA1, sB0, sB1, sC0, sC1;
  int res_cols; long long sBias0, sBias1;
  int cPadX, cKHp, cKWp, cTapH0, cTapHS, cTapW0, cTapWS;
  int cDil;
} cape_gemm_desc;

int cape_gemm_f32(const cape_gemm_desc* d, cape_stream_t stream);

#define CAPE_GEMM_GROUP_MAX 32
int cape_gemm_group_f32(const cape_gemm_desc* descs, int n, int tile, cape_stream_t stream);

typedef struct { const float* B; uint16_t* out; long long ldb; int N, K, b_mode, pad; } cape_pack_item;
size_t cape_packed_weight_bytes(int N, int K);
int cape_pack_weights(const cape_pack_item* items_dev, int n_items, int max_blocks_per_item, cape_stream_t stream);

int cape_colsum_f32(const float* X, long long ldx, int nbatch, long long batch_stride, int M, int N, float* out,
                    int accumulate, cape_stream_t stream);

typedef struct {
  int N, K, Nout;
  const float* X; long long ldx; const float* in_gamma; const float* in_beta; const float* in_add; long long ld_add;
  const float* W; long long ldw; const float* bias;
  const float* X2; long long ldx2; int K2; const float* W2; long long ldw2; int n2;
  const float* R; long long ldr; const float* res_gamma; const float* res_beta;
  int relu;
  int nseg, seg; float* out[3]; long long ldo[3];
} cape_decode_linear_desc;
int cape_decode_linear(const cape_decode_linear_desc* d, cape_stream_t stream);

typedef struct {
  int N, L;
  const float* P4; long long ldp; const float* g3; const float* b3;
  const float* W1; const float* B1; const float* W2; const float* B2; const float* W3; const float* B3;
  const float* ref;
  const float* Wc; const float* Bc; int ncls;
  const float* Wp; const float* Bp; const float* gp; const float* bp;
  const float* dim_t; const float* vr;
  float* ref_out; long long ld_ref;
  float* qpos_out; float* refin_out;
  float* cls_out; long long ld_cls;
  float* hs_out; long long ld_hs;
} cape_decode_tail_desc;
int cape_decode_tail(const cape_decode_tail_desc* d, cape_stream_t stream);

#define CAPE_DECODE_MAX_LAYERS 8
typedef struct {
  const float *w_qkv, *b_qkv;
  const float* w_qin;
  float *k_cache, *v_cache;
  const float *w_o, *b_o, *ln2_g, *ln2_b;
  const float *w_sq, *b_sq;
  const float *sup_k, *sup_v;
  const unsigned char* sup_mask;
  const float *w_so, *b_so, *lns_g, *lns_b;
  const float *w_off, *b_off;
  const float* value;
  const float *w_mo, *b_mo, *ln1_g, *ln1_b;
  const float *w1, *b1, *w2, *b2;
  const float *ln3_g, *ln3_b;
  const float *m1w, *m1b, *m2w, *m2b, *m3w, *m3b;
} cape_decode_layer_desc;
typedef struct {
  int N, n_layers, step, T, P, S, L, n_points, ncls, ffn_dim;
  int shapes[8];
  int level_start[4];
  const float* emb;
  const float* qpos0;
  const float* refin0;
  const float* ref0;
  const float* vr;
  const float* dim_t;
  const float *class_w, *class_b;
  const float *pos_w, *pos_b, *pos_gamma, *pos_beta;
  float* out_logits; long long ld_logits;
  float* out_coords; long long ld_coords;
  float* out_hs; long long ld_hs;
  cape_decode_layer_desc layers[CAPE_DECODE_MAX_LAYERS];
} cape_decode_step_desc;
int cape_decode_step(const cape_decode_step_desc* d, cape_stream_t stream);

int cape_add_layernorm_fwd(const float* x, const float* y, const float* gamma, const float* beta,
                           float* out, float* mean, float* rstd, const float* pos, float* out_pos,
                           int rows, int C, float dropout_p, const uint64_t* rng_state, uint32_t rng_stream,
                           cape_stream_t stream);
int cape_add_layernorm_bwd(const float* d_out, const float* d_out_pos, const float* x, const float* y,
                           const float* gamma, const float* mean, const float* rstd,
                           float* d_x, float* d_y, float* dgamma, float* dbeta,
                           int rows, int C, float dropout_p, const uint64_t* rng_state, uint32_t rng_stream,
                           cape_stream_t stream);

size_t cape_groupnorm_workspace_bytes(int N, int C, int G);
int cape_groupnorm_fwd(const float* x, const float* gamma, const float* beta, float* out,
                       long long out_image_stride, float* mean, float* rstd,
                       int N, int HW, int C, int G, void* workspace, size_t workspace_bytes, cape_stream_t stream);
int cape_groupnorm_bwd(const float* d_out, long long d_out_image_stride, const float* x,
                       const float* gamma, const float* mean, const float* rstd,
                       float* d_x, float* dgamma, float* dbeta, int N, int HW, int C, int G,
                       void* workspace, size_t workspace_bytes, cape_stream_t stream);

int cape_msda_fwd(const float* value, const float* offw, const float* ref, const int* shapes,
                  const int* level_start, float* out, int N, int S, int Lq, int L, int P,
                  cape_stream_t stream);
int cape_msda_bwd(const float* d_out, const float* value, const float* offw, const float* ref,
                  const int* shapes, const int* level_start, float* d_value, float* d_offw, float* d_ref,
                  int N, int S, int Lq, int L, int P, cape_stream_t stream);
int cape_msda_bwd_ex(const float* d_out, const float* value, const float* offw, const float* ref,
                     const int* shapes, const int* level_start, float* d_value, float* d_offw, float* d_ref,
                     int N, int S, int Lq, int L, int P, int value_accum, cape_stream_t stream);
int cape_msda_bwd_atomic(const float* d_out, const float* value, const float* offw, const float* ref,
                         const int* shapes, const int* level_start, float* d_value, float* d_offw, float* d_ref,
                         int N, int S, int Lq, int L, int P, cape_stream_t stream);

int cape_attn_fwd(const float* Q, const float* K, const float* V, float* O, float* lse,
                  long long ldq, long long ldk, long long ldv, long long ldo,
                  long long bsq, long long bsk, long long bsv, long long bso,
                  int N, int H, int Lq, int Lk, float scale, int mask_mode, int causal_offset,
                  const uint8_t* kpm, float dropout_p, const uint64_t* rng_state, uint32_t rng_stream,
                  cape_stream_t stream);
int cape_attn_bwd(const float* dO, const float* Q, const float* K, const float* V, const float* O,
                  const float* lse, float* dQ, float* dK, float* dV,
                  long long ldq, long long ldk, long long ldv, long long ldo,
                  long long bsq, long long bsk, long long bsv, long long bso,
                  int N, int H, int Lq, int Lk, float scale, int mask_mode, int causal_offset,
                  const uint8_t* kpm, float dropout_p, const uint64_t* rng_state, uint32_t rng_stream,
                  cape_stream_t stream);
int cape_attn_softmax_fwd(const float* S, float* P, float* Pd, int N, int H, int Lq, int Lk, float scale, int mask_mode,
                          int causal_offset, const uint8_t* kpm, float dropout_p, const uint64_t* rng_state,
                          uint32_t rng_stream, cape_stream_t stream);
int cape_attn_softmax_bwd(const float* P, float* dS, int N, int H, int Lq, int Lk, float scale, float dropout_p,
                          const uint64_t* rng_state, uint32_t rng_stream, cape_stream_t stream);

int cape_flash_attn_fwd(const float* Q, const float* K, const float* V, float* O, float* lse, long long ldq, long long ldk,
                        long long ldv, long long ldo, long long bsq, long long bsk, long long bsv, long long bso, int N, int H,
                        int Lq, int Lk, float scale, int mask_mode, int causal_offset, const uint8_t* kpm, float dropout_p,
                        const uint64_t* rng_state, uint32_t rng_stream, cape_stream_t stream);
int cape_flash_attn_bwd(const float* dO, const float* Q, const float* K, const float* V, const float* O, const float* lse,
                        float* dQ, float* dK, float* dV, float* d_ws, long long ldq, long long ldk, long long ldv, long long ldo,
                        long long bsq, long long bsk, long long bsv, long long bso, int N, int H, int Lq, int Lk, float scale,
                        int mask_mode, int causal_offset, const uint8_t* kpm, float dropout_p, const uint64_t* rng_state,
                        uint32_t rng_stream, cape_stream_t stream);


int cape_add_f32(const float* a, const float* b, float* out, long long n, cape_stream_t stream);
int cape_level_embed_add(const float* base, const float* level_embed, const int* level_start, float* out, int N, int S, int L, int C,
                         cape_stream_t stream);
int cape_add_n_f32(const float* const* srcs, int k, float* out, long long n, cape_stream_t stream);
int cape_interleave2x2_f32(const float* const* cls, const float* acc, float* out, int N, int H, int W, int C, cape_stream_t stream);
int cape_add_n_rows_f32(const float* const* srcs, const long long* lds, int k, float* out, long long ldo, long long rows, int cols,
                        cape_stream_t stream);
int cape_gelu_f32(const float* x, float* out, long long n, cape_stream_t stream);
int cape_scale_residual_f32(const float* x, const float* y, const float* gamma, float* out, long long rows, int C,
                            cape_stream_t stream);
int cape_gelu_bwd_f32(const float* x, const float* g, float* dx, long long n, cape_stream_t stream);
int cape_scale_residual_bwd_f32(const float* g, const float* y, const float* gamma, float* dy, float* dgamma, long long rows, int C,
                                cape_stream_t stream);
int cape_nchw_to_nhwc(const float* x, float* out, int N, int C, int H, int W, int Cp, cape_stream_t stream);
int cape_bn_fold(const float* w, const float* b, const float* rm, const float* rv, float eps,
                 float* scale, float* shift, int C, cape_stream_t stream);
int cape_maxpool3x3s2_nhwc(const float* x, float* out, int N, int H, int W, int C, cape_stream_t stream);
int cape_bn_relu_bwd(const float* dy, const float* y, const float* scale, float* d_pre, float* d_res,
                     long long rows, int C, int relu, cape_stream_t stream);
int cape_affine_act_f32(float* x, const float* scale, const float* bias, const float* residual, long long rows, int C, int relu,
                        cape_stream_t stream);
int cape_relu_drop_bwd(const float* dh, const float* h, float* d_pre, long long n, float inv_keep,
                       cape_stream_t stream);
int cape_pos_sine_level(const uint8_t* mask, const float* level_embed_l, const float* dim_t, float* out,
                        long long out_image_stride, int N, int h, int w, int C, cape_stream_t stream);

int cape_token_embed_fwd(const float* table, const int64_t* s11, const int64_t* s21, const int64_t* s12,
                         const int64_t* s22, const float* dx1, const float* dx2, const float* dy1,
                         const float* dy2, float* out, long long R, int C, int vocab, cape_stream_t stream);
int cape_token_embed_bwd(const float* d_out, const int64_t* s11, const int64_t* s21, const int64_t* s12,
                         const int64_t* s22, const float* dx1, const float* dx2, const float* dy1,
                         const float* dy2, float* d_table, long long R, int C, int vocab, int pad_idx,
                         cape_stream_t stream);

int cape_query_sine_fwd(const float* ref, const float* dim_t, float* out, long long R, cape_stream_t stream);
int cape_query_sine_bwd(const float* d_out, const float* ref, const float* dim_t, float* d_ref, int accumulate, long long R,
                        cape_stream_t stream);

int cape_refine_fwd(const float* delta, const float* ref, float* new_ref, long long n, cape_stream_t stream);
int cape_refine_bwd(const float* d_new, const float* new_ref, const float* ref, float* d_delta,
                    float* d_ref, int accumulate_ref, long long n, cape_stream_t stream);
int cape_sigmoid_fwd(const float* x, float* y, long long n, cape_stream_t stream);
int cape_sigmoid_bwd(const float* dy, const float* y, float* dx, int accumulate, long long n,
                     cape_stream_t stream);
int cape_ref_scale_fwd(const float* ref, const float* valid_ratios, float* ref_in, long long R,
                       int rows_per_image, int L, cape_stream_t stream);
int cape_ref_scale_bwd(const float* d_ref_in, const float* valid_ratios, float* d_ref, int accumulate,
                       long long R, int rows_per_image, int L, cape_stream_t stream);

int cape_support_embed_fwd(const float* coords, const float* W0, const float* b0, const float* pe1d,
                           const float* dim_t, float* h, float* pe, int N, int P, int C, cape_stream_t stream);
int cape_support_embed_bwd(const float* d_h, const float* h, const float* coords, float* dW0, float* db0,
                           int N, int P, int C, cape_stream_t stream);
int cape_adjacency(const int* edges, const int* edge_start, const uint8_t* mask, float* adj, int N, int P,
                   cape_stream_t stream);
int cape_support_masks(const uint8_t* mask, uint8_t* kpm, uint8_t* zero, int N, int P, int pad_rows, cape_stream_t stream);
int cape_gcn_aggregate_fwd(const float* y, const float* adj, float* out, int N, int P, int C,
                           cape_stream_t stream);
int cape_gcn_aggregate_bwd(const float* d_out, const float* out, const float* adj, float* d_y, int N,
                           int P, int C, cape_stream_t stream);
int cape_zero_rows(float* x, const uint8_t* rowmask, long long rows, int C, cape_stream_t stream);

int cape_legacy_coord_embed_fwd(const float* coords, const float* W0, const float* b0, float* h, int R, int C, cape_stream_t stream);
int cape_legacy_coord_embed_bwd(const float* d_h, const float* h, const float* coords, const float* W0, float* dW0, float* db0,
                                float* d_coords, int R, int C, cape_stream_t stream);
int cape_support_edge_info_fwd(const int* edges, const int* edge_start, const float* E, float* out, long long ldo, float* scale,
                               uint8_t* has, float* deg, int N, int P, int C, cape_stream_t stream);
int cape_support_edge_info_bwd(const float* g, long long ldg, const float* scale, const uint8_t* has, float* dE, int R, int C,
                               cape_stream_t stream);
int cape_pe_dropout_fwd(const float* x, const float* pe, float* out, int R, int P, int C, float dropout_p, const uint64_t* rng_state,
                        uint32_t rng_stream, cape_stream_t stream);
int cape_pe_dropout_bwd(const float* g, float* dx, long long total, float dropout_p, const uint64_t* rng_state, uint32_t rng_stream,
                        cape_stream_t stream);

int cape_loss_fwd_bwd(const float* logits, const float* coords, const int64_t* labels, const uint8_t* vis,
                      const float* target, const float* class_w, float w_ce, float w_l1, float loss_scale,
                      float* losses, float* total, float* d_logits, float* d_coords, int NL, long long R,
                      cape_stream_t stream);

#define CAPE_SUMSQ_PARTS 256
int cape_sumsq(const float* g, long long n, float* out_parts, cape_stream_t stream);
int cape_adamw_step(float* p, const float* g, float* m, float* v, long long n, float lr, float beta1,
                    float beta2, float eps, float weight_decay, float max_norm, const float* sumsq_parts, int n_parts,
                    const int64_t* step_count, const float* lr_dev ,
                    cape_stream_t stream);
int cape_step_increment(int64_t* step_count, cape_stream_t stream);

#define CAPE_GUARD_ROW_SERIAL 0
#define CAPE_GUARD_ROW_OK 1
#define CAPE_GUARD_ROW_TOTAL 2
#define CAPE_GUARD_ROW_NORM 3
#define CAPE_GUARD_ROW_COEF 4
#define CAPE_GUARD_ROW_LR 5
#define CAPE_GUARD_ROW_LOSSES 6
#define CAPE_GUARD_NO_STEP (-1.0f)
int cape_step_guard(const float* total, const float* losses, int n_losses, const float* sumsq_parts, int n_parts,
                    float max_norm, const float* lr_dev, int64_t* step_count, int* serial, int* bad, float* ring,
                    int ring_len, int row_stride, cape_stream_t stream);
int cape_adamw_step_guarded(float* p, const float* g, float* m, float* v, long long n, float lr, float beta1,
                            float beta2, float eps, float weight_decay, float max_norm, const float* sumsq_parts, int n_parts,
                            const int64_t* step_count, const float* lr_dev, const int* bad, cape_stream_t stream);

int cape_decode_advance(const float* cls_logits, long long ld_cls, const float* reg, long long ld_reg, int32_t* unfinished,
                        int64_t* tok, float* delta, int step, int N, int num_bins, int min_len, int eos_id, int sep_id, int pad_id,
                        const float* table, int vocab, int C, float* embed_out, int32_t* alive_out, cape_stream_t stream);
int cape_decode_next_tokens(const float* cls_logits, const float* reg, int32_t* unfinished,
                            int64_t* tok , float* delta ,
                            const int32_t* step , int N, int num_bins, int min_len,
                            int eos_id, int sep_id, int pad_id, cape_stream_t stream);

typedef struct {
  const uint8_t* src; float* aug; float* out; float* stat;
  int h, w;
  float M[6];
  int color_on, order[4];
  float bright, contrast, sat, hue;
  int mode;
  float noise_std; uint32_t seed;
  int blur_k; float blur_w[49];
} cape_augment_item;
int cape_augment_batch(const cape_augment_item* items_dev, int n_items, int max_pixels, int out_size, const float* mean,
                       const float* stdv, cape_stream_t stream);

#ifdef __cplusplus
}
#endif
#endif
```

Baseline: 653.9 episodes/s.

## Hoist decoder value projections into one batched GEMM with strided MSDA access

Concatenates the per-layer decoder cross-attention value_proj weights so that all layers' value projections are computed by one wide GEMM over the shared memory src. The MSDA forward and backward kernels gain a leading-dimension parameter, so each layer can read its slice of the wide value tensor and write its d_value slice in place without copies. Parameters are re-ordered in the arena so the stacked weights and biases sit contiguously. This is meant to cut per-layer GEMM launches and the src fanout, at the cost of strided gathers that may cache less well and a larger live value buffer.

After: 657.6 episodes/s, median of 2. About the same (+0.6%).

```diff
diff --git a/category-agnostic-pose-estimation_amd/csrc/msda.hip b/category-agnostic-pose-estimation_amd/csrc/msda.hip
--- a/category-agnostic-pose-estimation_amd/csrc/msda.hip
+++ b/category-agnostic-pose-estimation_amd/csrc/msda.hip
@@ -11,9 +11,11 @@
 
 __device__ __forceinline__ int sel4(const int (&a)[4], int l) { return l == 0 ? a[0] : (l == 1 ? a[1] : (l == 2 ? a[2] : a[3])); }
 
+template <bool DENSE>
 __global__ void __launch_bounds__(256) msda_fwd_kernel(const float* __restrict__ value, const float* __restrict__ offw,
                                                         const float* __restrict__ ref, float* __restrict__ out,
-                                                        Levels lv, int N, int S, int Lq, int L, int P, int blocks_per_image) {
+                                                        Levels lv, int N, int S, int Lq, int L, int P, int blocks_per_image, int ldv) {
+  const long long LDV = DENSE ? CH : ldv;
   const int lane = threadIdx.x & 63, wv = threadIdx.x >> 6;
   int n, chunk;
   {
@@ -60,7 +62,7 @@
   const float aw[2] = {e0 * inv, e1 * inv};
 
   float4 acc = make_float4(0.f, 0.f, 0.f, 0.f);
-  const float* vbase = value + (long long)n * S * CH + h * HD + c4 * 4;
+  const float* vbase = value + (long long)n * S * LDV + h * HD + c4 * 4;
 #pragma unroll
   for (int s = 0; s < 2; ++s) {
 #pragma unroll
@@ -74,17 +76,17 @@
       const float xf = floorf(x), yf = floorf(y);
       const float fx = x - xf, fy = y - yf;
       const int x0 = (int)xf, y0 = (int)yf;
-      const float* vl = vbase + (long long)sel4(lv.start, l) * CH;
+      const float* vl = vbase + (long long)sel4(lv.start, l) * LDV;
       const bool xa = x0 >= 0 && x0 < W, xb = x0 + 1 >= 0 && x0 + 1 < W;
       const bool ya = y0 >= 0 && y0 < H, yb = y0 + 1 >= 0 && y0 + 1 < H;
       float4 v;
-      if (ya && xa) { v = *reinterpret_cast<const float4*>(vl + (long long)(y0 * W + x0) * CH); const float w = a * (1.f - fx) * (1.f - fy);
+      if (ya && xa) { v = *reinterpret_cast<const float4*>(vl + (long long)(y0 * W + x0) * LDV); const float w = a * (1.f - fx) * (1.f - fy);
         acc.x += w * v.x; acc.y += w * v.y; acc.z += w * v.z; acc.w += w * v.w; }
-      if (ya && xb) { v = *reinterpret_cast<const float4*>(vl + (long long)(y0 * W + x0 + 1) * CH); const float w = a * fx * (1.f - fy);
+      if (ya && xb) { v = *reinterpret_cast<const float4*>(vl + (long long)(y0 * W + x0 + 1) * LDV); const float w = a * fx * (1.f - fy);
         acc.x += w * v.x; acc.y += w * v.y; acc.z += w * v.z; acc.w += w * v.w; }
-      if (yb && xa) { v = *reinterpret_cast<const float4*>(vl + (long long)((y0 + 1) * W + x0) * CH); const float w = a * (1.f - fx) * fy;
+      if (yb && xa) { v = *reinterpret_cast<const float4*>(vl + (long long)((y0 + 1) * W + x0) * LDV); const float w = a * (1.f - fx) * fy;
         acc.x += w * v.x; acc.y += w * v.y; acc.z += w * v.z; acc.w += w * v.w; }
-      if (yb && xb) { v = *reinterpret_cast<const float4*>(vl + (long long)((y0 + 1) * W + x0 + 1) * CH); const float w = a * fx * fy;
+      if (yb && xb) { v = *reinterpret_cast<const float4*>(vl + (long long)((y0 + 1) * W + x0 + 1) * LDV); const float w = a * fx * fy;
         acc.x += w * v.x; acc.y += w * v.y; acc.z += w * v.z; acc.w += w * v.w; }
     }
   }
@@ -97,11 +99,13 @@
   return v;
 }
 
+template <bool DENSE>
 __global__ void __launch_bounds__(256) msda_bwd_kernel(const float* __restrict__ d_out, const float* __restrict__ value,
                                                         const float* __restrict__ offw, const float* __restrict__ ref,
                                                         float* __restrict__ d_value, float* __restrict__ d_offw,
                                                         float* __restrict__ d_ref, Levels lv, int N, int S, int Lq, int L,
-                                                        int P, long long total_waves) {
+                                                        int P, long long total_waves, int ldv, int ldd) {
+  const long long LDV = DENSE ? CH : ldv, LDD = DENSE ? CH : ldd;
   const int lane = threadIdx.x & 63, wv = threadIdx.x >> 6;
   const long long wid = (long long)blockIdx.x * 4 + wv;
   if (wid >= total_waves) return;
@@ -134,8 +138,8 @@
   const float aw = e / sm;
 
   const float go = d_out[qrow * CH + h * HD + c];
-  const float* vbase = value + (long long)n * S * CH + h * HD + c;
-  float* dvbase = d_value + (long long)n * S * CH + h * HD + c;
+  const float* vbase = value + (long long)n * S * LDV + h * HD + c;
+  float* dvbase = d_value + (long long)n * S * LDD + h * HD + c;
   float my_daw = 0.f, my_dpx = 0.f, my_dpy = 0.f;
   for (int jj = 0; jj < LP; ++jj) {
     const int src = (lane & 32) | jj;
@@ -145,15 +149,15 @@
     const float xf = floorf(x), yf = floorf(y);
     const float fx = x - xf, fy = y - yf;
     const int x0 = (int)xf, y0 = (int)yf;
-    const long long lofs = (long long)sel4(lv.start, l) * CH;
+    const long long lpix = sel4(lv.start, l);
     const bool xa = x0 >= 0 && x0 < W, xb = x0 + 1 >= 0 && x0 + 1 < W;
     const bool ya = y0 >= 0 && y0 < H, yb = y0 + 1 >= 0 && y0 + 1 < H;
     float v00 = 0.f, v01 = 0.f, v10 = 0.f, v11 = 0.f;
     const float ga = go * a;
-    if (ya && xa) { const long long o = lofs + (long long)(y0 * W + x0) * CH; v00 = vbase[o]; atomicAdd(dvbase + o, ga * (1.f - fx) * (1.f - fy)); }
-    if (ya && xb) { const long long o = lofs + (long long)(y0 * W + x0 + 1) * CH; v01 = vbase[o]; atomicAdd(dvbase + o, ga * fx * (1.f - fy)); }
-    if (yb && xa) { const long long o = lofs + (long long)((y0 + 1) * W + x0) * CH; v10 = vbase[o]; atomicAdd(dvbase + o, ga * (1.f - fx) * fy); }
-    if (yb && xb) { const long long o = lofs + (long long)((y0 + 1) * W + x0 + 1) * CH; v11 = vbase[o]; atomicAdd(dvbase + o, ga * fx * fy); }
+    if (ya && xa) { const long long o = lpix + (long long)(y0 * W + x0); v00 = vbase[o * LDV]; atomicAdd(dvbase + o * LDD, ga * (1.f - fx) * (1.f - fy)); }
+    if (ya && xb) { const long long o = lpix + (long long)(y0 * W + x0 + 1); v01 = vbase[o * LDV]; atomicAdd(dvbase + o * LDD, ga * fx * (1.f - fy)); }
+    if (yb && xa) { const long long o = lpix + (long long)((y0 + 1) * W + x0); v10 = vbase[o * LDV]; atomicAdd(dvbase + o * LDD, ga * (1.f - fx) * fy); }
+    if (yb && xb) { const long long o = lpix + (long long)((y0 + 1) * W + x0 + 1); v11 = vbase[o * LDV]; atomicAdd(dvbase + o * LDD, ga * fx * fy); }
     const float samp = (1.f - fy) * ((1.f - fx) * v00 + fx * v01) + fy * ((1.f - fx) * v10 + fx * v11);
     const float dsx = (1.f - fy) * (v01 - v00) + fy * (v11 - v10);
     const float dsy = (1.f - fx) * (v10 - v00) + fx * (v11 - v01);
@@ -218,9 +222,11 @@
   return t;
 }
 
+template <bool DENSE>
 __global__ void __launch_bounds__(256) msda_fwd_rec_kernel(const float* __restrict__ value, const float* __restrict__ offw,
                                                             const float* __restrict__ ref, float* __restrict__ out, Levels lv,
-                                                            int N, int S, int Lq, int L, int P, int blocks_per_image) {
+                                                            int N, int S, int Lq, int L, int P, int blocks_per_image, int ldv) {
+  const unsigned LDV = DENSE ? (unsigned)CH : (unsigned)ldv;
   __shared__ uint2 rec_ids[4][HEADS * 16];
   __shared__ float4 rec_w[4][HEADS * 16];
   const int lane = threadIdx.x & 63, wv = threadIdx.x >> 6;
@@ -274,17 +280,17 @@
     rec_ids[wv][h * 16 + j] = make_uint2(min(t.i00, cl) | (min(t.i01, cl) << 16), min(t.i10, cl) | (min(t.i11, cl) << 16));
     rec_w[wv][h * 16 + j] = w;
   }
-  const float* vb = value + (long long)n * S * CH + h * HD + i * 4;
+  const float* vb = value + (long long)n * S * LDV + h * HD + i * 4;
   const uint2* rid = &rec_ids[wv][h * 16];
   const float4* rw = &rec_w[wv][h * 16];
   constexpr int PF = 4;
   float4 v[PF + 1][4];
   auto fetch = [&](int j, int slot) {
     const uint2 ids = rid[j];
-    v[slot][0] = *reinterpret_cast<const float4*>(vb + (ids.x & 0xFFFFu) * (unsigned)CH);
-    v[slot][1] = *reinterpret_cast<const float4*>(vb + (ids.x >> 16) * (unsigned)CH);
-    v[slot][2] = *reinterpret_cast<const float4*>(vb + (ids.y & 0xFFFFu) * (unsigned)CH);
-    v[slot][3] = *reinterpret_cast<const float4*>(vb + (ids.y >> 16) * (unsigned)CH);
+    v[slot][0] = *reinterpret_cast<const float4*>(vb + (ids.x & 0xFFFFu) * LDV);
+    v[slot][1] = *reinterpret_cast<const float4*>(vb + (ids.x >> 16) * LDV);
+    v[slot][2] = *reinterpret_cast<const float4*>(vb + (ids.y & 0xFFFFu) * LDV);
+    v[slot][3] = *reinterpret_cast<const float4*>(vb + (ids.y >> 16) * LDV);
   };
 #pragma unroll
   for (int j = 0; j < PF; ++j)
@@ -304,10 +310,12 @@
   *reinterpret_cast<float4*>(out + qrow * CH + h * HD + i * 4) = acc;
 }
 
+template <bool DENSE>
 __global__ void __launch_bounds__(256) msda_bwd_offw_kernel(const float* __restrict__ d_out, const float* __restrict__ value,
                                                              const float* __restrict__ offw, const float* __restrict__ ref,
                                                              float* __restrict__ d_offw, float* __restrict__ d_ref, Levels lv,
-                                                             int N, int S, int Lq, int L, int P, int blocks_per_image) {
+                                                             int N, int S, int Lq, int L, int P, int blocks_per_image, int ldv) {
+  const unsigned LDV = DENSE ? (unsigned)CH : (unsigned)ldv;
   __shared__ uint4 recs[4][HEADS * 16];
   const int lane = threadIdx.x & 63, wv = threadIdx.x >> 6;
   int n, chunk;
@@ -356,7 +364,7 @@
     aw[0] = e0 * inv; aw[1] = e1 * inv;
   }
   const float4 go = *reinterpret_cast<const float4*>(d_out + qrow * CH + h * HD + i * 4);
-  const float* vb = value + (long long)n * S * CH + h * HD + i * 4;
+  const float* vb = value + (long long)n * S * LDV + h * HD + i * 4;
   float daw[2] = {0.f, 0.f}, dpx[2] = {0.f, 0.f}, dpy[2] = {0.f, 0.f};
   const uint4* myrec = &recs[wv][h * 16];
   constexpr int PF = 2;
@@ -368,7 +376,7 @@
 #pragma unroll
     for (int k = 0; k < 4; ++k) {
       const unsigned idc = min(ids[k], (unsigned)(S - 1));
-      const float4 x = *reinterpret_cast<const float4*>(vb + idc * (unsigned)CH);
+      const float4 x = *reinterpret_cast<const float4*>(vb + idc * LDV);
       v[slot][k] = ids[k] < (unsigned)S ? x : make_float4(0.f, 0.f, 0.f, 0.f);
     }
   };
@@ -426,10 +434,11 @@
 
 struct ValRec { uint2 ids; float4 w; };
 
-template <int VC>
+template <int VC, bool DENSE>
 __global__ void __launch_bounds__(1024) msda_bwd_value_kernel(const float* __restrict__ d_out, const float* __restrict__ offw,
                                                               const float* __restrict__ ref, float* __restrict__ d_value,
-                                                              Levels lv, int N, int S, int Lq, int L, int P) {
+                                                              Levels lv, int N, int S, int Lq, int L, int P, int ldd) {
+  const long long LDD = DENSE ? CH : ldd;
   constexpr int VS = VC, GROUPS = HD / VC, BPI = HEADS * GROUPS;
   constexpr int SLOTS = 64 / VC;
   extern __shared__ __attribute__((aligned(16))) double slab[];
@@ -504,26 +513,27 @@
     cur = nxt;
   }
   __syncthreads();
-  float* dvb = d_value + (long long)n * S * CH + h * HD + grp * VC;
+  float* dvb = d_value + (long long)n * S * LDD + h * HD + grp * VC;
   if constexpr (VC >= 4) {
     constexpr int Q = VC / 4;
     for (int k = threadIdx.x; k < S * Q; k += 1024) {
       const int p_ = k / Q, c4 = (k % Q) * 4;
       const double* sp = &slab[p_ * VS + c4];
-      *reinterpret_cast<float4*>(dvb + (long long)p_ * CH + c4) = make_float4((float)sp[0], (float)sp[1], (float)sp[2], (float)sp[3]);
+      *reinterpret_cast<float4*>(dvb + (long long)p_ * LDD + c4) = make_float4((float)sp[0], (float)sp[1], (float)sp[2], (float)sp[3]);
     }
   } else {
     for (int k = threadIdx.x; k < S; k += 1024)
-      *reinterpret_cast<float2*>(dvb + (long long)k * CH) = make_float2((float)slab[k * VS], (float)slab[k * VS + 1]);
+      *reinterpret_cast<float2*>(dvb + (long long)k * LDD) = make_float2((float)slab[k * VS], (float)slab[k * VS + 1]);
   }
 }
 
 typedef float v2f __attribute__((ext_vector_type(2)));
 
-template <int VP>
+template <int VP, bool DENSE>
 __global__ void __launch_bounds__(1024) msda_bwd_value_fx_kernel(const float* __restrict__ d_out, const float* __restrict__ offw,
                                                                  const float* __restrict__ ref, float* __restrict__ d_value,
-                                                                 Levels lv, int N, int S, int Lq, int L, int P) {
+                                                                 Levels lv, int N, int S, int Lq, int L, int P, int ldd) {
+  const long long LDD = DENSE ? CH : ldd;
   constexpr int VC = 2 * VP, GROUPS = HD / VC, BPI = HEADS * GROUPS;
   constexpr int SLOTS = 64 / VP;
   extern __shared__ __attribute__((aligned(16))) unsigned long long fslab[];
@@ -631,7 +641,7 @@
     cur = nxt;
   }
   __syncthreads();
-  float* dvb = d_value + (long long)n * S * CH + ch0;
+  float* dvb = d_value + (long long)n * S * LDD + ch0;
   const float nanv = __uint_as_float(0x7fc00000u);
   auto dec = [&](unsigned long long wd, float& lo, float& hi) {
     const int l = (int)(unsigned)wd;
@@ -645,7 +655,7 @@
     float4 o;
     dec(fslab[p_ * VP + c2], o.x, o.y);
     dec(fslab[p_ * VP + c2 + 1], o.z, o.w);
-    *reinterpret_cast<float4*>(dvb + (long long)p_ * CH + c2 * 2) = o;
+    *reinterpret_cast<float4*>(dvb + (long long)p_ * LDD + c2 * 2) = o;
   }
 }
 
@@ -667,11 +677,28 @@
 
 }
 
+static int msda_ld_check(const char* who, const char* what, int ld, int S, bool offsets32) {
+  CAPE_REQUIRE(ld >= CH, "%s: %s=%d must be >= %d", who, what, ld, CH);
+  CAPE_REQUIRE(ld % 4 == 0, "%s: %s=%d must be a multiple of 4 (16-byte accesses)", who, what, ld);
+  CAPE_REQUIRE(!offsets32 || (long long)(S - 1) * ld + CH < (1ll << 32), "%s: (S-1)*%s + %d = %lld does not fit 32 bits", who, what,
+               CH, (long long)(S - 1) * ld + CH);
+  return 0;
+}
+
 extern "C" int cape_msda_fwd(const float* value, const float* offw, const float* ref, const int* shapes,
                              const int* level_start, float* out, int N, int S, int Lq, int L, int P,
                              cape_stream_t stream) {
+  return cape_msda_fwd_ld(value, offw, ref, shapes, level_start, out, N, S, Lq, L, P, CH, stream);
+}
+
+extern "C" int cape_msda_fwd_ld(const float* value, const float* offw, const float* ref, const int* shapes,
+                                const int* level_start, float* out, int N, int S, int Lq, int L, int P, int ldv,
+                                cape_stream_t stream) {
   CAPE_REQUIRE(value && offw && ref && shapes && level_start && out, "cape_msda_fwd: null pointer");
   CAPE_REQUIRE(P >= 1 && L * P <= 16, "cape_msda_fwd: L*P=%d must be <= 16", L * P);
+  static const bool shuffle_form = getenv("CAPE_MSDA_FWD_SHUFFLE") != nullptr;
+  const bool rec = S < 65535 && !shuffle_form;
+  if (msda_ld_check("cape_msda_fwd", "ldv", ldv, S, rec)) return 1;
   if (N <= 0 || Lq <= 0) return 0;
   Levels lv;
   if (fill_levels(lv, shapes, level_start, L, S)) return 1;
@@ -679,13 +706,15 @@
   const int imgs_per_x = (N + 7) / 8;
   const long long blocks = (long long)imgs_per_x * bpi * 8;
   CAPE_REQUIRE(blocks < (1ll << 31), "cape_msda_fwd: grid too large");
-  static const bool shuffle_form = getenv("CAPE_MSDA_FWD_SHUFFLE") != nullptr;
-  if (S < 65535 && !shuffle_form)
-    hipLaunchKernelGGL(msda_fwd_rec_kernel, dim3((unsigned)blocks), dim3(256), 0, as_stream(stream), value, offw, ref, out, lv,
-                       N, S, Lq, L, P, bpi);
-  else
-    hipLaunchKernelGGL(msda_fwd_kernel, dim3((unsigned)blocks), dim3(256), 0, as_stream(stream), value, offw, ref, out, lv,
-                       N, S, Lq, L, P, bpi);
+#define FWD_LAUNCH(KERNEL, DENSE)                                                                                              \
+  hipLaunchKernelGGL((KERNEL<DENSE>), dim3((unsigned)blocks), dim3(256), 0, as_stream(stream), value, offw, ref, out, lv, N, S, \
+                     Lq, L, P, bpi, ldv)
+  if (rec) {
+    if (ldv == CH) FWD_LAUNCH(msda_fwd_rec_kernel, true); else FWD_LAUNCH(msda_fwd_rec_kernel, false);
+  } else {
+    if (ldv == CH) FWD_LAUNCH(msda_fwd_kernel, true); else FWD_LAUNCH(msda_fwd_kernel, false);
+  }
+#undef FWD_LAUNCH
   CAPE_LAUNCH_CHECK("cape_msda_fwd");
   return 0;
 }
@@ -700,18 +729,32 @@
 extern "C" int cape_msda_bwd_atomic(const float* d_out, const float* value, const float* offw, const float* ref,
                                     const int* shapes, const int* level_start, float* d_value, float* d_offw, float* d_ref,
                                     int N, int S, int Lq, int L, int P, cape_stream_t stream) {
+  return cape_msda_bwd_atomic_ld(d_out, value, offw, ref, shapes, level_start, d_value, d_offw, d_ref, N, S, Lq, L, P, CH, CH, stream);
+}
+
+extern "C" int cape_msda_bwd_atomic_ld(const float* d_out, const float* value, const float* offw, const float* ref,
+                                       const int* shapes, const int* level_start, float* d_value, float* d_offw, float* d_ref,
+                                       int N, int S, int Lq, int L, int P, int ldv, int ldd, cape_stream_t stream) {
   if (msda_bwd_check(d_out, value, offw, ref, shapes, level_start, d_value, d_offw, L, P)) return 1;
+  if (msda_ld_check("cape_msda_bwd_atomic", "ldv", ldv, S, false) || msda_ld_check("cape_msda_bwd_atomic", "ldd", ldd, S, false))
+    return 1;
   if (N <= 0 || Lq <= 0) return 0;
   Levels lv;
   if (fill_levels(lv, shapes, level_start, L, S)) return 1;
-  hipError_t e = hipMemsetAsync(d_value, 0, sizeof(float) * (size_t)N * S * CH, as_stream(stream));
+  hipError_t e = ldd == CH ? hipMemsetAsync(d_value, 0, sizeof(float) * (size_t)N * S * CH, as_stream(stream))
+                           : hipMemset2DAsync(d_value, sizeof(float) * (size_t)ldd, 0, sizeof(float) * CH, (size_t)N * S,
+                                              as_stream(stream));
   if (e == hipSuccess && d_ref) e = hipMemsetAsync(d_ref, 0, sizeof(float) * (size_t)N * Lq * L * 2, as_stream(stream));
   if (e != hipSuccess) return cape_set_error("cape_msda_bwd_atomic: memset: %s", hipGetErrorString(e));
   const long long waves = (long long)N * Lq * 4;
   const long long blocks = (waves + 3) / 4;
   CAPE_REQUIRE(blocks < (1ll << 31), "cape_msda_bwd_atomic: grid too large");
-  hipLaunchKernelGGL(msda_bwd_kernel, dim3((unsigned)blocks), dim3(256), 0, as_stream(stream), d_out, value, offw, ref,
-                     d_value, d_offw, d_ref, lv, N, S, Lq, L, P, waves);
+  if (ldv == CH && ldd == CH)
+    hipLaunchKernelGGL(msda_bwd_kernel<true>, dim3((unsigned)blocks), dim3(256), 0, as_stream(stream), d_out, value, offw, ref,
+                       d_value, d_offw, d_ref, lv, N, S, Lq, L, P, waves, ldv, ldd);
+  else
+    hipLaunchKernelGGL(msda_bwd_kernel<false>, dim3((unsigned)blocks), dim3(256), 0, as_stream(stream), d_out, value, offw, ref,
+                       d_value, d_offw, d_ref, lv, N, S, Lq, L, P, waves, ldv, ldd);
   CAPE_LAUNCH_CHECK("cape_msda_bwd_atomic");
   return 0;
 }
@@ -719,15 +762,21 @@
 extern "C" int cape_msda_bwd(const float* d_out, const float* value, const float* offw, const float* ref,
                              const int* shapes, const int* level_start, float* d_value, float* d_offw, float* d_ref,
                              int N, int S, int Lq, int L, int P, cape_stream_t stream) {
-  return cape_msda_bwd_ex(d_out, value, offw, ref, shapes, level_start, d_value, d_offw, d_ref, N, S, Lq, L, P, 0, stream);
+  return cape_msda_bwd_ld(d_out, value, offw, ref, shapes, level_start, d_value, d_offw, d_ref, N, S, Lq, L, P, 0, CH, CH, stream);
 }
 
 extern "C" int cape_msda_bwd_ex(const float* d_out, const float* value, const float* offw, const float* ref,
                                 const int* shapes, const int* level_start, float* d_value, float* d_offw, float* d_ref,
                                 int N, int S, int Lq, int L, int P, int value_accum, cape_stream_t stream) {
+  return cape_msda_bwd_ld(d_out, value, offw, ref, shapes, level_start, d_value, d_offw, d_ref, N, S, Lq, L, P, value_accum, CH, CH,
+                          stream);
+}
+
+extern "C" int cape_msda_bwd_ld(const float* d_out, const float* value, const float* offw, const float* ref,
+                                const int* shapes, const int* level_start, float* d_value, float* d_offw, float* d_ref,
+                                int N, int S, int Lq, int L, int P, int value_accum, int ldv, int ldd, cape_stream_t stream) {
   CAPE_REQUIRE(value_accum == 0 || value_accum == 1, "cape_msda_bwd_ex: value_accum must be 0 (fp64 slab) or 1 (fixed-point pairs)");
   if (msda_bwd_check(d_out, value, offw, ref, shapes, level_start, d_value, d_offw, L, P)) return 1;
-  if (N <= 0 || Lq <= 0) return 0;
   const size_t kMaxSlab = 160 * 1024 - 16 * 64 * (sizeof(uint4) + sizeof(float4)) - 512;
   int vc = 8;
   while (vc >= 2 && (size_t)(S + 1) * vc * sizeof(double) > kMaxSlab) vc >>= 1;
@@ -737,36 +786,44 @@
   const int bpi = (Lq + 3) / 4;
   const long long vblocks = imgs8 * 8 * HEADS * (HD / (vc < 2 ? 2 : vc));
   if (force_atomic || vc < 2 || S >= 65535 || vblocks >= (1ll << 31) || imgs8 * 8 * bpi >= (1ll << 31))
-    return cape_msda_bwd_atomic(d_out, value, offw, ref, shapes, level_start, d_value, d_offw, d_ref, N, S, Lq, L, P, stream);
+    return cape_msda_bwd_atomic_ld(d_out, value, offw, ref, shapes, level_start, d_value, d_offw, d_ref, N, S, Lq, L, P, ldv, ldd,
+                                   stream);
+  if (msda_ld_check("cape_msda_bwd", "ldv", ldv, S, true) || msda_ld_check("cape_msda_bwd", "ldd", ldd, S, false)) return 1;
+  if (N <= 0 || Lq <= 0) return 0;
   Levels lv;
   if (fill_levels(lv, shapes, level_start, L, S)) return 1;
   static bool attr_done = false;
   if (!attr_done) {
-    hipError_t e = hipFuncSetAttribute(reinterpret_cast<const void*>(msda_bwd_value_kernel<8>),
-                                       hipFuncAttributeMaxDynamicSharedMemorySize, (int)kMaxSlab);
-    if (e == hipSuccess) e = hipFuncSetAttribute(reinterpret_cast<const void*>(msda_bwd_value_kernel<4>),
-                                                 hipFuncAttributeMaxDynamicSharedMemorySize, (int)kMaxSlab);
-    if (e == hipSuccess) e = hipFuncSetAttribute(reinterpret_cast<const void*>(msda_bwd_value_kernel<2>),
-                                                 hipFuncAttributeMaxDynamicSharedMemorySize, (int)kMaxSlab);
-    if (e == hipSuccess) e = hipFuncSetAttribute(reinterpret_cast<const void*>(msda_bwd_value_fx_kernel<8>),
-                                                 hipFuncAttributeMaxDynamicSharedMemorySize, (int)kMaxSlab);
-    if (e == hipSuccess) e = hipFuncSetAttribute(reinterpret_cast<const void*>(msda_bwd_value_fx_kernel<4>),
-                                                 hipFuncAttributeMaxDynamicSharedMemorySize, (int)kMaxSlab);
-    if (e == hipSuccess) e = hipFuncSetAttribute(reinterpret_cast<const void*>(msda_bwd_value_fx_kernel<2>),
-                                                 hipFuncAttributeMaxDynamicSharedMemorySize, (int)kMaxSlab);
-    if (e != hipSuccess) return cape_set_error("cape_msda_bwd: hipFuncSetAttribute: %s", hipGetErrorString(e));
+    const void* fns[] = {reinterpret_cast<const void*>(msda_bwd_value_kernel<8, true>),
+                         reinterpret_cast<const void*>(msda_bwd_value_kernel<4, true>),
+                         reinterpret_cast<const void*>(msda_bwd_value_kernel<2, true>),
+                         reinterpret_cast<const void*>(msda_bwd_value_fx_kernel<8, true>),
+                         reinterpret_cast<const void*>(msda_bwd_value_fx_kernel<4, true>),
+                         reinterpret_cast<const void*>(msda_bwd_value_fx_kernel<2, true>),
+                         reinterpret_cast<const void*>(msda_bwd_value_kernel<8, false>),
+                         reinterpret_cast<const void*>(msda_bwd_value_kernel<4, false>),
+                         reinterpret_cast<const void*>(msda_bwd_value_kernel<2, false>),
+                         reinterpret_cast<const void*>(msda_bwd_value_fx_kernel<8, false>),
+                         reinterpret_cast<const void*>(msda_bwd_value_fx_kernel<4, false>),
+                         reinterpret_cast<const void*>(msda_bwd_value_fx_kernel<2, false>)};
+    for (const void* fn : fns) {
+      const hipError_t e = hipFuncSetAttribute(fn, hipFuncAttributeMaxDynamicSharedMemorySize, (int)kMaxSlab);
+      if (e != hipSuccess) return cape_set_error("cape_msda_bwd: hipFuncSetAttribute: %s", hipGetErrorString(e));
+    }
     attr_done = true;
   }
   if (d_ref && P != 4) {
     hipError_t e = hipMemsetAsync(d_ref, 0, sizeof(float) * (size_t)N * Lq * L * 2, as_stream(stream));
     if (e != hipSuccess) return cape_set_error("cape_msda_bwd: memset: %s", hipGetErrorString(e));
   }
-#define VALUE_LAUNCH(W)                                                                                                     \
-  hipLaunchKernelGGL((msda_bwd_value_kernel<W>), dim3((unsigned)vblocks), dim3(1024), slab_bytes, as_stream(stream), d_out, offw, \
-                     ref, d_value, lv, N, S, Lq, L, P)
-#define VALUE_LAUNCH_FX(W)                                                                                                  \
-  hipLaunchKernelGGL((msda_bwd_value_fx_kernel<W>), dim3((unsigned)fxblocks), dim3(1024), fx_bytes, as_stream(stream),           \
-                     d_out, offw, ref, d_value, lv, N, S, Lq, L, P)
+#define VALUE_LAUNCH_D(W, DENSE)                                                                                            \
+  hipLaunchKernelGGL((msda_bwd_value_kernel<W, DENSE>), dim3((unsigned)vblocks), dim3(1024), slab_bytes, as_stream(stream), d_out, \
+                     offw, ref, d_value, lv, N, S, Lq, L, P, ldd)
+#define VALUE_LAUNCH_FX_D(W, DENSE)                                                                                         \
+  hipLaunchKernelGGL((msda_bwd_value_fx_kernel<W, DENSE>), dim3((unsigned)fxblocks), dim3(1024), fx_bytes, as_stream(stream),    \
+                     d_out, offw, ref, d_value, lv, N, S, Lq, L, P, ldd)
+#define VALUE_LAUNCH(W) do { if (ldd == CH) VALUE_LAUNCH_D(W, true); else VALUE_LAUNCH_D(W, false); } while (0)
+#define VALUE_LAUNCH_FX(W) do { if (ldd == CH) VALUE_LAUNCH_FX_D(W, true); else VALUE_LAUNCH_FX_D(W, false); } while (0)
   if (value_accum == 1) {
     int vp = vc;
     while (vp > 2 && imgs8 * 8 * HEADS * (HD / (2 * vp)) < 256) vp >>= 1;
@@ -778,8 +835,14 @@
   }
 #undef VALUE_LAUNCH_FX
 #undef VALUE_LAUNCH
-  hipLaunchKernelGGL(msda_bwd_offw_kernel, dim3((unsigned)(imgs8 * 8 * bpi)), dim3(256), 0, as_stream(stream), d_out, value, offw,
-                     ref, d_offw, d_ref, lv, N, S, Lq, L, P, bpi);
+#undef VALUE_LAUNCH_FX_D
+#undef VALUE_LAUNCH_D
+  if (ldv == CH)
+    hipLaunchKernelGGL(msda_bwd_offw_kernel<true>, dim3((unsigned)(imgs8 * 8 * bpi)), dim3(256), 0, as_stream(stream), d_out, value,
+                       offw, ref, d_offw, d_ref, lv, N, S, Lq, L, P, bpi, ldv);
+  else
+    hipLaunchKernelGGL(msda_bwd_offw_kernel<false>, dim3((unsigned)(imgs8 * 8 * bpi)), dim3(256), 0, as_stream(stream), d_out, value,
+                       offw, ref, d_offw, d_ref, lv, N, S, Lq, L, P, bpi, ldv);
   CAPE_LAUNCH_CHECK("cape_msda_bwd");
   return 0;
 }
diff --git a/category-agnostic-pose-estimation_amd/hip/functional.py b/category-agnostic-pose-estimation_amd/hip/functional.py
--- a/category-agnostic-pose-estimation_amd/hip/functional.py
+++ b/category-agnostic-pose-estimation_amd/hip/functional.py
@@ -862,10 +862,25 @@
     return LevelPosFn.apply(geo, level_embed, *masks_u8)
 
 
+class _WideGrad:
+    __slots__ = ("shape", "device", "buf")
+
+    def __init__(self, shape, device):
+        self.shape, self.device, self.buf = tuple(shape), device, None
+
+    def block(self, l, C=256):
+        if self.buf is None:
+            self.buf = torch.empty(self.shape, dtype=torch.float32, device=self.device)
+        return self.buf[..., l * C:(l + 1) * C]
+
+
 class MSDAFn(torch.autograd.Function):
     @staticmethod
     def forward(ctx, value, offw, ref, geo, P):
-        value, offw, ref = _c(value), _c(offw), _c(ref)
+        ctx.wide = getattr(value, "_cape_wide", None)
+        if ctx.wide is None:
+            value = _c(value)
+        offw, ref = _c(offw), _c(ref)
         N, Lq = offw.shape[0], offw.shape[1]
         out = ops.msda_fwd(value, offw, ref, geo, N, Lq, P)
         ctx.save_for_backward(value, offw, ref)
@@ -876,12 +891,92 @@
     def backward(ctx, d_out):
         value, offw, ref = ctx.saved_tensors
         geo, N, Lq, P = ctx.meta
-        dv, do, dr = ops.msda_bwd(_c(d_out), value, offw, ref, geo, N, Lq, P, need_ref_grad=ctx.needs_input_grad[2])
+        d_value = ctx.wide[0].block(ctx.wide[1]).view(value.shape) if ctx.wide is not None else None
+        dv, do, dr = ops.msda_bwd(_c(d_out), value, offw, ref, geo, N, Lq, P, need_ref_grad=ctx.needs_input_grad[2], d_value=d_value)
         return dv, do, dr, None, None
 
 
 def msda(value, offw, ref, geo, P=4):
     return MSDAFn.apply(value, offw, ref, geo, P)
+
+
+class ValueHoistFn(torch.autograd.Function):
+
+    @staticmethod
+    def forward(ctx, x, rowmask_u8, wide, *wb):
+        k = len(wb) // 2
+        w0, b0 = wb[0], wb[k]
+        K, C = x.shape[-1], w0.shape[0]
+        NT = k * C
+        x2 = _c(x).view(-1, K)
+        M = x2.shape[0]
+        y = torch.empty(*x.shape[:-1], NT, dtype=torch.float32, device=x.device)
+        ops.gemm(x2, torch.as_strided(w0, (NT, K), (K, 1)), y, M, NT, K, bias=torch.as_strided(b0, (NT,), (1,)))
+        if rowmask_u8 is not None:
+            ops.zero_rows(y, rowmask_u8)
+        ctx.save_for_backward(x2, rowmask_u8)
+        ctx.refs, ctx.wide, ctx.slot = wb, wide, _slot_of(x)
+        ctx.meta = (x.shape, M, K, C, k)
+        ctx.set_materialize_grads(False)
+        wide.shape, wide.device = tuple(y.shape), y.device
+        return tuple(y[..., l * C:(l + 1) * C] for l in range(k))
+
+    @staticmethod
+    def backward(ctx, *grads):
+        x2, rm = ctx.saved_tensors
+        xshape, M, K, C, k = ctx.meta
+        NT = k * C
+        wide = ctx.wide
+        for l, g in enumerate(grads):
+            blk = wide.block(l, C)
+            if g is None:
+                blk.zero_()
+            elif g.data_ptr() != blk.data_ptr() or g.stride() != blk.stride():
+                blk.copy_(g)
+        dy = wide.buf.view(M, NT)
+        wide.buf = None
+        if rm is not None:
+            ops.zero_rows(dy, rm)
+        dx = None
+        if ctx.needs_input_grad[0]:
+            dx, acc = _grad_target(ctx.slot, (M, K), dy.device)
+            ops.gemm(dy, torch.as_strided(ctx.refs[0], (NT, K), (K, 1)), dx, M, K, NT, a_mode=0, b_mode=1, ldb=K, accumulate=acc)
+            dx = dx.view(xshape)
+        pg = _ParamGrads(ctx.refs)
+        dws, dbs = pg.bufs[:k], pg.bufs[k:]
+        with pg.side(dy, x2):
+            if all(_adjacent(dws[i], dws[i + 1]) and _adjacent(dbs[i], dbs[i + 1]) for i in range(k - 1)):
+                pg.gemm(dy, x2, torch.as_strided(dws[0], (NT, K), (K, 1)), NT, K, M, a_mode=1, b_mode=1, lda=NT, accumulate=True,
+                        split_k=ops.pick_split_k(NT, K, M), colsum_out=torch.as_strided(dbs[0], (NT,), (1,)))
+            else:
+                for l in range(k):
+                    pg.gemm(dy[:, l * C:], x2, dws[l], C, K, M, a_mode=1, b_mode=1, lda=NT, accumulate=True,
+                            split_k=ops.pick_split_k(C, K, M), colsum_out=dbs[l])
+        return (dx, None, None) + pg.result()
+
+
+_HOIST_VERSIONS = {}
+
+
+def value_hoist_ok(ws, bs):
+    k = len(ws)
+    return (k > 1 and all(w.shape == ws[0].shape and w.shape[0] == 256 for w in ws) and all(b is not None for b in bs)
+            and all(_adjacent(ws[i], ws[i + 1]) and _adjacent(bs[i], bs[i + 1]) for i in range(k - 1)))
+
+
+def value_hoist(x, ws, bs, rowmask_u8=None):
+    vers = tuple(w._version for w in ws)
+    key = ws[0].data_ptr()
+    if _HOIST_VERSIONS.get(key, vers) != vers and not capturing():
+        for kk in [kk for kk in ops.PackedWeights.entries if kk[0] == key and kk[1] == len(ws) * ws[0].shape[0]]:
+            del ops.PackedWeights.entries[kk]
+        ops.PackedWeights._table = None
+    _HOIST_VERSIONS[key] = vers
+    wide = _WideGrad((), x.device)
+    outs = ValueHoistFn.apply(x, rowmask_u8, wide, *ws, *bs)
+    for l, o in enumerate(outs):
+        o._cape_wide = (wide, l)
+    return outs
 
 
 def _from_row(t, r):
diff --git a/category-agnostic-pose-estimation_amd/hip/lib.py b/category-agnostic-pose-estimation_amd/hip/lib.py
--- a/category-agnostic-pose-estimation_amd/hip/lib.py
+++ b/category-agnostic-pose-estimation_amd/hip/lib.py
@@ -126,6 +126,9 @@
     "cape_msda_bwd": [P, P, P, P, P, P, P, P, P, I, I, I, I, I, P],
     "cape_msda_bwd_ex": [P, P, P, P, P, P, P, P, P, I, I, I, I, I, I, P],
     "cape_msda_bwd_atomic": [P, P, P, P, P, P, P, P, P, I, I, I, I, I, P],
+    "cape_msda_fwd_ld": [P, P, P, P, P, P, I, I, I, I, I, I, P],
+    "cape_msda_bwd_ld": [P, P, P, P, P, P, P, P, P, I, I, I, I, I, I, I, I, P],
+    "cape_msda_bwd_atomic_ld": [P, P, P, P, P, P, P, P, P, I, I, I, I, I, I, I, P],
     "cape_attn_fwd": [P, P, P, P, P, LL, LL, LL, LL, LL, LL, LL, LL, I, I, I, I, F, I, I, P, F, P, U32, P],
     "cape_attn_bwd": [P, P, P, P, P, P, P, P, P, LL, LL, LL, LL, LL, LL, LL, LL, I, I, I, I, F, I, I, P, F, P, U32, P],
     "cape_flash_attn_fwd": [P, P, P, P, P, LL, LL, LL, LL, LL, LL, LL, LL, I, I, I, I, F, I, I, P, F, P, U32, P],
diff --git a/category-agnostic-pose-estimation_amd/hip/ops.py b/category-agnostic-pose-estimation_amd/hip/ops.py
--- a/category-agnostic-pose-estimation_amd/hip/ops.py
+++ b/category-agnostic-pose-estimation_amd/hip/ops.py
@@ -456,13 +456,26 @@
         self._starts_c = (ctypes.c_int * self.L)(*starts)
 
 
+def _msda_ld(t, N, S, name):
+    _chk(t, name, contiguous=False)
+    assert t.numel() == N * S * 256, f"{name}: expected {N} x {S} rows of 256"
+    if t.is_contiguous():
+        return 256
+    ld = t.stride(-2)
+    assert t.shape[-1] == 256 and t.stride(-1) == 1 and ld >= 256 and t.dim() in (2, 3), f"{name}: not a column block of a row-major tensor"
+    assert t.dim() == 2 or t.shape[0] == 1 or t.stride(0) == S * ld, f"{name}: images must be {S} rows apart"
+    assert t.data_ptr() % 16 == 0 and _avail(t) >= (N * S - 1) * ld + 256, f"{name}: misaligned or too small"
+    return ld
+
+
 def msda_fwd(value, offw, ref, geo, N, Lq, P=4):
-    for t, n in ((value, "value"), (offw, "offw"), (ref, "ref")):
+    for t, n in ((offw, "offw"), (ref, "ref")):
         _chk(t, "msda." + n)
-    assert value.numel() == N * geo.S * 256 and offw.numel() == N * Lq * 8 * geo.L * P * 3
+    ldv = _msda_ld(value, N, geo.S, "msda.value")
+    assert offw.numel() == N * Lq * 8 * geo.L * P * 3
     assert ref.numel() == N * Lq * geo.L * 2
     out = torch.empty(N, Lq, 256, dtype=_F32, device=value.device)
-    lib.call("cape_msda_fwd", _p(value), _p(offw), _p(ref), geo._shapes_c, geo._starts_c, _p(out), N, geo.S, Lq, geo.L, P,
+    lib.call("cape_msda_fwd_ld", _p(value), _p(offw), _p(ref), geo._shapes_c, geo._starts_c, _p(out), N, geo.S, Lq, geo.L, P, ldv,
              _stream())
     return out
 
@@ -470,19 +483,22 @@
 MSDA_VALUE_ACCUM = os.environ.get("CAPE_MSDA_VALUE_ACCUM", "auto")
 
 
-def msda_bwd(d_out, value, offw, ref, geo, N, Lq, P=4, need_ref_grad=True, form="split"):
+def msda_bwd(d_out, value, offw, ref, geo, N, Lq, P=4, need_ref_grad=True, form="split", d_value=None):
     _chk(d_out, "msda_bwd.d_out")
-    d_value = torch.empty_like(value)
+    ldv = _msda_ld(value, N, geo.S, "msda_bwd.value")
+    if d_value is None:
+        d_value = torch.empty_like(value) if value.is_contiguous() else torch.empty(value.shape, dtype=_F32, device=value.device)
+    ldd = _msda_ld(d_value, N, geo.S, "msda_bwd.d_value")
     d_offw = torch.empty_like(offw)
     d_ref = torch.empty_like(ref) if need_ref_grad else None
     if form == "split":
         form = MSDA_VALUE_ACCUM if MSDA_VALUE_ACCUM != "auto" else ("f64" if GEMM_PRECISION == 0 else "fx")
     if form == "atomic":
-        lib.call("cape_msda_bwd_atomic", _p(d_out), _p(value), _p(offw), _p(ref), geo._shapes_c, geo._starts_c, _p(d_value),
-                 _p(d_offw), _p(d_ref), N, geo.S, Lq, geo.L, P, _stream())
+        lib.call("cape_msda_bwd_atomic_ld", _p(d_out), _p(value), _p(offw), _p(ref), geo._shapes_c, geo._starts_c, _p(d_value),
+                 _p(d_offw), _p(d_ref), N, geo.S, Lq, geo.L, P, ldv, ldd, _stream())
     else:
-        lib.call("cape_msda_bwd_ex", _p(d_out), _p(value), _p(offw), _p(ref), geo._shapes_c, geo._starts_c, _p(d_value),
-                 _p(d_offw), _p(d_ref), N, geo.S, Lq, geo.L, P, {"f64": 0, "fx": 1}[form], _stream())
+        lib.call("cape_msda_bwd_ld", _p(d_out), _p(value), _p(offw), _p(ref), geo._shapes_c, geo._starts_c, _p(d_value),
+                 _p(d_offw), _p(d_ref), N, geo.S, Lq, geo.L, P, {"f64": 0, "fx": 1}[form], ldv, ldd, _stream())
     return d_value, d_offw, d_ref
 
 
diff --git a/category-agnostic-pose-estimation_amd/models/deformable_transformer_v2.py b/category-agnostic-pose-estimation_amd/models/deformable_transformer_v2.py
--- a/category-agnostic-pose-estimation_amd/models/deformable_transformer_v2.py
+++ b/category-agnostic-pose-estimation_amd/models/deformable_transformer_v2.py
@@ -15,6 +15,7 @@
 
 _ONES_VR = {}
 _FUSED_SELF_ATTN = os.environ.get("CAPE_DEC_SELF_ATTN_NODE", "1") == "1"
+_MSDA_FORCED = ("CAPE_MSDA_BWD_ATOMIC", "CAPE_MSDA_FWD_SHUFFLE")
 
 
 def Embedding(num_embeddings, embedding_dim, padding_idx=None, zero_init=False):
@@ -63,7 +64,7 @@
         self._streams = [ops.new_stream_id() for _ in range(8)]
 
     def forward(self, tgt, query_pos, reference_points, src, geo, padding_rows_u8=None, support_features=None,
-                support_kpm_u8=None):
+                support_kpm_u8=None, value=None):
         p = self.dropout2.p if self.training else 0.0
         st = self._streams
         sa = self.self_attn
@@ -91,7 +92,7 @@
         else:
             tgt, t_r = HF.fanout(tgt, 2)
             tgt_pos = HF.add(t_r, qp_s)
-        t2 = self.cross_attn(tgt_pos, reference_points, src, geo, padding_rows_u8)
+        t2 = self.cross_attn(tgt_pos, reference_points, src, geo, padding_rows_u8, value=value)
         tgt = HF.add_layernorm(tgt, t2, self.norm1.weight, self.norm1.bias, dropout_p=p, rng_stream=st[4])
         t_f, t_r = HF.fanout(tgt, 2)
         h = HF.ffn(t_f, self.linear1.weight, self.linear1.bias, self.linear2.weight, self.linear2.bias, dropout_p=p, rng_stream=st[5])
@@ -186,6 +187,15 @@
             x = HF.linear(x, layer.weight, layer.bias, relu=(i < n - 1))
         return x
 
+    def _hoisted_values(self, src, padding_rows_u8):
+        if os.environ.get("CAPE_DEC_VALUE_HOIST", "1") == "0" or any(os.environ.get(k) is not None for k in _MSDA_FORCED):
+            return None
+        ws = [l.cross_attn.value_proj.weight for l in self.layers]
+        bs = [l.cross_attn.value_proj.bias for l in self.layers]
+        if not (src.is_cuda and src.shape[-1] == 256 and HF.value_hoist_ok(ws, bs)):
+            return None
+        return HF.value_hoist(src, ws, bs, padding_rows_u8)
+
     def forward(self, reference_points, src, geo, src_valid_ratios, padding_rows_u8=None, seq_kwargs=None,
                 support_features=None, support_mask=None):
         if support_features is None:
@@ -198,13 +208,18 @@
                                  delta_y1=seq_kwargs["delta_y1"], delta_y2=seq_kwargs["delta_y2"])
         hs, refs, clss = [], [], []
         nl = len(self.layers)
-        mems = HF.fanout(src, nl)
+        values = self._hoisted_values(src, padding_rows_u8)
+        if values is None:
+            values = (None,) * nl
+            mems = HF.fanout(src, nl)
+        else:
+            mems = (src,) * nl
         sups = HF.fanout(support_features, nl) if support_features is not None else (None,) * nl
         for lid, layer in enumerate(self.layers):
             r_scale, r_sine, r_ref = HF.fanout(reference_points, 3)
             ref_in = HF.ref_scale(r_scale, src_valid_ratios)
             query_pos = self._query_pos(r_sine)
-            output = layer(output, query_pos, ref_in, mems[lid], geo, padding_rows_u8, sups[lid], kpm)
+            output = layer(output, query_pos, ref_in, mems[lid], geo, padding_rows_u8, sups[lid], kpm, value=values[lid])
             o_mlp, o_cls, o_hs, output = HF.fanout(output, 4)
             delta = self._mlp(self.coords_embed[lid], o_mlp)
             reference_points, r_keep = HF.fanout(HF.refine(delta, r_ref), 2)
diff --git a/category-agnostic-pose-estimation_amd/runtime/arena.py b/category-agnostic-pose-estimation_amd/runtime/arena.py
--- a/category-agnostic-pose-estimation_amd/runtime/arena.py
+++ b/category-agnostic-pose-estimation_amd/runtime/arena.py
@@ -1,3 +1,5 @@
+import re
+
 import torch
 
 DEAD_PREFIXES = ("support_cross_attention_layers.", "support_attn_layer_norms.", "base_model.room_class_embed.")
@@ -77,4 +79,24 @@
         if a.endswith("sampling_offsets.weight") and b.endswith("sampling_offsets.bias") and c.endswith("attention_weights.weight") \
                 and a[:-len("sampling_offsets.weight")] == c[:-len("attention_weights.weight")]:
             out[i + 1], out[i + 2] = out[i + 2], out[i + 1]
+    return _colocate_dec_value_proj(out)
+
+
+_DEC_VALUE_PROJ = re.compile(r"^(.*decoder\.layers\.)(\d+)\.cross_attn\.value_proj\.(weight|bias)$")
+
+
+def _colocate_dec_value_proj(named):
+    out = list(named)
+    for prefix in dict.fromkeys(m.group(1) for m in (_DEC_VALUE_PROJ.match(n) for n, _ in out) if m):
+        found = {"weight": [], "bias": []}
+        for i, (n, _) in enumerate(out):
+            m = _DEC_VALUE_PROJ.match(n)
+            if m and m.group(1) == prefix:
+                found[m.group(3)].append((int(m.group(2)), i))
+        if len(found["weight"]) < 2 or len(found["weight"]) != len(found["bias"]):
+            continue
+        idx = [i for _, i in sorted(found["weight"])] + [i for _, i in sorted(found["bias"])]
+        first, moved = min(idx), set(idx)
+        out = ([e for i, e in enumerate(out) if i < first and i not in moved] + [out[i] for i in idx]
+               + [e for i, e in enumerate(out) if i > first and i not in moved])
     return out
diff --git a/include/cape_hip.h b/include/cape_hip.h
--- a/include/cape_hip.h
+++ b/include/cape_hip.h
@@ -151,6 +151,16 @@
                          const int* shapes, const int* level_start, float* d_value, float* d_offw, float* d_ref,
                          int N, int S, int Lq, int L, int P, cape_stream_t stream);
 
+int cape_msda_fwd_ld(const float* value, const float* offw, const float* ref, const int* shapes,
+                     const int* level_start, float* out, int N, int S, int Lq, int L, int P, int ldv,
+                     cape_stream_t stream);
+int cape_msda_bwd_ld(const float* d_out, const float* value, const float* offw, const float* ref,
+                     const int* shapes, const int* level_start, float* d_value, float* d_offw, float* d_ref,
+                     int N, int S, int Lq, int L, int P, int value_accum, int ldv, int ldd, cape_stream_t stream);
+int cape_msda_bwd_atomic_ld(const float* d_out, const float* value, const float* offw, const float* ref,
+                            const int* shapes, const int* level_start, float* d_value, float* d_offw, float* d_ref,
+                            int N, int S, int Lq, int L, int P, int ldv, int ldd, cape_stream_t stream);
+
 int cape_attn_fwd(const float* Q, const float* K, const float* V, float* O, float* lse,
                   long long ldq, long long ldk, long long ldv, long long ldo,
                   long long bsq, long long bsk, long long bsv, long long bso,
```
